# GuildOfWeavers/distaff

Hardware: AMD Instinct MI355X
Metric: trace_cells_per_sec (higher is better)
Workload: dtype u128 (prime field 2^128-45*2^40+1, 4x u32 limbs)

## Files before the change

### distaff_amd/csrc/air_kernel.h

```cpp
#pragma once
#include "ctx.h"
#include "air_stack_nested.h"

#ifndef AIR_THREADS
#define AIR_THREADS 128
#endif
#ifndef AIR_WAVES_PER_SIMD
#define AIR_WAVES_PER_SIMD 2
#endif

struct AirConsts { fe sponge_mds[16], sponge_inv_mds[16], hasher_mds[36], hasher_inv_mds[36]; };

struct AirArgs {
    const fe* lde;
    fe* out;
    const fe* coef;
    const fe* tc;
    const fe* periodic;
    const AirConsts* consts;
    fe* partial;
    fe* ev[10];
    const fe* tw_lo; const fe* tw_hi; uint32_t lo_bits;
    unsigned long long* bad_step;
    size_t n, col_stride;
    uint32_t log_n, log_N, log_b, W, ctx_depth, loop_depth, stack_depth;
    uint32_t cl, ll, sl;
    uint32_t coset_step;
    uint32_t q0;
    uint32_t num_inputs, num_outputs;
    fe inputs[8], outputs[8], program_hash[2], op_count;
};



__device__ __forceinline__ fe dpow(const AirArgs& a, uint64_t e) {
    uint32_t l = (uint32_t)e & ((1u << a.lo_bits) - 1u), h = (uint32_t)(e >> a.lo_bits);
    fe v = a.tw_lo[l];
    return h ? fe_mul(v, a.tw_hi[h]) : v;
}

template <int Wd>
__device__ __forceinline__ void matmul(fe* s, const fe* m) {
    fe r[Wd];
#pragma unroll
    for (int i = 0; i < Wd; i++) {
        fe_acc A; fe_acc_zero(A);
#pragma unroll
        for (int j = 0; j < Wd; j++) fe_acc_mac(A, m[i * Wd + j], s[j]);
        r[i] = fe_acc_reduce(A);
    }
#pragma unroll
    for (int i = 0; i < Wd; i++) s[i] = r[i];
}

#define AS_BOUNDARY 1
#define AS_OP_BITS 2
#define AS_SPONGE 4
#define AS_STACK_MOVE 8
#define AS_STACK_HIGH 16
#define AS_STACK_ARITH 32
#define AS_STACK_RESCR 64
#define AS_FLOW 128
#define AS_STACK_ANY (AS_STACK_MOVE | AS_STACK_HIGH | AS_STACK_ARITH | AS_STACK_RESCR)
#define AS_STACK_AUX (AS_STACK_MOVE | AS_STACK_ARITH)
#define AF_FIRST 1
#define AF_LAST 2
#define AF_EV_IN 4
#define AF_EV_OUT 8

struct AirStack {
    bool nested, deep;
    int sl;
    int slots;
    int partials;
};
constexpr AirStack air_stack(int sd, int slcap) {
    if (sd == 4) return AirStack{true, false, 8, 4, 6};
    if (sd == 0 && slcap == 8) return AirStack{true, false, 8, 8, 10};
    if (sd == 0 && slcap == 12) return AirStack{true, true, 12, 8, 10};
    return AirStack{false, false, sd ? (sd > 8 ? sd : 8) : slcap, 0, 0};
}

template <uint32_t ACC_MASK>
struct Acc {
    fe_acc res_acc;
    fe_acc adj_acc[6];
    fe res, adj[6];
    bool nonzero;
    const fe* tc; uint32_t nc;
    __device__ __forceinline__ void emit(uint32_t cidx, int slot, const fe& d) {
        nonzero |= !fe_is_zero(d);
        fe_acc_mac(res_acc, d, tc[cidx]);
        if ((ACC_MASK >> slot) & 1u) fe_acc_mac(adj_acc[slot], d, tc[nc + cidx]);
        else adj[slot] = fe_add(adj[slot], fe_mul(d, tc[nc + cidx]));
    }
};
constexpr uint32_t air_acc_mask(const AirStack& st, int sect) { return !st.nested ? 0u : ((sect & AS_OP_BITS) ? 0x01u : 0x3Fu); }

struct AirColumns {
    const fe* cur_p; const fe* nxt_p; size_t cs;
    __device__ __forceinline__ fe cur(size_t c) const { return cur_p[c * cs]; }
    __device__ __forceinline__ fe nxt(size_t c) const { return nxt_p[c * cs]; }
};

template <int CL, int LL>
struct AirRows {
    fe c_opc, n_opc, c_sp[4], n_sp[4], cf[3], n_cf[3], ld[5], hd[2];
    fe c_ctx[CL], n_ctx[CL], c_lp[LL], n_lp[LL];
};

template <int SL, int CL, int LL>
__device__ __forceinline__ void air_load_rows(AirRows<CL, LL>& r, fe* o, fe* nw, const AirArgs& a, const AirColumns p, int sd) {
    r.c_opc = p.cur(0); r.n_opc = p.nxt(0);
#pragma unroll
    for (int i = 0; i < 4; i++) { r.c_sp[i] = p.cur(1 + i); r.n_sp[i] = p.nxt(1 + i); }
#pragma unroll
    for (int i = 0; i < 3; i++) { r.cf[i] = p.cur(5 + i); r.n_cf[i] = p.nxt(5 + i); }
#pragma unroll
    for (int i = 0; i < 5; i++) r.ld[i] = p.cur(8 + i);
#pragma unroll
    for (int i = 0; i < 2; i++) r.hd[i] = p.cur(13 + i);
    uint32_t col = 15;
#pragma unroll
    for (int i = 0; i < CL; i++) { bool on = (uint32_t)i < a.ctx_depth; r.c_ctx[i] = on ? p.cur(col + i) : fe_zero(); r.n_ctx[i] = on ? p.nxt(col + i) : fe_zero(); }
    col += a.ctx_depth;
#pragma unroll
    for (int i = 0; i < LL; i++) { bool on = (uint32_t)i < a.loop_depth; r.c_lp[i] = on ? p.cur(col + i) : fe_zero(); r.n_lp[i] = on ? p.nxt(col + i) : fe_zero(); }
    col += a.loop_depth;
#pragma unroll
    for (int i = 0; i < SL; i++) { bool on = i < sd; o[i] = on ? p.cur(col + i) : fe_zero(); nw[i] = on ? p.nxt(col + i) : fe_zero(); }
}

struct AirFlags {
    fe cff[8], hdf[4], begin_flag, noop_flag, n_void, assert_flag;
    fe lo2[4], mid[4], top[2];
    fe ld_all;
    __device__ __forceinline__ fe ldf(int idx) const { return fe_mul(fe_mul(lo2[idx & 3], mid[(idx >> 2) & 3]), top[idx >> 4]); }
};

__device__ __forceinline__ void air_bit_pairs(fe* t, const fe& a, const fe& na, const fe& nb) {
    t[0] = fe_mul(na, nb); t[1] = fe_sub(nb, t[0]); t[2] = fe_sub(na, t[0]); t[3] = fe_sub(a, t[1]);
}

template <class ROWS>
__device__ __forceinline__ void air_op_flags(AirFlags& f, const ROWS& r) {
    const fe* cf = r.cf; const fe* ld = r.ld; const fe* hd = r.hd;
    {
        fe n0 = bnot(cf[0]), n1 = bnot(cf[1]), n2 = bnot(cf[2]);
        fe t[4];
        air_bit_pairs(t, cf[0], n0, n1);
#pragma unroll
        for (int i = 0; i < 4; i++) { f.cff[i] = fe_mul(t[i], n2); f.cff[4 + i] = fe_sub(t[i], f.cff[i]); }
        f.n_void = fe_mul(fe_mul(r.n_cf[0], r.n_cf[1]), r.n_cf[2]);
        fe l0 = bnot(ld[0]), l1 = bnot(ld[1]), l2 = bnot(ld[2]), l3 = bnot(ld[3]);
        f.lo2[0] = fe_mul(l0, l1); f.lo2[1] = fe_sub(l1, f.lo2[0]);
        f.lo2[2] = fe_mul(l0, cf[1]);
        f.lo2[3] = fe_sub(ld[0], f.lo2[1]);
        air_bit_pairs(f.mid, ld[2], l2, l3);
        f.top[0] = bnot(ld[4]); f.top[1] = ld[4];
        fe h0 = bnot(hd[0]), h1 = bnot(hd[1]);
        air_bit_pairs(f.hdf, hd[0], h0, h1);
    }
    {
        fe ld0 = f.ldf(0);
        f.ld_all = f.ldf(31);
        f.begin_flag = fe_mul(ld0, f.hdf[0]);
        f.noop_flag = fe_mul(f.ld_all, f.hdf[3]);
        f.hdf[0] = fe_mul(f.hdf[0], ld[0]);
        f.assert_flag = fe_mul(ld0, hd[0]);
    }
}

#include "air_stack_perop.h"

template <int CL, int LL, class ROWS>
__device__ __forceinline__ void air_boundary(const AirArgs& a, const ROWS& r, const fe* o, int cl, int ll, uint64_t gi, uint64_t n64, uint64_t nmask, uint32_t ql, size_t k) {
    const fe xp = dpow(a, (gi * (6 * n64 + 2)) & nmask);
    const fe one = fe_one();
#pragma unroll 1
    for (int pass = 0; pass < 2; pass++) {
        const fe* cc = a.coef + pass * 94;
        fe_acc R, A; fe_acc_zero(R); fe_acc_zero(A);
        auto term = [&](const fe& v, uint32_t idx) { fe_acc_mac(R, v, cc[idx]); fe_acc_mac(A, v, cc[idx + 1]); };
        term(pass ? fe_sub(r.c_opc, a.op_count) : r.c_opc, 0);
        if (pass == 0) { for (int i = 0; i < 4; i++) term(r.c_sp[i], 2 + 2 * i); }
        else { for (int i = 0; i < 2; i++) term(fe_sub(r.c_sp[i], a.program_hash[i]), 2 + 2 * i); }
        for (int i = 0; i < 3; i++) term(pass ? fe_sub(r.cf[i], one) : r.cf[i], 10 + 2 * i);
        for (int i = 0; i < 5; i++) term(pass ? fe_sub(r.ld[i], one) : r.ld[i], 16 + 2 * i);
        for (int i = 0; i < 2; i++) term(pass ? fe_sub(r.hd[i], one) : r.hd[i], 26 + 2 * i);
        for (int i = 0; i < CL; i++) if (i < cl) term(r.c_ctx[i], 30 + 2 * i);
        for (int i = 0; i < LL; i++) if (i < ll) term(r.c_lp[i], 62 + 2 * i);
        const uint32_t nio = pass ? a.num_outputs : a.num_inputs;
#pragma unroll
        for (int i = 0; i < 8; i++) if ((uint32_t)i < nio) term(fe_sub(o[i], pass ? a.outputs[i] : a.inputs[i]), 78 + 2 * i);
        const fe adj = fe_acc_reduce(A);
        fe_acc_mac(R, adj, xp);
        a.out[((size_t)pass * gridDim.y + ql) * a.n + k] = fe_acc_reduce(R);
    }
}

template <class ACC, class ROWS>
__device__ __forceinline__ void air_op_bits(ACC& acc, const ROWS& r, const AirFlags& f, const fe* per) {
    const fe* cf = r.cf; const fe* ld = r.ld; const fe* hd = r.hd;
    fe cf_sum = fe_add(fe_add(cf[0], cf[1]), cf[2]);
    const fe ld_prod = f.ld_all, hd_prod = f.hdf[3], all_prod = f.noop_flag;
#pragma unroll
    for (int i = 0; i < 3; i++) acc.emit(i, 0, is_bin(cf[i]));
#pragma unroll
    for (int i = 0; i < 5; i++) acc.emit(3 + i, 0, is_bin(ld[i]));
#pragma unroll
    for (int i = 0; i < 2; i++) acc.emit(8 + i, 0, is_bin(hd[i]));
    const fe is_hacc = f.cff[0];
    acc.emit(10, 1, fe_sub(fe_add(r.c_opc, is_hacc), r.n_opc));
    acc.emit(11, 5, fe_mul(r.c_opc, fe_add(fe_sub(bnot(ld_prod), hd_prod), all_prod)));
    acc.emit(12, 5, fe_mul(cf_sum, bnot(all_prod)));
    acc.emit(13, 3, fe_mul(f.cff[7], bnot(f.n_void)));
    fe prefix = fe_add(fe_add(f.cff[1], f.cff[4]), fe_add(f.cff[5], f.cff[6]));
    fe v = fe_mul(prefix, per[21]);
    v = fe_add(v, fe_mul(fe_add(f.cff[2], f.cff[3]), per[20]));
    v = fe_add(v, fe_mul(f.hdf[0], per[22]));
    acc.emit(14, 2, v);
}

template <bool OWN_CTX, class ACC, class ROWS>
__device__ __forceinline__ void air_sponge(ACC& acc, const AirArgs& a, const AirColumns p, const ROWS& r, const fe* nw, const AirFlags& f, const fe* per) {
    const AirConsts* consts = a.consts;
    fe ctx0;
    if constexpr (OWN_CTX) ctx0 = 0u < a.ctx_depth ? p.cur(15u) : fe_zero();
    else ctx0 = r.c_ctx[0];
    fe sp[4];
    const fe f_begin = f.cff[1], f_tend = f.cff[2], f_fend = f.cff[3], f_loop = f.cff[4], f_wrap = f.cff[5], f_break = f.cff[6], f_void = f.cff[7];
    {
        fe os[4], ns[4];
#pragma unroll
        for (int i = 0; i < 4; i++) os[i] = fe_cube(fe_add(r.c_sp[i], per[i]));
        matmul<4>(os, consts->sponge_mds);
        fe op_code = r.hd[1];
        op_code = fe_add(fe_double(op_code), r.hd[0]);
        op_code = fe_add(fe_double(op_code), r.ld[4]);
        op_code = fe_add(fe_double(op_code), r.ld[3]);
        op_code = fe_add(fe_double(op_code), r.ld[2]);
        op_code = fe_add(fe_double(op_code), r.ld[1]);
        op_code = fe_add(fe_double(op_code), r.ld[0]);
        os[0] = fe_add(os[0], op_code);
        os[1] = fe_add(os[1], fe_mul(nw[0], f.hdf[0]));
#pragma unroll
        for (int i = 0; i < 4; i++) ns[i] = r.n_sp[i];
        matmul<4>(ns, consts->sponge_inv_mds);
#pragma unroll
        for (int i = 0; i < 4; i++) ns[i] = fe_sub(fe_cube(ns[i]), per[4 + i]);
        const fe clr = fe_add(fe_add(f_begin, f_loop), f_wrap);
        const fe cpy = fe_add(f_break, f_void);
        const fe tf = fe_add(f_tend, f_fend);
        const fe xf[4] = {tf, f_tend, f_fend, tf};
        const fe xv[4] = {fe_sub(ctx0, r.n_sp[0]), fe_sub(r.c_sp[0], r.n_sp[1]), fe_sub(r.c_sp[0], r.n_sp[2]), r.n_sp[3]};
#pragma unroll
        for (int i = 0; i < 4; i++) {
            fe_acc A; fe_acc_zero(A);
            fe_acc_mac(A, f.cff[0], fe_sub(os[i], ns[i]));
            fe_acc_mac(A, clr, r.n_sp[i]);
            fe_acc_mac(A, cpy, fe_sub(r.c_sp[i], r.n_sp[i]));
            fe_acc_mac(A, xf[i], xv[i]);
            sp[i] = fe_acc_reduce(A);
        }
    }
    acc.emit(15, 3, sp[0]); acc.emit(16, 4, sp[1]); acc.emit(17, 3, sp[2]); acc.emit(18, 3, sp[3]);
}

template <class CUR>
__device__ __forceinline__ fe air_ctx_constraint(int i, int cl, const fe& push, const fe& pop, const fe& ccpy, const fe& sp0, CUR&& ctx_cur, const fe& ni) {
    fe_acc A; fe_acc_zero(A);
    fe_acc_mac(A, push, fe_sub(i == 0 ? sp0 : ctx_cur(i - 1), ni));
    fe_acc_mac(A, pop, i + 1 < cl ? fe_sub(ctx_cur(i + 1), ni) : ni);
    fe_acc_mac(A, ccpy, fe_sub(ctx_cur(i), ni));
    return fe_acc_reduce(A);
}

template <int CL, int LL, class ACC, class ROWS>
__device__ __forceinline__ void air_flow(ACC& acc, const AirArgs& a, const AirColumns p, const ROWS& r, const AirFlags& f, int cl, int ll) {
    const fe f_begin = f.cff[1], f_tend = f.cff[2], f_fend = f.cff[3], f_loop = f.cff[4], f_wrap = f.cff[5], f_break = f.cff[6], f_void = f.cff[7];
    acc.emit(19, 2, fe_mul(fe_add(f_wrap, f_break), fe_sub(r.c_sp[0], r.c_lp[0])));
    const fe push = fe_add(f_begin, f_loop), pop = fe_add(f_tend, f_fend), ccpy = fe_add(fe_add(f_wrap, f_break), f_void);
    const fe lcpy = fe_add(fe_add(fe_add(f_begin, f_tend), fe_add(f_fend, f_wrap)), f_void);
    if constexpr (CL <= 2 && LL <= 1) {
        auto ctx_cur = [&](int j) { return r.c_ctx[j < 0 ? 0 : (j < CL ? j : 0)]; };
#pragma unroll
        for (int i = 0; i < CL; i++) {
            if (i >= cl) break;
            const fe v = air_ctx_constraint(i, cl, push, pop, ccpy, r.c_sp[0], ctx_cur, r.n_ctx[i]);
            acc.emit(20 + i, 2, v);
        }
#pragma unroll
        for (int i = 0; i < LL; i++) {
            if (i >= ll) break;
            fe v = fe_mul(lcpy, fe_sub(r.c_lp[i], r.n_lp[i]));
            if (i >= 1) v = fe_add(v, fe_mul(f_loop, fe_sub(r.c_lp[i - 1 < 0 ? 0 : i - 1], r.n_lp[i])));
            v = fe_add(v, fe_mul(f_break, i + 1 < ll ? fe_sub(r.c_lp[i + 1 < LL ? i + 1 : 0], r.n_lp[i]) : r.n_lp[i]));
            acc.emit(20 + cl + i, 2, v);
        }
    } else {
        auto ctx_cur = [&](int i) { return (uint32_t)i < a.ctx_depth ? p.cur(15 + i) : fe_zero(); };
        auto ctx_nxt = [&](int i) { return (uint32_t)i < a.ctx_depth ? p.nxt(15 + i) : fe_zero(); };
        const uint32_t lcol = 15 + a.ctx_depth;
        auto lp_cur = [&](int i) { return (uint32_t)i < a.loop_depth ? p.cur(lcol + i) : fe_zero(); };
        auto lp_nxt = [&](int i) { return (uint32_t)i < a.loop_depth ? p.nxt(lcol + i) : fe_zero(); };
#pragma unroll 1
        for (int i = 0; i < cl; i++) {
            const fe ni = ctx_nxt(i);
            acc.emit(20 + i, 2, air_ctx_constraint(i, cl, push, pop, ccpy, r.c_sp[0], ctx_cur, ni));
        }
#pragma unroll 1
        for (int i = 0; i < ll; i++) {
            const fe ni = lp_nxt(i);
            fe_acc A; fe_acc_zero(A);
            fe_acc_mac(A, lcpy, fe_sub(lp_cur(i), ni));
            if (i >= 1) fe_acc_mac(A, f_loop, fe_sub(lp_cur(i - 1), ni));
            fe_acc_mac(A, f_break, i + 1 < ll ? fe_sub(lp_cur(i + 1), ni) : ni);
            acc.emit(20 + cl + i, 2, fe_acc_reduce(A));
        }
    }
}

template <int SD, int NS>
__device__ __forceinline__ void air_rescr_differences(fe* resc, const fe* o, const fe* nw, const fe* per, const AirConsts* consts) {
    constexpr int NZ = (SD != 0 && SD < 6) ? SD : 6;
    fe os[6], ns[6];
#pragma unroll
    for (int i = 0; i < 6; i++) os[i] = i < NZ ? fe_cube(fe_add(o[i], per[8 + i])) : per[23 + i];
    matmul<6>(os, consts->hasher_mds);
    constexpr int NR = NS < 6 ? NS : 6;
#pragma unroll
    for (int i = 0; i < NR; i++) {
        fe_acc A; fe_acc_zero(A);
#pragma unroll
        for (int j = 0; j < NZ; j++) fe_acc_mac(A, consts->hasher_inv_mds[i * 6 + j], nw[j]);
        ns[i] = fe_acc_reduce(A);
    }
#pragma unroll
    for (int i = 0; i < NR; i++) resc[i] = fe_sub(fe_sub(fe_cube(ns[i]), per[14 + i]), os[i]);
}

template <int SD, bool DEEP, int NS, int SL, uint32_t GROUPS, bool EV_IN, bool EV_OUT, class ACC, class ROWS>
__device__ __forceinline__ void air_stack_nested(ACC& acc, const AirArgs& a, const ROWS& r, const fe* o, const fe* nw, const AirFlags& f, const fe* per, int cl, int ll, int sl, int sd, size_t pidx) {
    StackRows rows;
#pragma unroll
    for (int i = 0; i < 8; i++) { rows.o[i] = o[i]; rows.nw[i] = nw[i]; }
#pragma unroll
    for (int i = 8; i < 12; i++) rows.o[i] = DEEP ? o[i < SL ? i : 0] : fe_zero();
    rows.sl = DEEP ? sl : 8;
    const fe lo0h = fe_mul(f.lo2[0], r.hd[0]);
    StackHigh high;
    high.push = f.hdf[0]; high.cmp = f.hdf[1]; high.rescr = f.hdf[2]; high.keep = fe_add(f.begin_flag, f.noop_flag);
    if constexpr ((GROUPS & AG_RESCR) != 0) air_rescr_differences<SD, NS>(high.resc, o, nw, per, a.consts);
    const uint32_t sbase = 20 + cl + ll;
    static_for_air<0, NS + 2>([&](auto k_) {
        constexpr int kk = decltype(k_)::value;
        constexpr int I = kk < NS ? kk : (kk == NS ? ST_AUX0 : ST_AUX1);
        constexpr bool touched = st_touches<I, GROUPS>();
        if constexpr (touched || !EV_OUT) {
            if (I >= 8 || I < sd) {
                fe v = fe_zero();
                if constexpr (touched) v = st_output<I, GROUPS, SD, DEEP>(rows, f.lo2, lo0h, f.mid, f.top, high);
                fe* slot = a.ev[I] + pidx;
                if constexpr (EV_IN) v = touched ? fe_add(v, *slot) : *slot;
                if constexpr (EV_OUT) *slot = v;
                else acc.emit(I >= 8 ? sbase + (I - 8) : sbase + 2 + I, 4, v);
            }
        } else if constexpr (!EV_IN) {
            a.ev[I][pidx] = fe_zero();
        }
    });
}

template <class ACC>
__device__ __forceinline__ void air_stack_deep_slots(ACC& acc, const AirArgs& a, const AirColumns p, const AirFlags& f, int cl, int ll, int sl, int sd) {
    const fe* lo2 = f.lo2; const fe* mid = f.mid; const fe* top = f.top;
    const uint32_t sbase = 20 + cl + ll;
    const fe lo_all = fe_add(fe_add(lo2[0], lo2[1]), fe_add(lo2[2], lo2[3]));
    fe fl1, fl2, fl4, fr1, fr2, fr4, fcp;
    { fe_acc A; fe_acc_zero(A); fe_acc_mac(A, mid[0], lo2[3]); fe_acc_mac(A, mid[2], lo_all); fl1 = fe_add(fe_mul(top[0], fe_acc_reduce(A)), f.assert_flag); }
    { fe_acc A; fe_acc_zero(A); fe_acc_mac(A, mid[0], fe_add(lo2[1], lo2[2])); fe_acc_mac(A, mid[1], fe_add(lo2[1], lo2[3])); fl2 = fe_mul(top[0], fe_acc_reduce(A)); }
    fl4 = fe_mul(top[0], fe_mul(mid[1], fe_add(lo2[0], lo2[2])));
    fr1 = fe_add(fe_mul(top[1], fe_mul(mid[0], fe_add(lo2[0], lo2[2]))), f.hdf[0]);
    { fe_acc A; fe_acc_zero(A); fe_acc_mac(A, mid[0], fe_add(lo2[1], lo2[3])); fe_acc_mac(A, mid[1], lo2[1]); fr2 = fe_mul(top[1], fe_acc_reduce(A)); }
    fr4 = fe_mul(top[1], fe_mul(mid[1], lo2[0]));
    {
        fe_acc A; fe_acc_zero(A); fe_acc_mac(A, mid[2], lo_all); fe_acc_mac(A, mid[3], fe_add(lo2[0], lo2[1]));
        fe_acc B; fe_acc_zero(B); fe_acc_mac(B, top[1], fe_acc_reduce(A)); fe_acc_mac(B, top[0], fe_mul(mid[3], fe_add(fe_add(lo2[0], lo2[1]), lo2[2])));
        fcp = fe_add(fe_add(fe_acc_reduce(B), fe_add(f.hdf[1], f.hdf[2])), fe_add(f.begin_flag, f.noop_flag));
    }
    const uint32_t scol = 15 + a.ctx_depth + a.loop_depth;
#pragma unroll 1
    for (int i = 8; i < sd; i++) {
        const fe ni = p.nxt(scol + i);
        auto item = [&](int j) { return p.cur(scol + j); };
        auto left = [&](int num) { return i + num < sl ? fe_sub(item(i + num), ni) : ni; };
        fe_acc A; fe_acc_zero(A);
        fe_acc_mac(A, fcp, fe_sub(item(i), ni));
        fe_acc_mac(A, fr1, fe_sub(item(i - 1), ni)); fe_acc_mac(A, fr2, fe_sub(item(i - 2), ni)); fe_acc_mac(A, fr4, fe_sub(item(i - 4), ni));
        fe_acc_mac(A, fl1, left(1)); fe_acc_mac(A, fl2, left(2)); fe_acc_mac(A, fl4, left(4));
        acc.emit(sbase + 2 + i, 4, fe_acc_reduce(A));
    }
}

__device__ __forceinline__ void air_combine(const fe& res, const fe* adj, const AirArgs& a, size_t k, uint32_t ql, uint32_t qg, uint64_t gi, uint64_t n64, uint64_t nmask) {
    const bool on_trace = (qg == 0);
    fe t;
    if (on_trace && k + 1 != a.n) {
        t = fe_zero();
    } else {
        const uint32_t degs[6] = {2, 3, 4, 6, 7, 8};
        fe_acc T; fe_acc_zero(T);
        fe_acc_add(T, res);
#pragma unroll
        for (int g = 0; g < 6; g++) {
            uint64_t p = 8 * n64 - 1 - (n64 - 1) * degs[g];
            fe_acc_mac(T, adj[g], dpow(a, (gi * p) & nmask));
        }
        t = fe_acc_reduce(T);
    }
    a.out[((size_t)2 * gridDim.y + ql) * a.n + k] = t;
}

template <int CL, int LL, int SD, int SLCAP, int SECT, uint32_t GROUPS, int FLAGS>
__global__ void __launch_bounds__(AIR_THREADS, AIR_WAVES_PER_SIMD) air_kernel(AirArgs a) {
    constexpr AirStack ST = air_stack(SD, SLCAP);
    constexpr bool FIRST = (FLAGS & AF_FIRST) != 0, LAST = (FLAGS & AF_LAST) != 0, EV_IN = (FLAGS & AF_EV_IN) != 0, EV_OUT = (FLAGS & AF_EV_OUT) != 0;
    static_assert(ST.nested ? (SECT & AS_STACK_ANY) == 0 : (GROUPS == 0 && !EV_IN && !EV_OUT),
                  "nested-sum instances select stack operations with GROUPS, the per-operation instance with SECT");
    const int cl = (int)a.cl, ll = (int)a.ll;
    const int sl = SD ? ST.sl : (int)a.sl;
    const int sd = SD ? SD : (int)a.stack_depth;
    const size_t k = (size_t)blockIdx.x * AIR_THREADS + threadIdx.x;
    if (k >= a.n) return;
    const uint32_t ql = blockIdx.y;
    const uint32_t qg = a.q0 + ql;
    const uint32_t jl = ql * a.coset_step;
    const size_t kn = (k + 1 == a.n) ? 0 : k + 1;
    const AirColumns cols{a.lde + (size_t)jl * a.n + k, a.lde + (size_t)jl * a.n + kn, a.col_stride};
    const uint64_t nmask = ((uint64_t)1 << a.log_N) - 1;
    const uint64_t gi = ((uint64_t)k << a.log_b) + (uint64_t)qg * a.coset_step;
    const uint32_t step = (uint32_t)(((uint64_t)k << 3) + qg);
    const uint64_t n64 = a.n;

    AirRows<CL, LL> rows;
    fe o[ST.sl], nw[ST.sl];
    air_load_rows<ST.sl>(rows, o, nw, a, cols, sd);
    if constexpr ((SECT & AS_BOUNDARY) != 0) air_boundary<CL, LL>(a, rows, o, cl, ll, gi, n64, nmask, ql, k);
    if constexpr (SECT == AS_BOUNDARY) return;
    AirFlags flags;
    air_op_flags(flags, rows);
    const fe* per = a.periodic + (size_t)(step & 127u) * AIR_PERIODIC_STRIDE;

    constexpr uint32_t ACC_MASK = air_acc_mask(ST, SECT);
    Acc<ACC_MASK> acc;
#pragma unroll
    for (int i = 0; i < 6; i++) if ((ACC_MASK >> i) & 1u) fe_acc_zero(acc.adj_acc[i]);
    fe_acc_zero(acc.res_acc); acc.res = fe_zero(); acc.nonzero = false; acc.tc = a.tc; acc.nc = 20 + cl + ll + 2 + sd;
#pragma unroll
    for (int i = 0; i < 6; i++) acc.adj[i] = fe_zero();
    const size_t pstride = (size_t)gridDim.y * a.n, pidx = (size_t)ql * a.n + k;

    if constexpr ((SECT & AS_OP_BITS) != 0) air_op_bits(acc, rows, flags, per);
    if constexpr ((SECT & AS_SPONGE) != 0) air_sponge<SD == 0>(acc, a, cols, rows, nw, flags, per);
    if constexpr ((SECT & AS_FLOW) != 0) air_flow<CL, LL>(acc, a, cols, rows, flags, cl, ll);
    if constexpr (ST.nested && (GROUPS & AG_STACK_ALL & ~AG_DEEP) != 0) air_stack_nested<SD, ST.deep, ST.slots, ST.sl, GROUPS, EV_IN, EV_OUT>(acc, a, rows, o, nw, flags, per, cl, ll, sl, sd, pidx);
    if constexpr (!ST.nested && (SECT & AS_STACK_ANY) != 0) air_stack_per_operation<ST.sl, SECT>(acc, o, nw, sl, sd, 20 + cl + ll, flags, per, a.consts);
    if constexpr (ST.deep && (GROUPS & AG_DEEP) != 0) air_stack_deep_slots(acc, a, cols, flags, cl, ll, sl, sd);

    constexpr bool EMITS_STACK = (SECT & AS_STACK_ANY) != 0 || (GROUPS & AG_DEEP) != 0 || ((GROUPS & AG_STACK_ALL) != 0 && !EV_OUT);
    constexpr uint32_t USED = ((SECT & AS_OP_BITS) ? 0x2Fu : 0u) | ((SECT & AS_SPONGE) ? 0x18u : 0u) | ((SECT & AS_FLOW) ? 0x04u : 0u) | (EMITS_STACK ? 0x10u : 0u);
    const bool on_trace = (qg == 0);
    if (on_trace && k + 1 != a.n && acc.nonzero) atomicMin(a.bad_step, (unsigned long long)k);
    acc.res = fe_acc_reduce(acc.res_acc);
#pragma unroll
    for (int i = 0; i < 6; i++) if (((ACC_MASK & USED) >> i) & 1u) acc.adj[i] = fe_add(acc.adj[i], fe_acc_reduce(acc.adj_acc[i]));
    if constexpr (!FIRST) {
        acc.res = fe_add(acc.res, a.partial[pidx]);
#pragma unroll
        for (int i = 0; i < 6; i++) if (LAST || ((USED >> i) & 1u)) acc.adj[i] = fe_add(acc.adj[i], a.partial[(size_t)(i + 1) * pstride + pidx]);
    }
    if constexpr (!LAST) {
        a.partial[pidx] = acc.res;
#pragma unroll
        for (int i = 0; i < 6; i++) if (FIRST || ((USED >> i) & 1u)) a.partial[(size_t)(i + 1) * pstride + pidx] = acc.adj[i];
        return;
    }
    air_combine(acc.res, acc.adj, a, k, ql, qg, gi, n64, nmask);
}


template <int CL, int LL, int SD, int SLCAP, int SECT, uint32_t GROUPS, int FLAGS>
static void launch_air(dst_ctx* c, const AirArgs& a, uint32_t Q) {
    dim3 g((unsigned)((c->n + AIR_THREADS - 1) / AIR_THREADS), Q);
    static char name[64];
    if (!name[0]) snprintf(name, sizeof(name), "air_kernel<%d,%d,%d,%d,%d,%u,%d>", CL, LL, SD, SLCAP, SECT, (unsigned)GROUPS, FLAGS);
    constexpr int NS = air_stack(SD, SLCAP).partials;
    const double units = c->W + ((FLAGS & AF_FIRST) ? 0 : 7) + ((FLAGS & AF_LAST) ? 1 : 7) + ((SECT & AS_BOUNDARY) ? 2 : 0) + ((FLAGS & AF_EV_IN) ? NS : 0) + ((FLAGS & AF_EV_OUT) ? NS : 0);
    { KScope ks_(c, name, 16.0 * c->n * Q * units, true); hipLaunchKernelGGL((air_kernel<CL, LL, SD, SLCAP, SECT, GROUPS, FLAGS>), g, dim3(AIR_THREADS), 0, c->stream, a); }
}
template <int CL, int LL, int SD, int SLCAP>
static void launch_air_boundary(dst_ctx* c, const AirArgs& a, uint32_t Q) {
#if DST_TEST_HOOKS
    if (dst_internal_boundary_by_evaluation(c)) launch_air<CL, LL, SD, SLCAP, AS_BOUNDARY, 0, 0>(c, a, Q);
#endif
}
void air_launch_sd4(dst_ctx* c, const AirArgs& a, uint32_t Q);
void air_launch_small(dst_ctx* c, const AirArgs& a, uint32_t Q);
void air_launch_deep(dst_ctx* c, const AirArgs& a, uint32_t Q);
void air_launch_generic(dst_ctx* c, const AirArgs& a, uint32_t Q);
```

### distaff_amd/csrc/api.hip

```cpp
#include <algorithm>
#include <cstdio>
#include <cstdlib>
#include "ctx.h"
#include "host/ctx_tables.h"
#include "host/steps.h"
#include "host_proof.h"
#include "host_util.h"
#include "host_vm.h"
#include "verify/host_verify.h"

using namespace dsth;
#include "host/steps_impl.h"
using step::wall_ms;
using step::event_ms;

static std::string g_create_error;

static std::vector<fe> build_periodic_table() {
    const size_t cyc = 128;
    std::vector<fe> out(cyc * AIR_PERIODIC_STRIDE);
    u128 w16 = fe_to_u128(h_root_of_unity(4)), w128 = fe_to_u128(h_root_of_unity(7));
    u128 w16_inv = hf_pow(w16, 15), inv16 = hf_pow(16, FIELD_P - 2);
    static const uint8_t masks[3][16] = {{0, 1, 1, 1, 1, 1, 1, 1, 1, 1, 1, 1, 1, 1, 1, 1}, {1, 1, 1, 1, 1, 1, 1, 1, 1, 1, 1, 1, 1, 1, 1, 0}, {0, 1, 1, 1, 1, 1, 1, 1, 0, 1, 1, 1, 1, 1, 1, 1}};
    for (int row = 0; row < 23; row++) {
        u128 vals[16], coef[16];
        for (int i = 0; i < 16; i++) vals[i] = row < 8 ? limbs(SPONGE_ARK[row][i]) : row < 20 ? limbs(HASHER_ARK[row - 8][i]) : (u128)masks[row - 20][i];
        for (int j = 0; j < 16; j++) {
            u128 acc = 0;
            for (int i = 0; i < 16; i++) acc = hf_add(acc, hf_mul(vals[i], hf_pow(w16_inv, (u128)((i * j) % 16))));
            coef[j] = hf_mul(acc, inv16);
        }
        for (size_t s = 0; s < cyc; s++) {
            u128 x = hf_pow(w128, s), acc = 0, pw = 1;
            for (int j = 0; j < 16; j++) { acc = hf_add(acc, hf_mul(coef[j], pw)); pw = hf_mul(pw, x); }
            out[s * AIR_PERIODIC_STRIDE + row] = fe_from_u128(acc);
        }
    }
    for (size_t s = 0; s < cyc; s++)
        for (int i = 0; i < 6; i++) { const u128 v = fe_to_u128(out[s * AIR_PERIODIC_STRIDE + 8 + i]); out[s * AIR_PERIODIC_STRIDE + 23 + i] = fe_from_u128(hf_mul(hf_mul(v, v), v)); }
    return out;
}

static void free_all(dst_ctx* c) {
    void* ptrs[] = {c->tw_lo, c->tw_hi, c->itw_lo, c->itw_hi, c->prescale, c->dit_last, c->tw4_lde, c->tw4_fwd, c->tw4_inv, c->tw4_row_fwd, c->tw4_row_inv, c->tmp2, c->periodic, c->trace == c->lde ? nullptr : c->trace, c->polys, c->lde, c->tmp,
                    c->trace_leaves, c->trace_nodes, c->air_consts, c->ceval, c->cwork, c->cpoly, c->cevals, c->cnodes, c->comp_poly, c->comp, c->scratch, c->d_u64, c->d_stage, c->d_fri_chain};
    for (void* p : ptrs) if (p) hipFree(p);
    for (auto& pass : c->ntt_stage_tw) for (fe_tw* p : pass) if (p) hipFree(p);
    for (auto& pass : c->ntt_pre_tw) for (fe_tw* p : pass) if (p) hipFree(p);
    for (auto& e : c->kpending) { hipEventDestroy(e.e0); hipEventDestroy(e.e1); }
    for (hipEvent_t e : c->event_pool) hipEventDestroy(e);
    if (c->gather_buf) hipFree(c->gather_buf);
    if (c->trace_upper) hipFree(c->trace_upper);
    if (c->c_upper) hipFree(c->c_upper);
    for (int d = 0; d < DST_MAX_FRI_LAYERS; d++) if (c->fri_upper[d]) hipFree(c->fri_upper[d]);
    if (c->fri_nat0) hipFree(c->fri_nat0);
    for (int d = 0; d < DST_MAX_FRI_LAYERS; d++) {
        if (d > 0 && c->fri_e[d]) hipFree(c->fri_e[d]);
        if (c->fri_leaves[d]) hipFree(c->fri_leaves[d]);
        if (c->fri_nodes[d]) hipFree(c->fri_nodes[d]);
    }
    for (hipEvent_t e : c->upload_done) hipEventDestroy(e);
    if (c->upload_stream) hipStreamDestroy(c->upload_stream);
    for (hipEvent_t e : c->comm_events) hipEventDestroy(e);
    if (c->comm_stream) hipStreamDestroy(c->comm_stream);
    if (c->d_status) hipFree(c->d_status);
    if (c->h_stage) hipHostFree(c->h_stage);
    for (hipEvent_t e : c->ph_ev) if (e) hipEventDestroy(e);
    for (hipEvent_t e : c->sh_ev) if (e) hipEventDestroy(e);
    for (auto& ce : c->coll_ev) { hipEventDestroy(ce.e0); hipEventDestroy(ce.e1); }
    if (c->stream) hipStreamDestroy(c->stream);
}

static int ctx_init(dst_ctx* c) {
    c->read_switches();
    const dst_params& p = c->prm;
    if (p.log_trace_length < 4 || p.log_trace_length > 24) { c->err = "log_trace_length must be in [4, 24]"; return DST_ERR_ARG; }
    if (p.log_blowup < 4 || p.log_blowup > 8) { c->err = "extension factor must be in [16, 256]"; return DST_ERR_ARG; }
    if (p.ctx_depth > 16 || p.loop_depth > 8) { c->err = "context / loop depth out of range"; return DST_ERR_ARG; }
    if (p.width >= 128 || p.width <= 15 + p.ctx_depth + p.loop_depth) { c->err = "register count out of range"; return DST_ERR_ARG; }
    if (p.num_queries == 0 || p.num_queries > 128 || p.grinding_factor > 32) { c->err = "invalid proof options"; return DST_ERR_ARG; }
    if (p.world == 0 || p.rank >= p.world || (p.world & (p.world - 1)) || p.world > 8 || p.world > (1u << p.log_blowup) / 2) {
        c->err = "invalid rank / world: world must be a power of two <= min(8, blowup / 2)"; return DST_ERR_ARG;
    }
    if (p.log_trace_length + p.log_blowup > 40) { c->err = "LDE domain exceeds 2^40"; return DST_ERR_ARG; }
    c->log_n = p.log_trace_length; c->log_b = p.log_blowup; c->log_N = c->log_n + c->log_b;
    c->n = (size_t)1 << c->log_n; c->B = (size_t)1 << c->log_b; c->N = c->n * c->B; c->W = p.width;
    c->Bc = c->B / p.world; c->j0 = c->Bc * p.rank;
    c->stack_depth = p.width - 15 - p.ctx_depth - p.loop_depth;
    if (c->stack_depth > 32) { c->err = "user stack deeper than 32 registers"; return DST_ERR_ARG; }
    c->device = p.device;
    HIP_TRY(c, hipSetDevice(c->device));
    HIP_TRY(c, hipStreamCreate(&c->stream));
    HIP_TRY(c, hipHostMalloc((void**)&c->h_stage, HS_TOTAL, hipHostMallocDefault));
    for (hipEvent_t& e : c->ph_ev) HIP_TRY(c, hipEventCreate(&e));

    fe wN = h_root_of_unity(c->log_N), wN_inv = h_inv(wN);
    c->tw_lo_bits = (c->log_N + 1) / 2;
    uint32_t hi_bits = c->log_N - c->tw_lo_bits;
    int r;
    if ((r = dev_upload(c, &c->tw_lo, h_powers(wN, (size_t)1 << c->tw_lo_bits)))) return r;
    if ((r = dev_upload(c, &c->tw_hi, h_powers(h_pow(wN, (u128)1 << c->tw_lo_bits), (size_t)1 << hi_bits)))) return r;
    if ((r = dev_upload(c, &c->itw_lo, h_powers(wN_inv, (size_t)1 << c->tw_lo_bits)))) return r;
    if ((r = dev_upload(c, &c->itw_hi, h_powers(h_pow(wN_inv, (u128)1 << c->tw_lo_bits), (size_t)1 << hi_bits)))) return r;
    if ((r = k_ntt_init(c))) return r;
    if ((r = dev_upload(c, &c->periodic, build_periodic_table()))) return r;
    c->n_inv = fe_from_u128(hf_pow((u128)c->n, FIELD_P - 2));
    c->n_inv_tw = fe_tw_make(c->n_inv);
    c->eight_inv = fe_from_u128(hf_pow(8, FIELD_P - 2));
    c->four_inv = fe_from_u128(hf_pow(4, FIELD_P - 2));
    c->iota = h_root_of_unity(2);
    c->g_trace = h_root_of_unity(c->log_n);
    c->x_last = h_inv(c->g_trace);

    const size_t n = c->n, Nl = c->Bc * n;
    if ((r = dev_alloc(c, &c->polys, (c->W + c->prm.world - 1) / c->prm.world * c->prm.world * n))) return r;
    if ((r = dev_alloc(c, &c->lde, c->W * Nl))) return r;
    if (c->j0 == 0 && c->Bc > 1 && !c->sw_is("DISTAFF_TRACE_BUFFER", "1")) { c->trace = c->lde; c->trace_stride = Nl; }
    else { if ((r = dev_alloc(c, &c->trace, c->W * n))) return r; c->trace_stride = n; }
    size_t stage_cap = (size_t)12 << 30;
    { size_t free_b = 0, total_b = 0; if (hipMemGetInfo(&free_b, &total_b) == hipSuccess && free_b / 4 < stage_cap) stage_cap = free_b / 4; }
    c->tmp_regs = 4;
    while (c->tmp_regs < c->W && (c->tmp_regs + 1) * (c->plan.count == 3 ? 2 : 1) * c->Bc * n * sizeof(fe) <= stage_cap) c->tmp_regs++;
    if (const char* e = c->sw("DISTAFF_TMP_REGS")) { const long k = atol(e); if (k >= 4 && k <= (long)c->W) c->tmp_regs = (size_t)k; }
    if ((r = dev_alloc(c, &c->tmp, c->Bc * c->tmp_regs * n))) return r;
    if (c->plan.count == 3 && (r = dev_alloc(c, &c->tmp2, c->Bc * c->tmp_regs * n))) return r;
    if ((r = dev_alloc(c, &c->trace_leaves, Nl))) return r;
    if ((r = dev_alloc(c, &c->trace_nodes, Nl))) return r;
    if ((r = dev_alloc(c, &c->ceval, 3 * 8 * n))) return r;
    if ((r = dev_alloc(c, &c->cwork, 8 * 8 * n))) return r;
    if ((r = dev_alloc(c, &c->cpoly, 8 * n))) return r;
    if ((r = dev_alloc(c, &c->cevals, Nl))) return r;
    if ((r = dev_alloc(c, &c->cnodes, Nl / 2))) return r;
    if ((r = dev_alloc(c, &c->comp_poly, 8 * n))) return r;
    if ((r = dev_alloc(c, &c->comp, Nl))) return r;
    c->scratch_elems = (size_t)1 << 21;
    if ((r = dev_alloc(c, &c->scratch, c->scratch_elems))) return r;
    if ((r = dev_alloc(c, &c->d_u64, 64))) return r;
    if ((r = dev_alloc(c, &c->d_fri_chain, DST_MAX_FRI_LAYERS * 48))) return r;
    c->stage_bytes = (size_t)8 << 20;
    if ((r = dev_alloc(c, &c->d_stage, c->stage_bytes))) return r;
    size_t sz = c->N;
    int d = 0;
    for (;; d++) {
        if (d >= DST_MAX_FRI_LAYERS) { c->err = "too many FRI layers"; return DST_ERR_ARG; }
        c->fri_size[d] = sz;
        if (d == 0) c->fri_e[0] = c->comp;
        else if ((r = dev_alloc(c, &c->fri_e[d], sz))) return r;
        if ((r = dev_alloc(c, &c->fri_leaves[d], sz / 4))) return r;
        if ((r = dev_alloc(c, &c->fri_nodes[d], sz / 4))) return r;
        if (sz <= 256) break;
        sz /= 4;
    }
    c->num_fri_layers = d + 1;
    return DST_OK;
}

static const fe* as_fe(const uint8_t* p) { return reinterpret_cast<const fe*>(p); }
static std::vector<fe> copy_fe(const uint8_t* p, size_t count) { std::vector<fe> v(count); memcpy(v.data(), p, count * 16); return v; }

static int drain_pending_upload(dst_ctx* c) {
    if (c->upload_pending && c->upload_stream) HIP_TRY(c, hipStreamSynchronize(c->upload_stream));
    c->upload_pending = false;
    return DST_OK;
}


int dst_ctx_create(const dst_params* params, dst_ctx** out) {
    if (!params || !out) { g_create_error = "null argument"; return DST_ERR_ARG; }
    dst_ctx* c = new dst_ctx();
    c->prm = *params;
    int r = ctx_init(c);
    if (r == DST_OK && c->prm.world > 1) r = ensure_shard_buffers(c);
    if (r != DST_OK) { g_create_error = c->err; free_all(c); delete c; *out = nullptr; return r; }
    *out = c;
    return DST_OK;
}
void dst_ctx_destroy(dst_ctx* c) { if (!c) return; hipSetDevice(c->device); free_all(c); delete c; }
const char* dst_last_error(const dst_ctx* c) { return c ? c->err.c_str() : g_create_error.c_str(); }
int dst_phase_ms(const dst_ctx* c, double out_ms[9]) { if (!c || !out_ms) return DST_ERR_ARG; for (int i = 0; i < 9; i++) out_ms[i] = c->phase_ms[i]; return DST_OK; }

int dst_trace_upload(dst_ctx* c, const uint8_t* const* cols) {
    if (!c || !cols) return DST_ERR_ARG;
    HIP_TRY(c, hipSetDevice(c->device));
    { int rd = drain_pending_upload(c); if (rd) return rd; }
    for (size_t i = 0; i < c->W; i++) HIP_TRY(c, hipMemcpyAsync(c->trace + i * c->trace_stride, cols[i], c->n * 16, hipMemcpyHostToDevice, c->stream));
    HIP_TRY(c, hipStreamSynchronize(c->stream));
    c->upload_pending = false; c->trace_owned_only = false;
    c->have_trace = true; c->committed = c->constraints_done = c->composed = false;
    return DST_OK;
}
int dst_trace_upload_owned(dst_ctx* c, const uint8_t* const* cols) {
    if (!c || !cols) return DST_ERR_ARG;
    HIP_TRY(c, hipSetDevice(c->device));
    { int rd = drain_pending_upload(c); if (rd) return rd; }
    for (size_t i = c->prm.rank; i < c->W; i += c->prm.world) {
        if (!cols[i]) { c->err = "dst_trace_upload_owned: register " + std::to_string(i) + " belongs to this rank but has no data"; return DST_ERR_ARG; }
        HIP_TRY(c, hipMemcpyAsync(c->trace + i * c->trace_stride, cols[i], c->n * 16, hipMemcpyHostToDevice, c->stream));
    }
    HIP_TRY(c, hipStreamSynchronize(c->stream));
    c->upload_pending = false; c->trace_owned_only = c->prm.world > 1;
    c->have_trace = true; c->committed = c->constraints_done = c->composed = false;
    return DST_OK;
}
int dst_trace_upload_contiguous(dst_ctx* c, const uint8_t* cols) {
    if (!c || !cols) return DST_ERR_ARG;
    HIP_TRY(c, hipSetDevice(c->device));
    { int rd = drain_pending_upload(c); if (rd) return rd; }
    for (size_t i = 0; i < c->W; i++) HIP_TRY(c, hipMemcpy(c->trace + i * c->trace_stride, cols + i * c->n * 16, c->n * 16, hipMemcpyHostToDevice));
    c->upload_pending = false; c->trace_owned_only = false;
    c->have_trace = true; c->committed = c->constraints_done = c->composed = false;
    return DST_OK;
}

int dst_pinned_alloc(size_t bytes, void** out) {
    if (!out || bytes == 0) return DST_ERR_ARG;
    return hipHostMalloc(out, bytes, hipHostMallocDefault) == hipSuccess ? DST_OK : DST_ERR_HIP;
}
int dst_pinned_free(void* p) { return (!p || hipHostFree(p) == hipSuccess) ? DST_OK : DST_ERR_HIP; }

int dst_trace_upload_async(dst_ctx* c, const uint8_t* const* cols) {
    if (!c || !cols) return DST_ERR_ARG;
    HIP_TRY(c, hipSetDevice(c->device));
    if (!c->upload_stream) HIP_TRY(c, hipStreamCreateWithFlags(&c->upload_stream, hipStreamNonBlocking));
    { int rd = drain_pending_upload(c); if (rd) return rd; }
    HIP_TRY(c, hipStreamSynchronize(c->stream));
    c->upload_bounds.clear();
    for (size_t first = 0; first < c->W;) { c->upload_bounds.push_back(first); first += (first == 0 && c->W > 4) ? (c->W % 4 ? c->W % 4 : 1) : 4; }
    c->upload_bounds.push_back(c->W);
    const size_t groups = c->upload_bounds.size() - 1;
    while (c->upload_done.size() < groups) { hipEvent_t e; HIP_TRY(c, hipEventCreateWithFlags(&e, hipEventDisableTiming)); c->upload_done.push_back(e); }
    for (size_t g = 0; g < groups; g++) {
        for (size_t i = c->upload_bounds[g]; i < c->upload_bounds[g + 1]; i++)
            HIP_TRY(c, hipMemcpyAsync(c->trace + i * c->trace_stride, cols[i], c->n * 16, hipMemcpyHostToDevice, c->upload_stream));
        HIP_TRY(c, hipEventRecord(c->upload_done[g], c->upload_stream));
    }
    c->upload_pending = true; c->trace_owned_only = false;
    c->have_trace = true; c->committed = c->constraints_done = c->composed = false;
    return DST_OK;
}

int dst_commit_trace(dst_ctx* c, uint8_t trace_root[32]) {
    if (!c || !trace_root) return DST_ERR_ARG;
    if (!c->have_trace) { c->err = "dst_commit_trace: no trace uploaded"; return DST_ERR_STATE; }
    if (c->trace_owned_only) { c->err = "dst_commit_trace: only this rank's registers were uploaded (dst_trace_upload_owned): use dst_prove_sharded"; return DST_ERR_STATE; }
    HIP_TRY(c, hipSetDevice(c->device));
    c->sharded_layout = false;
    double t0 = wall_ms();
    HIP_TRY(c, hipEventRecord(c->ph_ev[4], c->stream));
    if (c->upload_pending) {
        for (size_t g = 0; g + 1 < c->upload_bounds.size(); g++) {
            const size_t first = c->upload_bounds[g], cnt = c->upload_bounds[g + 1] - first;
            HIP_TRY(c, hipStreamWaitEvent(c->stream, c->upload_done[g], 0));
            k_intt_columns(c, c->trace + first * c->trace_stride, c->trace_stride, c->polys + first * c->n, cnt);
            k_lde_columns(c, c->polys + first * c->n, c->lde + first * c->Bc * c->n, cnt);
        }
        c->upload_pending = false;
    } else {
        k_intt_columns(c, c->trace, c->trace_stride, c->polys, c->W);
        k_lde_columns(c, c->polys, c->lde, c->W);
    }
    HIP_TRY(c, hipEventRecord(c->ph_ev[5], c->stream));
    k_trace_leaves(c);
    k_merkle(c, c->trace_leaves, c->trace_nodes, c->Bc * c->n, 0);
    HIP_TRY(c, hipMemcpyAsync(c->trace_root, c->trace_nodes + 1, 32, hipMemcpyDeviceToHost, c->stream));
    fe last[3];
    for (int i = 0; i < 3; i++) HIP_TRY(c, hipMemcpyAsync(&last[i], c->trace + (size_t)i * c->trace_stride + (c->n - 1), 16, hipMemcpyDeviceToHost, c->stream));
    HIP_TRY(c, hipStreamSynchronize(c->stream));
    HIP_TRY(c, hipGetLastError());
    c->op_count = (uint64_t)fe_to_u128(last[0]); c->op_counter = last[0];
    c->program_hash[0] = last[1]; c->program_hash[1] = last[2];
    memcpy(trace_root, c->trace_root, 32);
    {
        const double total = wall_ms() - t0;
        double lde_ms = event_ms(c->ph_ev[4], c->ph_ev[5]);
        if (lde_ms < 0 || lde_ms > total) lde_ms = 0;
        c->phase_ms[0] = lde_ms; c->phase_ms[1] = total - lde_ms;
    }
    c->committed = true; c->constraints_done = c->composed = false;
    return DST_OK;
}

int dst_eval_constraints(dst_ctx* c, const dst_public* pub, const uint8_t* coeffs, uint8_t constraint_root[32], int64_t* bad_step) {
    if (!c || !pub || !coeffs || !constraint_root) return DST_ERR_ARG;
    if (!c->committed) { c->err = "dst_eval_constraints: trace not committed"; return DST_ERR_STATE; }
    if (pub->num_inputs > 8 || pub->num_outputs > 8) { c->err = "too many public inputs / outputs"; return DST_ERR_ARG; }
    if (c->prm.world != 1) { c->err = "dst_eval_constraints: multi-GPU combination is driven by the host (see distaff_amd/sharded.py)"; return DST_ERR_ARG; }
    HIP_TRY(c, hipSetDevice(c->device));
    const double t0 = wall_ms();
    HIP_TRY(c, hipEventRecord(c->ph_ev[0], c->stream));
    const bool steps = dst_internal_combine_by_steps(c);
    int r = step::eval_constraints(c, pub, coeffs, bad_step, !steps);
    if (r != DST_OK) return r;
    HIP_TRY(c, hipEventRecord(c->ph_ev[1], c->stream));
    if ((r = step::combine(c, 3))) return r;
    HIP_TRY(c, hipEventRecord(c->ph_ev[2], c->stream));
    k_lde_fold8(c, c->cpoly, c->cevals);
    k_constraint_tree(c);
    HIP_TRY(c, hipMemcpyAsync(c->constraint_root, c->cnodes + 1, 32, hipMemcpyDeviceToHost, c->stream));
    HIP_TRY(c, hipEventRecord(c->ph_ev[3], c->stream));
    HIP_TRY(c, hipStreamSynchronize(c->stream));
    HIP_TRY(c, hipGetLastError());
    if (!steps) {
        c->air_flag_host = *reinterpret_cast<unsigned long long*>(c->h_stage + HS_AIR_FLAG);
        if ((r = k_constraint_check(c, bad_step)) != DST_OK) { c->err = "transition constraints were not satisfied"; return r; }
    }
    memcpy(constraint_root, c->constraint_root, 32);
    auto between = [&](int from, int to) { const double ms = event_ms(c->ph_ev[from], c->ph_ev[to]); return ms > 0 ? ms : 0.0; };
    const double total = wall_ms() - t0, e1 = between(0, 1), e2 = between(1, 2), e3 = between(2, 3);
    const double rest = total > e1 + e2 + e3 ? total - (e1 + e2 + e3) : 0.0;
    c->phase_ms[2] = e1 + rest / 2; c->phase_ms[3] = e2; c->phase_ms[4] = e3 + rest / 2;
    c->constraints_done = true; c->composed = false;
    return DST_OK;
}

static void finish_deep_values(dst_ctx* c) {
    if (!c->deep_pending) return;
    const size_t W = c->W;
    c->deep_z1.assign(c->h_stage + HS_DEEP, c->h_stage + HS_DEEP + W * 16);
    c->deep_z2.assign(c->h_stage + HS_DEEP + HS_DEEP_HALF, c->h_stage + HS_DEEP + HS_DEEP_HALF + W * 16);
    c->deep_pending = false;
}
static int compose_impl(dst_ctx* c, const uint8_t* draws_bytes, uint8_t* trace_at_z1, uint8_t* trace_at_z2, bool wait);
int dst_compose(dst_ctx* c, const uint8_t* draws_bytes, uint8_t* trace_at_z1, uint8_t* trace_at_z2) {
    if (!c || !draws_bytes || !trace_at_z1 || !trace_at_z2) return DST_ERR_ARG;
    return compose_impl(c, draws_bytes, trace_at_z1, trace_at_z2, true);
}
static int compose_impl(dst_ctx* c, const uint8_t* draws_bytes, uint8_t* trace_at_z1, uint8_t* trace_at_z2, bool wait) {
    if (!c->constraints_done) { c->err = "dst_compose: constraints not evaluated"; return DST_ERR_STATE; }
    HIP_TRY(c, hipSetDevice(c->device));
    double t0 = wall_ms();
    HIP_TRY(c, hipEventRecord(c->ph_ev[0], c->stream));
    const size_t n = c->n, D = 8 * n, W = c->W;
    std::vector<fe> draws = copy_fe(draws_bytes, 516);
    const fe z = draws[0];
    const fe next_z = fe_mul(z, c->g_trace);
    const fe k1 = draws[513], k2 = draws[514], k3 = draws[515];
    const step::ScratchTail tail(c);
    fe* d_draws = tail.draws(); fe* d_tz1 = tail.tz1(); fe* d_tz2 = tail.tz2(); fe* d_cz = tail.cz();
    {
        fe* h_draws = reinterpret_cast<fe*>(c->h_stage + HS_COMPOSE);
        memcpy(h_draws, draws.data(), 516 * 16);
        HIP_TRY(c, hipMemcpyAsync(d_draws, h_draws, 516 * 16, hipMemcpyHostToDevice, c->stream));
    }
    const bool steps = dst_internal_combine_by_steps(c);
    const fe zz[2] = {z, next_z};
    k_horner(c, c->polys, W, n, z, d_tz1);
    k_horner(c, c->polys, W, n, next_z, d_tz2);
    fe* t1 = c->cwork; fe* t2 = c->cwork + n; fe* cp = c->cwork + D;
    k_lincomb2(c, c->polys, W, n, d_draws + 1, 256, t1, t2);
    const size_t inc = 6 * n + 1;
    if (steps) {
        k_sub_dot_at0(c, t1, d_tz1, d_draws + 1, W);
        k_sub_dot_at0(c, t2, d_tz2, d_draws + 257, W);
        k_syn_div(c, t1, n, z);
        k_syn_div(c, t2, n, next_z);
        k_add(c, t1, t2, n);
        HIP_TRY(c, hipMemsetAsync(c->comp_poly, 0, D * 16, c->stream));
        k_axpy(c, c->comp_poly, t1, k1, n);
        k_axpy(c, c->comp_poly + inc, t1, k2, n);
        k_horner(c, c->cpoly, 1, D, z, d_cz);
        HIP_TRY(c, hipMemcpyAsync(cp, c->cpoly, D * 16, hipMemcpyDeviceToDevice, c->stream));
        k_sub_at0(c, cp, d_cz);
        k_syn_div(c, cp, D, z);
        k_axpy(c, c->comp_poly, cp, k3, D);
    } else {
        fe* both[2] = {t1, t2};
        k_syn_div_batch(c, both, zz, 2, n);
        k_add(c, t1, t2, n);
        k_syn_div_compose(c, c->cpoly, c->comp_poly, D, z, t1, n, inc, k1, k2, k3);
    }
    k_lde_fold8(c, c->comp_poly, c->comp);
    HIP_TRY(c, hipEventRecord(c->ph_ev[1], c->stream));
    HIP_TRY(c, hipMemcpyAsync(c->h_stage + HS_DEEP, d_tz1, W * 16, hipMemcpyDeviceToHost, c->stream));
    HIP_TRY(c, hipMemcpyAsync(c->h_stage + HS_DEEP + HS_DEEP_HALF, d_tz2, W * 16, hipMemcpyDeviceToHost, c->stream));
    c->deep_pending = true;
    if (wait) {
        CTX_SYNC(c, "the DEEP composition");
        HIP_TRY(c, hipGetLastError());
        finish_deep_values(c);
        memcpy(trace_at_z1, c->deep_z1.data(), W * 16);
        memcpy(trace_at_z2, c->deep_z2.data(), W * 16);
    }
    c->phase_ms[5] = wall_ms() - t0;
    c->composed = true; c->fri_committed = 0; c->fri_folded = 0; c->fri_roots.clear(); c->fri_tail_pending = false;
    return DST_OK;
}

int dst_fri_commit_layer(dst_ctx* c, uint8_t layer_root[32], int* more) {
    if (!c || !layer_root || !more) return DST_ERR_ARG;
    if (!c->composed) { c->err = "dst_fri_commit_layer: composition not built"; return DST_ERR_STATE; }
    int d = c->fri_committed;
    if (d >= c->num_fri_layers || d != c->fri_folded) { c->err = "dst_fri_commit_layer: fold the previous layer first"; return DST_ERR_STATE; }
    HIP_TRY(c, hipSetDevice(c->device));
    double t0 = wall_ms();
    if (d == 0) k_fri_leaves_layer0(c); else k_fri_leaves(c, d);
    k_merkle(c, c->fri_leaves[d], c->fri_nodes[d], c->fri_size[d] / 4, 0);
    uint8_t root[32];
    HIP_TRY(c, hipMemcpyAsync(root, c->fri_nodes[d] + 1, 32, hipMemcpyDeviceToHost, c->stream));
    HIP_TRY(c, hipStreamSynchronize(c->stream));
    HIP_TRY(c, hipGetLastError());
    memcpy(layer_root, root, 32);
    step::fri_file_root(c, d, root);
    c->fri_committed = d + 1;
    *more = (d + 1 < c->num_fri_layers) ? 1 : 0;
    if (d == 0) c->phase_ms[6] = 0;
    c->phase_ms[6] += wall_ms() - t0;
    return DST_OK;
}
int dst_fri_fold(dst_ctx* c, const uint8_t special_x[16]) {
    if (!c || !special_x) return DST_ERR_ARG;
    int d = c->fri_folded;
    if (d + 1 != c->fri_committed || d + 1 >= c->num_fri_layers) { c->err = "dst_fri_fold: nothing to fold"; return DST_ERR_STATE; }
    HIP_TRY(c, hipSetDevice(c->device));
    double t0 = wall_ms();
    k_fri_fold(c, d, fe_from_bytes(special_x));
    c->fri_folded = d + 1;
    c->phase_ms[6] += wall_ms() - t0;
    return DST_OK;
}

int dst_pow_grind(dst_ctx* c, const uint8_t seed[32], uint32_t grinding_factor, uint8_t out_seed[32], uint64_t* nonce) {
    if (!c || !seed || !out_seed || !nonce || grinding_factor > 64) return DST_ERR_ARG;
    HIP_TRY(c, hipSetDevice(c->device));
    int r = k_pow(c, seed, grinding_factor, nonce);
    if (r != DST_OK) return r;
    uint8_t buf[64];
    memset(buf, 0, 64);
    memcpy(buf, seed, 32);
    memcpy(buf + 32, nonce, 8);
    blake3_short(buf, 64, out_seed);
    return DST_OK;
}

int dst_build_proof(dst_ctx* c, const uint64_t* positions_in, uint32_t num_positions, uint64_t pow_nonce, uint8_t* out, size_t cap, size_t* out_len) {
    if (!c || !positions_in || !out_len) return DST_ERR_ARG;
    if (!c->composed || c->fri_committed != c->num_fri_layers) { c->err = "dst_build_proof: FRI commit phase not finished"; return DST_ERR_STATE; }
    if (c->prm.world != 1) { c->err = "dst_build_proof: single-GPU contexts only"; return DST_ERR_ARG; }
    HIP_TRY(c, hipSetDevice(c->device));
    double t0 = wall_ms();
    finish_deep_values(c);
    std::vector<uint8_t> proof;
    int rc = build_proof_local(c, positions_in, num_positions, pow_nonce, proof);
    if (rc == DST_OK) {
        *out_len = proof.size();
        if (out) {
            if (cap < proof.size()) { c->err = "proof buffer too small"; rc = DST_ERR_ARG; }
            else memcpy(out, proof.data(), proof.size());
        }
    }
    c->phase_ms[8] = wall_ms() - t0;
    return rc;
}

static int fri_commit_all(dst_ctx* c, bool chained) {
    if (chained) {
        if (!c->composed || c->fri_committed != 0 || c->fri_folded != 0) { c->err = "dst_prove: FRI state"; return DST_ERR_STATE; }
        return step::fri_commit_natural(c, 0);
    }
    for (;;) {
        if (fri_tail_starts_at(c, c->fri_committed)) return step::fri_commit_natural(c, c->fri_committed);
        uint8_t root[32]; int more = 0, rc;
        if ((rc = dst_fri_commit_layer(c, root, &more))) return rc;
        if (!more) return DST_OK;
        fe sx = prng(root);
        if ((rc = dst_fri_fold(c, (const uint8_t*)&sx))) return rc;
    }
}

int dst_prove(dst_ctx* c, const dst_public* pub, uint8_t* proof_out, size_t cap, size_t* proof_len) {
    if (!c || !pub || !proof_len) return DST_ERR_ARG;
    int rc;
    uint8_t trace_root[32], constraint_root[32];
    if ((rc = dst_commit_trace(c, trace_root))) return rc;
    std::vector<fe> coef(344);
    prng_vector(trace_root, 344, coef.data());
    int64_t bad = -1;
    if ((rc = dst_eval_constraints(c, pub, (const uint8_t*)coef.data(), constraint_root, &bad))) return rc;
    std::vector<fe> draws(516);
    prng_vector(constraint_root, 516, draws.data());
    std::vector<uint8_t> z1(c->W * 16), z2(c->W * 16);
    const double t_compose = wall_ms();
    if ((rc = compose_impl(c, (const uint8_t*)draws.data(), z1.data(), z2.data(), false))) return rc;
    {
        const char* ce = c->sw("DISTAFF_FRI_CHAIN");
        if ((rc = fri_commit_all(c, !(ce && ce[0] == '0')))) return rc;
        const double both = wall_ms() - t_compose, dev = event_ms(c->ph_ev[0], c->ph_ev[1]);
        if (dev > 0 && dev < both) { c->phase_ms[5] = dev; c->phase_ms[6] = both - dev; }
        else { c->phase_ms[6] = both > c->phase_ms[5] ? both - c->phase_ms[5] : 0.0; }
    }
    double t0 = wall_ms();
    uint64_t nonce = 0;
    std::vector<uint64_t> positions;
    if ((rc = step::query_seed(c, &nonce, positions))) return rc;
    c->phase_ms[7] = wall_ms() - t0;
    return dst_build_proof(c, positions.data(), (uint32_t)positions.size(), nonce, proof_out, cap, proof_len);
}

void dst_prng_vector(const uint8_t seed[32], uint32_t count, uint8_t* out) {
    std::vector<fe> v(count);
    prng_vector(seed, count, v.data());
    memcpy(out, v.data(), (size_t)count * 16);
}
int dst_query_positions(const uint8_t seed[32], uint64_t domain_size, uint32_t blowup, uint32_t num_queries, uint64_t* out) {
    if (!seed || !out || domain_size == 0 || blowup == 0 || num_queries == 0 || num_queries > 128) return DST_ERR_ARG;
    std::vector<uint64_t> p;
    if (query_positions(seed, domain_size, blowup, num_queries, p)) return DST_ERR_ARG;
    memcpy(out, p.data(), p.size() * 8);
    return (int)p.size();
}
void dst_blake3(const uint8_t* in, size_t len, uint8_t out[32]) { if (!blake3_short(in, len, out)) memset(out, 0, 32); }

int dst_fibonacci_trace(uint32_t log_n, uint8_t* cols, uint8_t program_hash[32], uint8_t result[16]) {
    if (!cols || !program_hash || !result || log_n < 7 || log_n > 26) return DST_ERR_ARG;
    u128 ph[2], res;
    int r = fibonacci_trace(log_n, (u128*)cols, ph, &res);
    if (r) return DST_ERR_ARG;
    memcpy(program_hash, ph, 32);
    memcpy(result, &res, 16);
    return DST_OK;
}

static void put_text(char* err, size_t err_cap, const std::string& s) { if (err && err_cap) snprintf(err, err_cap, "%s", s.c_str()); }
int dst_verify(const uint8_t program_hash[32], const dst_public* pub, const uint8_t* proof, size_t len, int* accepted, char* err, size_t err_cap) {
    if (accepted) *accepted = 0;
    put_text(err, err_cap, "");
    if (!program_hash || !pub || !accepted || pub->num_inputs > 8 || pub->num_outputs > 8) { put_text(err, err_cap, "invalid argument"); return DST_ERR_ARG; }
    hver::VProof p;
    std::string why;
    if (hver::parse_proof(proof, len, p, why)) { put_text(err, err_cap, why); return DST_ERR_ARG; }
    u128 in[8], out[8];
    memcpy(in, pub->inputs, sizeof(in)); memcpy(out, pub->outputs, sizeof(out));
    for (uint32_t i = 0; i < 8; i++)
        if ((i < pub->num_inputs && in[i] >= FIELD_P) || (i < pub->num_outputs && out[i] >= FIELD_P)) { put_text(err, err_cap, "public value not below the modulus"); return DST_ERR_ARG; }
    hver::VerifyResult r = hver::verify_proof(program_hash, in, pub->num_inputs, out, pub->num_outputs, p);
    *accepted = r.ok ? 1 : 0;
    put_text(err, err_cap, r.error);
    return DST_OK;
}
int dst_proof_info(const uint8_t* proof, size_t len, dst_proof_info_t* info) {
    if (!info) return DST_ERR_ARG;
    memset(info, 0, sizeof(*info));
    hver::VProof p;
    std::string why;
    if (hver::parse_proof(proof, len, p, why)) return DST_ERR_ARG;
    info->log_trace_length = (uint32_t)p.domain_depth - p.log_blowup;
    info->extension_factor = 1u << p.log_blowup; info->num_queries = p.num_queries; info->grinding_factor = p.grinding;
    info->ctx_depth = p.ctx_depth; info->loop_depth = p.loop_depth; info->stack_depth = p.stack_depth;
    info->register_count = 15u + p.ctx_depth + p.loop_depth + p.stack_depth;
    info->op_count = p.op_count;
    info->fri_layers = (uint32_t)p.layers.size(); info->remainder_length = (uint32_t)p.rem_values.size();
    info->security_level = hver::security_level(p, true); info->security_level_proven = hver::security_level(p, false);
    info->pow_nonce = p.pow_nonce;
    return DST_OK;
}

#include "host/rtree_impl.h"
#include "host/stree_impl.h"

int dst_read_buffer(dst_ctx* c, uint32_t what, uint32_t arg, uint8_t* out, size_t cap, size_t* len) {
    if (!c || !len) return DST_ERR_ARG;
    HIP_TRY(c, hipSetDevice(c->device));
    const size_t n = c->n, Nl = c->Bc * n;
    const void* src = nullptr; size_t bytes = 0;
    const fe* coset_major = nullptr; size_t cosets = 0;
    switch (what) {
        case DST_BUF_POLYS: src = c->polys; bytes = c->W * n * 16; break;
        case DST_BUF_LDE: if (arg >= c->W) return DST_ERR_ARG; coset_major = c->lde + (size_t)arg * Nl; cosets = c->Bc; break;
        case DST_BUF_TRACE_LEAVES: src = c->trace_leaves; bytes = Nl * 32; break;
        case DST_BUF_TRACE_NODES: src = c->trace_nodes; bytes = Nl * 32; break;
        case DST_BUF_CEVAL_I: case DST_BUF_CEVAL_F: case DST_BUF_CEVAL_T: coset_major = c->ceval + (size_t)(what - DST_BUF_CEVAL_I) * 8 * n; cosets = 8; break;
        case DST_BUF_CPOLY: src = c->cpoly; bytes = 8 * n * 16; break;
        case DST_BUF_CEVALS: coset_major = c->cevals; cosets = c->Bc; break;
        case DST_BUF_CNODES: src = c->cnodes; bytes = Nl / 2 * 32; break;
        case DST_BUF_COMP_POLY: src = c->comp_poly; bytes = 8 * n * 16; break;
        case DST_BUF_COMP_EVALS: coset_major = c->comp; cosets = c->Bc; break;
        case DST_BUF_FRI_EVALS:
            if ((int)arg >= c->num_fri_layers) return DST_ERR_ARG;
            if (arg == 0) { coset_major = c->comp; cosets = c->Bc; } else { src = c->fri_e[arg]; bytes = c->fri_size[arg] * 16; }
            break;
        case DST_BUF_FRI_NODES: if ((int)arg >= c->num_fri_layers) return DST_ERR_ARG; src = c->fri_nodes[arg]; bytes = c->fri_size[arg] / 4 * 32; break;
        case DST_BUF_FRI_LEAVES: if ((int)arg >= c->num_fri_layers) return DST_ERR_ARG; src = c->fri_leaves[arg]; bytes = c->fri_size[arg] / 4 * 32; break;
        default: c->err = "unknown buffer id"; return DST_ERR_ARG;
    }
    if (coset_major) bytes = cosets * n * 16;
    *len = bytes;
    if (!out) return DST_OK;
    if (cap < bytes) { c->err = "output buffer too small"; return DST_ERR_ARG; }
    if (coset_major) {
        fe* tmp = nullptr;
        HIP_TRY(c, hipMalloc((void**)&tmp, bytes));
        k_coset_to_natural_len(c, coset_major, cosets, c->n, tmp);
        hipError_t e = hipMemcpyAsync(out, tmp, bytes, hipMemcpyDeviceToHost, c->stream);
        if (e == hipSuccess) e = hipStreamSynchronize(c->stream);
        hipFree(tmp);
        HIP_TRY(c, e);
    } else {
        HIP_TRY(c, hipMemcpyAsync(out, src, bytes, hipMemcpyDeviceToHost, c->stream));
        HIP_TRY(c, hipStreamSynchronize(c->stream));
    }
    return DST_OK;
}

int dst_field_op(dst_ctx* c, int op, const uint8_t* a, const uint8_t* b, uint8_t* out, size_t count) {
    if (!c || !a || !b || !out) return DST_ERR_ARG;
    HIP_TRY(c, hipSetDevice(c->device));
    return k_field_op(c, op, a, b, out, count);
}
int dst_set_profiling(dst_ctx* c, int level) { if (!c || level < 0 || level > 2) return DST_ERR_ARG; c->profile = level; return DST_OK; }
int dst_kernel_stats(dst_ctx* c, char* json_out, size_t cap, int reset) {
    if (!c || !json_out) return DST_ERR_ARG;
    HIP_TRY(c, hipSetDevice(c->device));
    HIP_TRY(c, hipStreamSynchronize(c->stream));
    for (auto& e : c->kpending) {
        const double ms = event_ms(e.e0, e.e1);
        if (ms >= 0) { auto& st = c->kstats[e.name]; st.launches++; st.ms += ms; st.bytes += e.bytes; st.mads += e.mads; }
        c->event_pool.push_back(e.e0); c->event_pool.push_back(e.e1);
    }
    c->kpending.clear();
    std::string js = "{";
    bool first = true;
    for (auto& kv : c->kstats) {
        char buf[256];
        snprintf(buf, sizeof(buf), "%s\"%s\": {\"launches\": %llu, \"ms\": %.6f, \"bytes\": %.0f, \"mads\": %.0f}", first ? "" : ", ", kv.first.c_str(),
                 (unsigned long long)kv.second.launches, kv.second.ms, kv.second.bytes, kv.second.mads);
        js += buf; first = false;
    }
    js += "}";
    if (reset) c->kstats.clear();
    if (js.size() + 1 > cap) { c->err = "stats buffer too small"; return DST_ERR_ARG; }
    memcpy(json_out, js.c_str(), js.size() + 1);
    return DST_OK;
}

#if DST_TEST_HOOKS
int dst_bench_mulmod(dst_ctx* c, uint64_t lanes, uint32_t iters, double* ms) {
    if (!c || !ms) return DST_ERR_ARG;
    HIP_TRY(c, hipSetDevice(c->device));
    return k_bench_mulmod(c, lanes, iters, ms);
}
int dst_bench_code(dst_ctx* c, uint32_t code_kib, double* ms) {
    if (!c || !ms) return DST_ERR_ARG;
    HIP_TRY(c, hipSetDevice(c->device));
    return k_bench_code(c, code_kib, ms);
}
int dst_bench_clock(dst_ctx* c, uint64_t lanes, uint32_t iters, double* mhz) {
    if (!c || !mhz) return DST_ERR_ARG;
    HIP_TRY(c, hipSetDevice(c->device));
    return k_bench_clock(c, lanes, iters, mhz);
}
int dst_bench_mad(dst_ctx* c, uint64_t lanes, uint32_t iters, double* ms) {
    if (!c || !ms) return DST_ERR_ARG;
    HIP_TRY(c, hipSetDevice(c->device));
    return k_bench_mad(c, lanes, iters, ms);
}
#else
static int no_hooks(dst_ctx* c) { if (c) c->err = "calibration kernels are part of the test / bench build (libdistaff_hip_hooks.so) only"; return c ? DST_ERR_STATE : DST_ERR_ARG; }
int dst_bench_mulmod(dst_ctx* c, uint64_t, uint32_t, double*) { return no_hooks(c); }
int dst_bench_code(dst_ctx* c, uint32_t, double*) { return no_hooks(c); }
int dst_bench_mad(dst_ctx* c, uint64_t, uint32_t, double*) { return no_hooks(c); }
int dst_bench_clock(dst_ctx* c, uint64_t, uint32_t, double*) { return no_hooks(c); }
#endif
int dst_test_hooks(void) { return DST_TEST_HOOKS; }
```

### distaff_amd/csrc/ctx.h

```cpp
#pragma once
#include <hip/hip_runtime.h>
#include <stdint.h>
#include <string.h>
#include <memory>
#include <string>
#include <map>
#include <vector>
#include "fe.h"
#include "../../include/distaff_hip.h"

struct __attribute__((aligned(16))) digest { uint32_t w[8]; };
#define AIR_PERIODIC_STRIDE 29

#ifndef NTT_TW4_PAIRS
#define NTT_TW4_PAIRS 0
#endif
#if NTT_TW4_PAIRS
typedef fe_tw tw4_t;
#else
typedef fe tw4_t;
#endif

#define DST_MAX_FRI_LAYERS 24

struct dst_switch_def { const char* name; bool product; const char* values; const char* what; };
static const dst_switch_def DST_SWITCHES[] = {
    {"DISTAFF_SHARD_DEBUG",        true,  "1",               "stderr line per tree exchange on rank 0; communicators record the order of their collectives (dst_comm_trace)"},
    {"DISTAFF_SHARD_TREE_GATHER",  true,  "1",               "sharded Merkle trees: all-gather of all boundary nodes + upper levels repeated on every rank (BASELINE north_star's all-gather-only form) instead of the k-range all-to-all"},
    {"DISTAFF_SHARD_NO_OVERLAP",   true,  "1",               "sharded prover: every collective on the context's main stream (no second stream / events) also on a stream-ordered transport"},
    {"DISTAFF_COMM_TIMEOUT_S",     true,  "seconds",         "communicators: limit of every host wait behind a collective (default 60; <= 0: none); on expiry the rank aborts the communicator and returns DST_ERR_COMM (dst_comm_set_timeout changes it per handle)"},
    {"DISTAFF_LOCAL_TRANSPORT",    true,  "blocking",        "in-process transport (dst_comm_init_local, dst_prove_sharded_local): drain every rank's stream around each collective instead of the stream-ordered form (events between the ranks' streams, nothing waited for)"},
    {"DISTAFF_TMP_REGS",           true,  "4..W",            "registers per transform launch = size of the staging array (default: as many as 12 GiB hold, at most W)"},
    {"DISTAFF_AIR",                false, "small|deep|generic", "force a more general constraint-kernel instance set than the trace shape needs (generic = per-operation formulation)"},
    {"DISTAFF_BOUNDARY",           false, "eval",            "boundary combinations by evaluation on the 8n domain (the reference's route) instead of coefficient form"},
    {"DISTAFF_COMBINE",            false, "steps",           "combine_polys / DEEP composition as the reference's sequence of whole-array steps instead of the fused passes"},
    {"DISTAFF_NTT",                false, "pre|pre_a|3pass|reg|lds|row", "force a transform plan family (pre_a: a register pre-stage in the first pass only; row: the default plan with row-major staging array and tables)"},
    {"DISTAFF_NTT_SHAPE",          false, "a,b",             "three-pass plans: log2 of the first two pass lengths"},
    {"DISTAFF_NTT_ORDER",          false, "0",               "first pass of an extension in coset-slow block order"},
    {"DISTAFF_NTT_WAVES",          false, "4|8",             "force the 512- or 1024-lane instances of the LDS passes"},
    {"DISTAFF_NTT_FIXED",          false, "0",               "use the any-shape instances where a shape-compiled one exists"},
    {"DISTAFF_NTT_DIF",            false, "0|1|2",           "first pass of an extension: coset DIT (0), pre-scale + DIF (1), DIT with last-stage twiddles from global memory (2)"},
    {"DISTAFF_NTT_DEBUG",          false, "1",               "print the occupancy of every transform launch shape once"},
    {"DISTAFF_LDE_BATCH",          false, "cols,cosets",     "registers x cosets per transform launch"},
    {"DISTAFF_FOLD8_DFT",          false, "0",               "8n-coefficient extensions without the fused fold + 8-point step"},
    {"DISTAFF_TRACE_BUFFER",       false, "1",               "give the trace its own buffer instead of coset 0 of the extension"},
    {"DISTAFF_MERKLE_LEVEL2_LOG",  false, "k",               "build two tree levels per launch from 2^k grandparents per launch on (default 2^19)"},
    {"DISTAFF_MERKLE_LEVELS",      false, "1",               "one launch per tree level"},
    {"DISTAFF_SYN_DIV_TABLES",     false, "1",               "synthetic division by power tables + scan instead of the blocked form"},
    {"DISTAFF_FRI_TAIL",           false, "0",               "no single-launch tail: every FRI layer by its own launches (the tail otherwise starts at the first layer of at most 2^13 elements)"},
    {"DISTAFF_FRI_CHAIN",          false, "0",               "FRI commit phase with a root read-back and a host draw per layer"},
    {"DISTAFF_FRI_REPLICATE_LOG",  false, "k",               "sharded prover: replicate FRI layers from 2^k elements on (default 2^17)"},
    {"DISTAFF_SHARD_FORCE_OVERLAP", false, "1",              "sharded prover: the two-stream choreography of a stream-ordered transport over a blocking one"},
    {"DISTAFF_TEST_STALL_COLLECTIVE", false, "k|k@r",        "communicators: fault injection -- before device collective number k (of rank r only) a kernel holds the stream until the communicator is aborted"},
};
enum : size_t {
    HS_WEIGHTS = 0,
    HS_WEIGHTS_BYTES = (4 * 128 + 4) * 16,
    HS_DEEP = 32768,
    HS_DEEP_HALF = 2048,
    HS_FRI_ROOTS = 40960,
    HS_FRI_SLOTS = 45056,
    HS_FRI_SLOT_BYTES = 800,
    HS_AIR_FLAG = 65536 - 64,
    HS_DRAWS = 65536,
    HS_DRAWS_BYTES = (344 + 160) * 16,
    HS_COMPOSE = 65536 + 8192,
    HS_COMPOSE_BYTES = 516 * 16,
    HS_STATUS = 65536 + 8192 + 8320,
    HS_STATUS_SLOTS = 32,
    HS_TREE_READBACK = 65536 + 8192 + 8320 + 2048,
    HS_TAIL_ROOTS = HS_TREE_READBACK + 1024,
    HS_POW = HS_TAIL_ROOTS + 1024,
    HS_TOTAL = 131072
};
static_assert(HS_WEIGHTS + HS_WEIGHTS_BYTES <= HS_DEEP, "boundary weights overlap the DEEP values");
static_assert(HS_DEEP_HALF >= 128 * 16 && HS_DEEP + 2 * HS_DEEP_HALF <= HS_FRI_ROOTS, "DEEP values: W <= 128 registers");
static_assert(HS_FRI_ROOTS + DST_MAX_FRI_LAYERS * 32 <= HS_FRI_SLOTS, "FRI roots overlap the layer slots");
static_assert(8 * 96 + 32 <= HS_FRI_SLOT_BYTES && HS_FRI_SLOTS + DST_MAX_FRI_LAYERS * HS_FRI_SLOT_BYTES <= HS_AIR_FLAG, "FRI layer slots: G <= 8 ranks, DST_MAX_FRI_LAYERS layers");
static_assert(HS_DRAWS + HS_DRAWS_BYTES <= HS_COMPOSE && HS_COMPOSE + HS_COMPOSE_BYTES <= HS_STATUS && HS_STATUS + HS_STATUS_SLOTS * 64 <= HS_TOTAL, "upload regions overlap");
static_assert(HS_STATUS_SLOTS >= 2 + DST_MAX_FRI_LAYERS, "one status slot per tree exchange of a proof");
static_assert(HS_STATUS + HS_STATUS_SLOTS * 64 <= HS_TREE_READBACK && 8 * 96 + 32 <= 1024 && DST_MAX_FRI_LAYERS * 32 <= 1024 && HS_POW + 64 <= HS_TOTAL, "read-back regions overlap");

#ifdef DISTAFF_TEST_HOOKS
#define DST_TEST_HOOKS 1
#else
#define DST_TEST_HOOKS 0
#endif

enum {
    DST_BUF_POLYS = 0,
    DST_BUF_LDE = 1,
    DST_BUF_TRACE_LEAVES = 2,
    DST_BUF_TRACE_NODES = 3,
    DST_BUF_CEVAL_I = 4,
    DST_BUF_CEVAL_F = 5,
    DST_BUF_CEVAL_T = 6,
    DST_BUF_CPOLY = 7,
    DST_BUF_CEVALS = 8,
    DST_BUF_CNODES = 9,
    DST_BUF_COMP_POLY = 10,
    DST_BUF_COMP_EVALS = 11,
    DST_BUF_FRI_EVALS = 12,
    DST_BUF_FRI_NODES = 13,
    DST_BUF_FRI_LEAVES = 14,
};

struct NttInstance;
struct NttRegInstance;
enum NttKind : uint32_t { NTT_FIRST, NTT_MIDDLE, NTT_LAST };
struct NttPass {
    NttKind kind = NTT_FIRST;
    uint32_t log_len = 0;
    uint32_t log_tile = 0, pre = 0;
    uint32_t dit = 0;
    size_t lds = 0;
    const NttInstance* inst = nullptr;
    const NttRegInstance* reg = nullptr;
    const fe_tw* stage_tw[2] = {nullptr, nullptr}; const fe_tw* pre_tw[2] = {nullptr, nullptr}; const tw4_t* tw4[2] = {nullptr, nullptr};
};
struct NttPlan {
    uint32_t log_n1 = 0, log_n2 = 0;
    uint32_t log_n3 = 0;
    uint32_t count = 0;
    bool coset_slow = false; uint32_t debug = 0;
    bool tile_major = false;
    NttPass pass[3], first_lde;
    const NttPass& at(uint32_t i, bool lde) const { return (i == 0 && lde) ? first_lde : pass[i]; }
};

struct dst_ctx {
    dst_params prm{};
    std::string err;
    std::map<std::string, std::string> sw_values;
    const char* sw(const char* name) const { auto it = sw_values.find(name); return it == sw_values.end() ? nullptr : it->second.c_str(); }
    bool sw_is(const char* name, const char* value) const { const char* v = sw(name); return v && !strcmp(v, value); }
    bool sw_flag(const char* name) const { const char* v = sw(name); return v && v[0] && v[0] != '0'; }
    void read_switches() {
        sw_values.clear();
        for (const dst_switch_def& d : DST_SWITCHES)
            if (d.product || DST_TEST_HOOKS) if (const char* v = getenv(d.name)) sw_values[d.name] = v;
    }
    int device = 0;
    hipStream_t stream = nullptr;

    uint32_t log_n = 0, log_b = 0, log_N = 0;
    size_t n = 0, B = 0, N = 0, W = 0;
    size_t Bc = 0, j0 = 0;
    size_t stack_depth = 0;
    NttPlan plan;
    std::vector<fe> air_draws;
    std::shared_ptr<void> open_plan;
    std::vector<uint64_t> open_plan_positions;
    uint8_t open_plan_root[32] = {0};
    int fri_rep_from = 0;
    bool fri_tail_pending = false;
    fe* fri_nat0 = nullptr;
    bool sharded_layout = false;

    fe *tw_lo = nullptr, *tw_hi = nullptr;
    fe *itw_lo = nullptr, *itw_hi = nullptr;
    uint32_t tw_lo_bits = 0;
    fe_tw *ntt_stage_tw[3][2] = {}, *ntt_pre_tw[3][2] = {};
    fe_tw *prescale = nullptr;
    fe_tw *dit_last = nullptr;
    tw4_t *tw4_lde = nullptr;
    tw4_t *tw4_fwd = nullptr, *tw4_inv = nullptr;
    tw4_t *tw4_row_fwd = nullptr, *tw4_row_inv = nullptr;
    fe *tmp2 = nullptr;
    fe *periodic = nullptr;
    void *air_consts = nullptr;
    fe c16f[8], c16i[8];
    fe_tw n_inv_tw{};
    fe n_inv{}, eight_inv{}, four_inv{}, iota{}, g_trace{}, x_last{};

    fe *trace = nullptr, *polys = nullptr, *lde = nullptr, *tmp = nullptr;
    size_t tmp_regs = 4;
    size_t trace_stride = 0;
    digest *trace_leaves = nullptr, *trace_nodes = nullptr;
    fe *ceval = nullptr;
    fe *cwork = nullptr;
    fe *cpoly = nullptr;
    fe *cevals = nullptr;
    digest *cnodes = nullptr;
    fe *comp_poly = nullptr;
    fe *comp = nullptr;
    fe *scratch = nullptr;
    size_t scratch_elems = 0;
    int num_fri_layers = 0, fri_committed = 0, fri_folded = 0;
    fe *fri_e[DST_MAX_FRI_LAYERS] = {nullptr};
    digest *fri_leaves[DST_MAX_FRI_LAYERS] = {nullptr};
    digest *fri_nodes[DST_MAX_FRI_LAYERS] = {nullptr};
    size_t fri_size[DST_MAX_FRI_LAYERS] = {0};
    digest *trace_upper = nullptr, *c_upper = nullptr, *fri_upper[DST_MAX_FRI_LAYERS] = {nullptr};
    uint8_t *gather_buf = nullptr; size_t gather_bytes = 0;
    bool tree_krange[2 + DST_MAX_FRI_LAYERS] = {false};
    uint64_t *d_u64 = nullptr;
    uint8_t *d_fri_chain = nullptr;
    uint8_t *h_stage = nullptr;
    unsigned long long air_flag_host = ~0ull;
    hipEvent_t ph_ev[6] = {nullptr};
    uint8_t *d_stage = nullptr;
    size_t stage_bytes = 0;

    dst_public pub{};
    uint8_t trace_root[32] = {0}, constraint_root[32] = {0};
    std::vector<uint8_t> deep_z1, deep_z2;
    bool deep_pending = false;
    std::vector<std::vector<uint8_t>> fri_roots;
    uint64_t op_count = 0;
    fe op_counter{};
    fe program_hash[2] = {};
    bool have_trace = false, committed = false, constraints_done = false, composed = false;
    hipStream_t upload_stream = nullptr;
    std::vector<hipEvent_t> upload_done;
    std::vector<size_t> upload_bounds;
    bool upload_pending = false;
    bool trace_owned_only = false;
    bool ceval_inverted = false;
    hipStream_t comm_stream = nullptr;
    std::vector<hipEvent_t> comm_events;
    uint8_t* d_status = nullptr;
    double phase_ms[9] = {0};
    double shard_ms[2] = {0, 0};
    uint32_t shard_trees = 0;
    struct dst_comm* wait_comm = nullptr;
    hipEvent_t sh_ev[8] = {nullptr};
    struct CollEv { hipEvent_t e0, e1; int kind; };
    std::vector<CollEv> coll_ev;
    size_t coll_used = 0;
    double exchange_ms[8] = {0};

    int profile = 0;
    struct KEvent { hipEvent_t e0, e1; std::string name; double bytes, mads; };
    std::vector<KEvent> kpending;
    std::vector<hipEvent_t> event_pool;
    struct KStat { uint64_t launches = 0; double ms = 0, bytes = 0, mads = 0; };
    std::map<std::string, KStat> kstats;
};

struct KScope {
    dst_ctx* c; bool on;
    dst_ctx::KEvent ev;
    KScope(dst_ctx* ctx, const char* name, double bytes, bool heavy = false, double mads = 0.0) : c(ctx), on(ctx->profile == 1 || (ctx->profile == 2 && heavy)) {
        if (!on) return;
        ev.name = name; ev.bytes = bytes; ev.mads = mads;
        if (c->event_pool.size() >= 2) { ev.e0 = c->event_pool.back(); c->event_pool.pop_back(); ev.e1 = c->event_pool.back(); c->event_pool.pop_back(); }
        else if (hipEventCreate(&ev.e0) != hipSuccess || hipEventCreate(&ev.e1) != hipSuccess) { on = false; return; }
        (void)hipEventRecord(ev.e0, c->stream);
    }
    ~KScope() { if (on) { (void)hipEventRecord(ev.e1, c->stream); c->kpending.push_back(ev); } }
};

#define HIP_TRY(ctx, expr)                                                                          \
    do {                                                                                            \
        hipError_t _e = (expr);                                                                     \
        if (_e != hipSuccess) {                                                                     \
            (ctx)->err = std::string(#expr) + ": " + hipGetErrorString(_e);                          \
            return DST_ERR_HIP;                                                                     \
        }                                                                                           \
    } while (0)

int ctx_sync(dst_ctx* c, const char* what);
#define CTX_SYNC(ctx, what) do { const int _r = ctx_sync((ctx), (what)); if (_r) return _r; } while (0)

inline bool dst_internal_boundary_by_evaluation(const dst_ctx* c) { return DST_TEST_HOOKS && c->sw_is("DISTAFF_BOUNDARY", "eval"); }
inline bool dst_internal_combine_by_steps(const dst_ctx* c) { return DST_TEST_HOOKS && (c->sw_is("DISTAFF_COMBINE", "steps") || dst_internal_boundary_by_evaluation(c)); }
inline bool fri_tail_starts_at(const dst_ctx* c, int d) {
    if (d < 1 || d >= c->num_fri_layers || c->fri_size[d] > ((size_t)1 << 13)) return false;
    const char* e = c->sw("DISTAFF_FRI_TAIL");
    return !(e && e[0] == '0');
}
int k_ntt_init(dst_ctx* c);
void k_intt_columns(dst_ctx* c, const fe* src, size_t src_stride, fe* dst, size_t ncols);
void k_lde_columns(dst_ctx* c, const fe* polys, fe* lde, size_t ncols);
void k_lde_fold8(dst_ctx* c, const fe* poly8n, fe* out);
void k_intt8_cosets(dst_ctx* c, fe* vals , fe* out8n, fe* work);
void k_coset_to_natural_len(dst_ctx* c, const fe* src, size_t cosets, size_t len, fe* dst);
void k_fri_leaves_at(dst_ctx* c, const fe* e, digest* leaves, size_t R);
void k_fri_fold_at(dst_ctx* c, const fe* e, fe* out, size_t R, int layer, fe special_x, const fe* alpha_dev = nullptr);
void k_trace_leaves(dst_ctx* c);
void k_merkle(dst_ctx* c, const digest* leaves, digest* nodes, size_t count, size_t stop_count);
void k_constraint_tree(dst_ctx* c);
void k_fri_leaves_layer0(dst_ctx* c);
void k_fri_leaves(dst_ctx* c, int layer);
int k_eval_constraints(dst_ctx* c, const fe* coeffs_dev, const fe* tc_dev, int64_t* bad_step, bool defer_check = false);
int k_constraint_check(dst_ctx* c, int64_t* bad_step);
void k_syn_div(dst_ctx* c, fe* a, size_t len, fe b);
void k_syn_div_batch(dst_ctx* c, fe* const* a, const fe* b, int count, size_t len);
void k_syn_div_compose(dst_ctx* c, const fe* a, fe* out, size_t len, fe b, const fe* t, size_t tn, size_t inc, fe k1, fe k2, fe k3);
void k_combine_fused(dst_ctx* c, const fe* work, const fe* q4, size_t q_stride, fe* cpoly);
void k_syn_div_expanded(dst_ctx* c, const fe* a, fe* out, size_t len, size_t degree, fe exception);
void k_horner(dst_ctx* c, const fe* polys, size_t ncols, size_t len, fe x, fe* out_dev);
void k_lincomb2(dst_ctx* c, const fe* cols, size_t ncols, size_t len, const fe* coeffs_dev, size_t coef_stride, fe* out0, fe* out1);
void k_lincomb4(dst_ctx* c, const fe* cols, size_t ncols, size_t len, const fe* coeffs_dev, fe* out0, fe* out1, fe* out2, fe* out3);
void k_axpy(dst_ctx* c, fe* y, const fe* x, fe a, size_t len);
void k_add(dst_ctx* c, fe* y, const fe* x, size_t len);
void k_sub_dot_at0(dst_ctx* c, fe* y, const fe* values_dev, const fe* coeffs_dev, size_t count);
void k_sub_at0(dst_ctx* c, fe* y, const fe* v_dev);
void k_fri_fold(dst_ctx* c, int layer, fe special_x);
void k_fri_fold_dev(dst_ctx* c, int layer, const fe* alpha_dev);
void k_fri_draw(dst_ctx* c, int layer, fe* alpha_out, digest* root_out);
void k_intt_cosets_local(dst_ctx* c, fe* vals, fe* out, size_t cosets);
void k_cross8(dst_ctx* c, const fe* work, fe* out8n);
int k_fri_tail(dst_ctx* c, int first, uint8_t* roots_out);
int k_pow(dst_ctx* c, const uint8_t seed[32], uint32_t grinding, uint64_t* nonce);
void k_gather(dst_ctx* c, const void* src, size_t item_bytes, const uint64_t* idx_dev, size_t count, void* dst);
void k_gather_rows(dst_ctx* c, const uint64_t* positions_dev, size_t count, fe* out);
void k_gather_pieces(dst_ctx* c, const uint64_t* addr_dev, size_t count, void* dst);
int k_bench_mulmod(dst_ctx* c, uint64_t lanes, uint32_t iters, double* ms);
int k_bench_mad(dst_ctx* c, uint64_t lanes, uint32_t iters, double* ms);
int k_bench_clock(dst_ctx* c, uint64_t lanes, uint32_t iters, double* mhz);
int k_bench_code(dst_ctx* c, uint32_t code_kib, double* ms);
void k_upper_tree(dst_ctx* c, const digest* gathered, digest* upper, size_t nb, uint32_t G);
void k_digests_from_records(dst_ctx* c, const void* recs, size_t stride, digest* dst, size_t count);
void k_constraint_level1(dst_ctx* c);
void k_fri_leaves_cm(dst_ctx* c, const fe* e, digest* leaves, size_t nd);
void k_fri_fold_cm(dst_ctx* c, const fe* e, fe* out, size_t nd, int layer, fe special_x, const fe* alpha_dev = nullptr);
void k_fri_draw_at(dst_ctx* c, const digest* nodes, fe* alpha_out, digest* root_out);
void k_copy(dst_ctx* c, void* dst, const void* src, size_t bytes);
int k_field_op(dst_ctx* c, int op, const uint8_t* a, const uint8_t* b, uint8_t* out, size_t count);
int k_rescue_digests(hipStream_t stream, const fe* in , fe* out , size_t count, uint32_t* bad);
int k_rescue_tree(hipStream_t stream, fe* nodes , size_t leaves, uint32_t* bad);
int k_rescue_tree_update(hipStream_t stream, fe* nodes, uint32_t log_leaves, const uint32_t* lists , const size_t* off, const size_t* cnt);
int k_rescue_tree_scatter(hipStream_t stream, fe* nodes, const uint32_t* pos , const fe* vals , size_t count);
int k_rescue_tree_gather(hipStream_t stream, const fe* nodes, const uint32_t* pos , fe* out , size_t count);
int k_rescue_stree_level(hipStream_t stream, fe* nodes, const uint64_t* pref, const uint32_t* list, size_t count, size_t pstart, size_t cstart, size_t ccnt, const fe* empty);
int k_rescue_stree_carry(hipStream_t stream, fe* dst, const fe* src, const uint32_t* from , size_t count);
int k_rescue_stree_open(hipStream_t stream, const fe* nodes, const uint64_t* pref, const uint64_t* levels, const fe* empties, const uint64_t* indices, fe* out, size_t count, uint32_t depth);
```

### distaff_amd/csrc/host/steps.h

```cpp
#pragma once
#include <chrono>
#include <vector>
#include "../ctx.h"

namespace step {

inline double wall_ms() { return std::chrono::duration<double, std::milli>(std::chrono::steady_clock::now().time_since_epoch()).count(); }
inline double event_ms(hipEvent_t from, hipEvent_t to) {
    float ms = 0;
    if (from && to && hipEventElapsedTime(&ms, from, to) == hipSuccess) return (double)ms;
    (void)hipGetLastError();
    return -1.0;
}

struct ScratchTail {
    enum : size_t { ELEMS = 1024, MAX_W = 128, DRAWS = 344, MAX_TC = HS_DRAWS_BYTES / sizeof(fe) - DRAWS, COMPOSE = 516, TZ1 = 520, TZ2 = TZ1 + MAX_W, CZ = TZ2 + MAX_W };
    fe* base;
    explicit ScratchTail(const dst_ctx* c) : base(c->scratch + c->scratch_elems - ELEMS) {}
    fe* coef() const { return base; }
    fe* tc() const { return base + DRAWS; }
    fe* draws() const { return base; }
    fe* tz1() const { return base + TZ1; }
    fe* tz2() const { return base + TZ2; }
    fe* cz() const { return base + CZ; }
};
static_assert(ScratchTail::DRAWS + ScratchTail::MAX_TC <= ScratchTail::ELEMS && ScratchTail::COMPOSE <= ScratchTail::TZ1 && ScratchTail::CZ + 1 <= ScratchTail::ELEMS,
              "the scratch tail holds every phase's vectors for W <= 128 registers");

int eval_constraints(dst_ctx* c, const dst_public* pub, const uint8_t* coeffs, int64_t* bad_step, bool defer_check);
int boundary_polys(dst_ctx* c, const fe* draws344, fe* ip, fe* fp, fe* o0 = nullptr, fe* o1 = nullptr, fe* o2 = nullptr, fe* o3 = nullptr);
int boundary_quotients(dst_ctx* c, const fe* draws344, fe* q4, size_t stride);
int combine(dst_ctx* c, int parts);

void fri_file_root(dst_ctx* c, int d, const uint8_t root[32]);
inline size_t fri_nd(const dst_ctx* c, int d) { return c->fri_size[d] / c->B; }
inline fe* fri_layer_natural(const dst_ctx* c, int d) { return (d == 0 && c->fri_rep_from == 0) ? c->fri_nat0 : c->fri_e[d]; }
int fri_commit_natural(dst_ctx* c, int d0);
void fri_shard_layer(dst_ctx* c, int d);
void fri_shard_fold(dst_ctx* c, int d, fe x, const fe* alpha_dev = nullptr);

int query_seed(dst_ctx* c, uint64_t* nonce, std::vector<uint64_t>& positions);

}

int build_proof_local(dst_ctx* c, const uint64_t* positions, uint32_t num_positions, uint64_t pow_nonce, std::vector<uint8_t>& proof);
int ensure_shard_buffers(dst_ctx* c);
```

### distaff_amd/csrc/host/steps_impl.h

```cpp
#pragma once
#include "steps.h"
#include "../host_util.h"
#include "../host_vm.h"

static void transition_coefficients(const dst_ctx* c, const fe* draws344, std::vector<fe>& tc) {
    const size_t cl = c->prm.ctx_depth > 1 ? c->prm.ctx_depth : 1, ll = c->prm.loop_depth > 1 ? c->prm.loop_depth : 1;
    const size_t sl = c->stack_depth > 8 ? c->stack_depth : 8;
    std::vector<int> deg = {2, 2, 2, 2, 2, 2, 2, 2, 2, 2, 3, 8, 8, 6, 4, 6, 7, 6, 6, 4};
    deg.resize(20 + cl + ll, 4);
    deg.resize(20 + cl + ll + 2 + c->stack_depth, 7);
    const fe* t = draws344 + 188;
    std::vector<fe> cc;
    auto take = [&](size_t from, size_t cnt) { for (size_t i = 0; i < cnt; i++) cc.push_back(t[from + i]); };
    take(0, 40); take(40, 2 * cl); take(72, 2 * ll); take(88, 4); take(92, 2 * sl);
    const size_t nc = deg.size();
    tc.assign(2 * nc, fe_zero());
    size_t i = 0;
    for (int d = 0; d <= 8; d++)
        for (size_t k = 0; k < nc; k++)
            if (deg[k] == d) { tc[k] = cc[2 * i]; tc[nc + k] = cc[2 * i + 1]; i++; }
}

int step::eval_constraints(dst_ctx* c, const dst_public* pub, const uint8_t* coeffs, int64_t* bad_step, bool defer_check) {
    c->pub = *pub;
    c->air_draws.resize(344);
    memcpy(c->air_draws.data(), coeffs, 344 * sizeof(fe));
    c->ceval_inverted = false;
    std::vector<fe> tc;
    transition_coefficients(c, c->air_draws.data(), tc);
    if (tc.size() > ScratchTail::MAX_TC) { c->err = "too many transition coefficients for the staging area"; return DST_ERR_ARG; }
    const ScratchTail tail(c);
    fe* h = reinterpret_cast<fe*>(c->h_stage + HS_DRAWS);
    memcpy(h, c->air_draws.data(), 344 * sizeof(fe));
    memcpy(h + 344, tc.data(), tc.size() * sizeof(fe));
    HIP_TRY(c, hipMemcpyAsync(tail.coef(), h, 344 * sizeof(fe), hipMemcpyHostToDevice, c->stream));
    HIP_TRY(c, hipMemcpyAsync(tail.tc(), h + 344, tc.size() * sizeof(fe), hipMemcpyHostToDevice, c->stream));
    const int r = k_eval_constraints(c, tail.coef(), tail.tc(), bad_step, defer_check);
    if (r == DST_ERR_AIR) c->err = "transition constraints were not satisfied";
    return r;
}

int step::boundary_polys(dst_ctx* c, const fe* draws344, fe* ip, fe* fp, fe* o0, fe* o1, fe* o2, fe* o3) {
    const size_t n = c->n, D = 8 * n, W = c->W, p = 6 * n + 2;
    const uint32_t ctx_depth = c->prm.ctx_depth, loop_depth = c->prm.loop_depth;
    const size_t sd = c->stack_depth;
    const size_t cl = ctx_depth > 1 ? ctx_depth : 1, ll = loop_depth > 1 ? loop_depth : 1;
    std::vector<u128> w(4 * W, 0);
    u128 g[4] = {0, 0, 0, 0};
    const u128 one = 1;
    for (int pass = 0; pass < 2; pass++) {
        const fe* cc = draws344 + pass * 94;
        auto term = [&](int col, u128 constant, size_t idx) {
            for (int adj = 0; adj < 2; adj++) {
                const u128 k = fe_to_u128(cc[idx + adj]);
                if (col >= 0) w[(pass * 2 + adj) * W + col] = hf_add(w[(pass * 2 + adj) * W + col], k);
                if (constant != 0) g[pass * 2 + adj] = hf_add(g[pass * 2 + adj], hf_mul(k, constant));
            }
        };
        term(0, pass ? fe_to_u128(c->op_counter) : 0, 0);
        if (pass == 0) { for (int i = 0; i < 4; i++) term(1 + i, 0, 2 + 2 * i); }
        else { for (int i = 0; i < 2; i++) term(1 + i, fe_to_u128(c->program_hash[i]), 2 + 2 * i); }
        for (int i = 0; i < 3; i++) term(5 + i, pass ? one : 0, 10 + 2 * i);
        for (int i = 0; i < 5; i++) term(8 + i, pass ? one : 0, 16 + 2 * i);
        for (int i = 0; i < 2; i++) term(13 + i, pass ? one : 0, 26 + 2 * i);
        for (size_t i = 0; i < cl; i++) if (i < ctx_depth) term(15 + (int)i, 0, 30 + 2 * i);
        for (size_t i = 0; i < ll; i++) if (i < loop_depth) term(15 + (int)ctx_depth + (int)i, 0, 62 + 2 * i);
        const uint32_t nio = pass ? c->pub.num_outputs : c->pub.num_inputs;
        for (uint32_t i = 0; i < nio && i < 8; i++) {
            u128 v; memcpy(&v, pass ? c->pub.outputs[i] : c->pub.inputs[i], 16);
            term(i < sd ? 15 + (int)ctx_depth + (int)loop_depth + (int)i : -1, v, 78 + 2 * i);
        }
    }
    std::vector<fe> up(4 * W + 4);
    for (size_t i = 0; i < 4 * W; i++) up[i] = fe_from_u128(w[i]);
    for (int i = 0; i < 4; i++) up[4 * W + i] = fe_from_u128(g[i]);
    fe* d_w = (fe*)c->d_stage;
    fe* h_w = reinterpret_cast<fe*>(c->h_stage + HS_WEIGHTS);
    memcpy(h_w, up.data(), up.size() * sizeof(fe));
    HIP_TRY(c, hipMemcpyAsync(d_w, h_w, up.size() * sizeof(fe), hipMemcpyHostToDevice, c->stream));
    fe* outs[4] = {o0, o1, o2, o3};
    if (ip) {
        HIP_TRY(c, hipMemsetAsync(ip, 0, D * sizeof(fe), c->stream));
        HIP_TRY(c, hipMemsetAsync(fp, 0, D * sizeof(fe), c->stream));
        outs[0] = ip; outs[1] = ip + p; outs[2] = fp; outs[3] = fp + p;
    }
    k_lincomb4(c, c->polys, W, n, d_w, outs[0], outs[1], outs[2], outs[3]);
    for (int q = 0; q < 4; q++) k_sub_at0(c, outs[q], d_w + 4 * W + q);
    return DST_OK;
}

int step::boundary_quotients(dst_ctx* c, const fe* draws344, fe* q4, size_t stride) {
    const size_t n = c->n;
    HIP_TRY(c, hipMemsetAsync(q4, 0, 4 * stride * sizeof(fe), c->stream));
    int r = boundary_polys(c, draws344, nullptr, nullptr, q4 + 1, q4 + stride + 1, q4 + 2 * stride + 1, q4 + 3 * stride + 1);
    if (r) return r;
    fe* arrays[4] = {q4, q4 + stride, q4 + 2 * stride, q4 + 3 * stride};
    const fe divisors[4] = {fe_one(), fe_one(), c->x_last, c->x_last};
    k_syn_div_batch(c, arrays, divisors, 4, n + 1);
    return DST_OK;
}

int step::combine(dst_ctx* c, int parts) {
    const size_t n = c->n, D = 8 * n;
    fe* ip = c->cwork; fe* fp = c->cwork + D; fe* tp = c->cwork + 2 * D; fe* work = c->cwork + 3 * D;
    const bool steps = dst_internal_combine_by_steps(c);
    fe* q4 = c->cwork; const size_t qs = n + 16;
    const fe* draws = c->air_draws.data();
    if (parts & 1) {
        if (!steps) { if (int rb = boundary_quotients(c, draws, q4, qs)) return rb; }
        else {
            if (dst_internal_boundary_by_evaluation(c)) {
                k_intt8_cosets(c, c->ceval, ip, work);
                k_intt8_cosets(c, c->ceval + D, fp, work);
            } else if (int rb = boundary_polys(c, draws, ip, fp)) return rb;
            k_syn_div(c, ip, D, fe_one());
            k_syn_div(c, fp, D, c->x_last);
        }
    }
    if (parts & 2) {
        const bool inverted = c->ceval_inverted;
        c->ceval_inverted = false;
        if (!steps) {
            const fe* inv = c->ceval + 2 * D;
            if (!inverted) { k_intt_cosets_local(c, c->ceval + 2 * D, work, 8); inv = work; }
            k_combine_fused(c, inv, q4, qs, c->cpoly);
        } else {
            if (inverted) k_cross8(c, c->ceval + 2 * D, tp);
            else k_intt8_cosets(c, c->ceval + 2 * D, tp, work);
            k_syn_div_expanded(c, tp, c->cpoly, D, n, c->x_last);
            k_add(c, c->cpoly, ip, D);
            k_add(c, c->cpoly, fp, D);
        }
    }
    return DST_OK;
}

void step::fri_file_root(dst_ctx* c, int d, const uint8_t root[32]) {
    if (c->fri_roots.size() <= (size_t)d) c->fri_roots.resize(d + 1);
    c->fri_roots[d].assign(root, root + 32);
}

int step::fri_commit_natural(dst_ctx* c, int d0) {
    const int L = c->num_fri_layers;
    digest* d_roots = reinterpret_cast<digest*>(c->d_fri_chain);
    fe* d_alpha = reinterpret_cast<fe*>(c->d_fri_chain + DST_MAX_FRI_LAYERS * 32);
    uint8_t* h_roots = c->h_stage + HS_FRI_ROOTS;
    int d = d0;
    for (; d < L && !fri_tail_starts_at(c, d); d++) {
        const size_t R = c->fri_size[d] / 4;
        const bool coset_major = d == 0 && !c->sharded_layout;
        const fe* e = fri_layer_natural(c, d);
        if (coset_major) k_fri_leaves_layer0(c); else k_fri_leaves_at(c, e, c->fri_leaves[d], R);
        k_merkle(c, c->fri_leaves[d], c->fri_nodes[d], R, 0);
        k_fri_draw(c, d, d_alpha + d, d_roots + d);
        if (d + 1 == L) continue;
        if (coset_major) k_fri_fold_dev(c, 0, d_alpha); else k_fri_fold_at(c, e, c->fri_e[d + 1], R, d, fe_zero(), d_alpha + d);
    }
    if (d > d0) HIP_TRY(c, hipMemcpyAsync(h_roots, d_roots + d0, (size_t)(d - d0) * 32, hipMemcpyDeviceToHost, c->stream));
    if (d < L) {
        uint8_t tail_roots[DST_MAX_FRI_LAYERS * 32];
        if (int rt = k_fri_tail(c, d, tail_roots)) return rt;
        for (int i = d; i < L; i++) fri_file_root(c, i, tail_roots + 32 * (i - d));
    } else {
        CTX_SYNC(c, "the gathered FRI layer");
        HIP_TRY(c, hipGetLastError());
    }
    for (int i = d0; i < d; i++) fri_file_root(c, i, h_roots + 32 * (i - d0));
    c->fri_committed = L; c->fri_folded = L - 1;
    return DST_OK;
}

void step::fri_shard_layer(dst_ctx* c, int d) {
    const size_t nd = fri_nd(c, d), nb = nd / 4;
    k_fri_leaves_cm(c, c->fri_e[d], c->fri_leaves[d], nd);
    k_merkle(c, c->fri_leaves[d], c->fri_nodes[d], nb * c->Bc, nb);
    c->fri_committed = d + 1;
}
void step::fri_shard_fold(dst_ctx* c, int d, fe x, const fe* alpha_dev) {
    k_fri_fold_cm(c, c->fri_e[d], c->fri_e[d + 1], fri_nd(c, d), d, x, alpha_dev);
    c->fri_folded = d + 1;
}

int step::query_seed(dst_ctx* c, uint64_t* nonce, std::vector<uint64_t>& positions) {
    std::vector<uint8_t> roots;
    for (int d = 0; d < c->num_fri_layers; d++) roots.insert(roots.end(), c->fri_roots[d].begin(), c->fri_roots[d].end());
    uint8_t seed0[32], seed1[32];
    if (!blake3_short(roots.data(), roots.size(), seed0)) { c->err = "too many FRI roots"; return DST_ERR_ARG; }
    if (int r = dst_pow_grind(c, seed0, c->prm.grinding_factor, seed1, nonce)) return r;
    if (query_positions(seed1, c->N, (uint32_t)c->B, c->prm.num_queries, positions)) { c->err = "could not generate enough query positions"; return DST_ERR_ARG; }
    return DST_OK;
}
```

### distaff_amd/csrc/kernels_air.hip

```cpp
#include "air_kernel.h"
#include "rescue_constants.h"

#if DST_TEST_HOOKS
void air_launch_generic(dst_ctx* c, const AirArgs& a, uint32_t Q) {
    launch_air<16, 8, 0, 32, AS_OP_BITS, 0, AF_FIRST>(c, a, Q);
    launch_air_boundary<16, 8, 0, 32>(c, a, Q);
    launch_air<16, 8, 0, 32, AS_SPONGE | AS_FLOW, 0, 0>(c, a, Q);
    launch_air<16, 8, 0, 32, AS_STACK_MOVE, 0, 0>(c, a, Q);
    launch_air<16, 8, 0, 32, AS_STACK_ARITH, 0, 0>(c, a, Q);
    launch_air<16, 8, 0, 32, AS_STACK_HIGH, 0, 0>(c, a, Q);
    launch_air<16, 8, 0, 32, AS_STACK_RESCR, 0, AF_LAST>(c, a, Q);
}
#endif

enum AirInstanceSet { AIR_SET_SD4, AIR_SET_SMALL, AIR_SET_DEEP, AIR_SET_GENERIC };
static AirInstanceSet air_instance_set(uint32_t cl, uint32_t ll, uint32_t sd, const char* force) {
    const bool small_shape = cl <= 2 && ll <= 1 && sd <= 8;
    const auto forced = [&](const char* name) { return force && !strcmp(force, name); };
    if (forced("generic")) return DST_TEST_HOOKS ? AIR_SET_GENERIC : AIR_SET_DEEP;
    if (forced("deep") || !small_shape) return AIR_SET_DEEP;
    return sd == 4 && !forced("small") ? AIR_SET_SD4 : AIR_SET_SMALL;
}

int k_constraint_check(dst_ctx* c, int64_t* bad_step) {
    const unsigned long long res = c->air_flag_host;
    if (res != ~0ull) { if (bad_step) *bad_step = (int64_t)res; return DST_ERR_AIR; }
    if (bad_step) *bad_step = -1;
    return DST_OK;
}
int k_eval_constraints(dst_ctx* c, const fe* coeffs_dev, const fe* tc_dev, int64_t* bad_step, bool defer_check) {
    if (!c->air_consts) {
        AirConsts h;
        memcpy(h.sponge_mds, SPONGE_MDS, sizeof(h.sponge_mds)); memcpy(h.sponge_inv_mds, SPONGE_INV_MDS, sizeof(h.sponge_inv_mds));
        memcpy(h.hasher_mds, HASHER_MDS, sizeof(h.hasher_mds)); memcpy(h.hasher_inv_mds, HASHER_INV_MDS, sizeof(h.hasher_inv_mds));
        HIP_TRY(c, hipMalloc(&c->air_consts, sizeof(AirConsts)));
        HIP_TRY(c, hipMemcpy(c->air_consts, &h, sizeof(AirConsts), hipMemcpyHostToDevice));
    }
    AirArgs a{};
    a.lde = c->lde; a.out = c->ceval; a.coef = coeffs_dev; a.tc = tc_dev; a.periodic = c->periodic; a.consts = (const AirConsts*)c->air_consts; a.partial = c->cwork;
    {
        const size_t per = (size_t)(c->Bc / (c->B / 8)) * c->n;
        if (8 * per > c->Bc * c->tmp_regs * c->n) { c->err = "constraint evaluation: staging buffer too small for the stack partial values"; return DST_ERR_STATE; }
        for (int i = 0; i < 8; i++) a.ev[i] = c->tmp + (size_t)i * per;
        a.ev[8] = c->cpoly; a.ev[9] = c->comp_poly;
    }
    a.tw_lo = c->tw_lo; a.tw_hi = c->tw_hi; a.lo_bits = c->tw_lo_bits;
    a.bad_step = (unsigned long long*)c->d_u64;
    a.n = c->n; a.col_stride = c->Bc * c->n;
    a.log_n = c->log_n; a.log_N = c->log_N; a.log_b = c->log_b; a.W = (uint32_t)c->W;
    a.ctx_depth = c->prm.ctx_depth; a.loop_depth = c->prm.loop_depth; a.stack_depth = (uint32_t)c->stack_depth;
    a.coset_step = (uint32_t)(c->B / 8);
    a.q0 = (uint32_t)(c->j0 / (c->B / 8));
    uint32_t Q = (uint32_t)(c->Bc / (c->B / 8));
    a.num_inputs = c->pub.num_inputs; a.num_outputs = c->pub.num_outputs;
    memcpy(a.inputs, c->pub.inputs, sizeof(a.inputs)); memcpy(a.outputs, c->pub.outputs, sizeof(a.outputs));
    memcpy(a.program_hash, c->program_hash, sizeof(a.program_hash));
    a.op_count = c->op_counter;
    HIP_TRY(c, hipMemsetAsync(c->d_u64, 0xFF, 8, c->stream));
    const uint32_t cd = c->prm.ctx_depth, lp = c->prm.loop_depth, sd = (uint32_t)c->stack_depth;
    a.cl = cd > 1 ? cd : 1; a.ll = lp > 1 ? lp : 1; a.sl = sd > 8 ? sd : 8;
    switch (air_instance_set(a.cl, a.ll, sd, c->sw("DISTAFF_AIR"))) {
        case AIR_SET_SD4: air_launch_sd4(c, a, Q); break;
        case AIR_SET_SMALL: air_launch_small(c, a, Q); break;
        case AIR_SET_GENERIC:
#if DST_TEST_HOOKS
            air_launch_generic(c, a, Q); break;
#endif
        case AIR_SET_DEEP: air_launch_deep(c, a, Q); break;
    }
    unsigned long long* flag = c->h_stage ? reinterpret_cast<unsigned long long*>(c->h_stage + HS_AIR_FLAG) : &c->air_flag_host;
    HIP_TRY(c, hipMemcpyAsync(flag, c->d_u64, 8, hipMemcpyDeviceToHost, c->stream));
    if (defer_check && c->h_stage) return DST_OK;
    HIP_TRY(c, hipStreamSynchronize(c->stream));
    c->air_flag_host = *flag;
    return k_constraint_check(c, bad_step);
}
```

### distaff_amd/csrc/kernels_air_deep.hip

```cpp
#include "air_kernel.h"
void air_launch_deep(dst_ctx* c, const AirArgs& a, uint32_t Q) {
    launch_air_boundary<16, 8, 0, 12>(c, a, Q);
    launch_air<16, 8, 0, 12, AS_OP_BITS, 0, AF_FIRST>(c, a, Q);
    launch_air<16, 8, 0, 12, AS_SPONGE, 0, 0>(c, a, Q);
    launch_air<16, 8, 0, 12, AS_FLOW, 0, 0>(c, a, Q);
    launch_air<16, 8, 0, 12, 0, AG_DEEP, 0>(c, a, Q);
    launch_air<16, 8, 0, 12, 0, AG_RESCR, AF_EV_OUT>(c, a, Q);
    launch_air<16, 8, 0, 12, 0, AG_PUSH | AG_CMP | AG_KEEP, AF_EV_IN | AF_EV_OUT>(c, a, Q);
    launch_air<16, 8, 0, 12, 0, AG_LOW(0, 0) | AG_LOW(0, 2), AF_EV_IN | AF_EV_OUT>(c, a, Q);
    launch_air<16, 8, 0, 12, 0, AG_LOW(0, 1) | AG_LOW(0, 3), AF_EV_IN | AF_EV_OUT>(c, a, Q);
    launch_air<16, 8, 0, 12, 0, AG_LOW(1, 2) | AG_LOW(1, 3), AF_EV_IN | AF_EV_OUT>(c, a, Q);
    launch_air<16, 8, 0, 12, 0, AG_LOW(1, 0) | AG_LOW(1, 1), AF_EV_IN | AF_LAST>(c, a, Q);
}
```

### distaff_amd/csrc/kernels_air_sd4.hip

```cpp
#include "air_kernel.h"
void air_launch_sd4(dst_ctx* c, const AirArgs& a, uint32_t Q) {
    launch_air_boundary<2, 1, 4, 8>(c, a, Q);
    launch_air<2, 1, 4, 8, AS_OP_BITS | AS_FLOW, 0, AF_FIRST>(c, a, Q);
    launch_air<2, 1, 4, 8, AS_SPONGE, 0, 0>(c, a, Q);
    launch_air<2, 1, 4, 8, 0, AG_HIGH, AF_EV_OUT>(c, a, Q);
    launch_air<2, 1, 4, 8, 0, AG_LOW0, AF_EV_IN | AF_EV_OUT>(c, a, Q);
    launch_air<2, 1, 4, 8, 0, AG_LOW1, AF_EV_IN | AF_LAST>(c, a, Q);
}
```

### distaff_amd/csrc/kernels_air_small.hip

```cpp
#include "air_kernel.h"
void air_launch_small(dst_ctx* c, const AirArgs& a, uint32_t Q) {
    launch_air_boundary<2, 1, 0, 8>(c, a, Q);
    launch_air<2, 1, 0, 8, AS_OP_BITS | AS_FLOW, 0, AF_FIRST>(c, a, Q);
    launch_air<2, 1, 0, 8, AS_SPONGE, 0, 0>(c, a, Q);
    launch_air<2, 1, 0, 8, 0, AG_RESCR, AF_EV_OUT>(c, a, Q);
    launch_air<2, 1, 0, 8, 0, AG_PUSH | AG_CMP | AG_KEEP, AF_EV_IN | AF_EV_OUT>(c, a, Q);
    launch_air<2, 1, 0, 8, 0, AG_LOW(0, 0) | AG_LOW(0, 2), AF_EV_IN | AF_EV_OUT>(c, a, Q);
    launch_air<2, 1, 0, 8, 0, AG_LOW(0, 1) | AG_LOW(0, 3), AF_EV_IN | AF_EV_OUT>(c, a, Q);
    launch_air<2, 1, 0, 8, 0, AG_LOW(1, 2) | AG_LOW(1, 3), AF_EV_IN | AF_EV_OUT>(c, a, Q);
    launch_air<2, 1, 0, 8, 0, AG_LOW(1, 0) | AG_LOW(1, 1), AF_EV_IN | AF_LAST>(c, a, Q);
}
```

### distaff_amd/lib.py

```python
import ctypes
import os

import numpy as np

_HERE = os.path.dirname(os.path.abspath(__file__))
PRODUCT_LIB = os.path.join(_HERE, "libdistaff_hip.so")
HOOKS_LIB = os.path.join(_HERE, "libdistaff_hip_hooks.so")
LIB_PATH = os.environ.get("DISTAFF_HIP_LIB") or (HOOKS_LIB if os.environ.get("DISTAFF_TEST_HOOKS") == "1" else PRODUCT_LIB)


def use_test_hooks():
    global LIB_PATH
    if _lib is not None:
        raise RuntimeError("use_test_hooks() must be called before the library is loaded")
    os.environ["DISTAFF_TEST_HOOKS"] = "1"
    if not os.environ.get("DISTAFF_HIP_LIB"):
        LIB_PATH = HOOKS_LIB


def use_product():
    global LIB_PATH
    if _lib is not None:
        raise RuntimeError("use_product() must be called before the library is loaded")
    os.environ.pop("DISTAFF_TEST_HOOKS", None)
    if not os.environ.get("DISTAFF_HIP_LIB"):
        LIB_PATH = PRODUCT_LIB


def library_path():
    return LIB_PATH

DST_OK, DST_ERR_ARG, DST_ERR_HIP, DST_ERR_AIR, DST_ERR_STATE, DST_ERR_COMM = 0, -1, -2, -3, -4, -5

BUF = {"polys": 0, "lde": 1, "trace_leaves": 2, "trace_nodes": 3, "ceval_i": 4, "ceval_f": 5, "ceval_t": 6, "cpoly": 7, "cevals": 8,
       "cnodes": 9, "comp_poly": 10, "comp_evals": 11, "fri_evals": 12, "fri_nodes": 13, "fri_leaves": 14}

EXPORTS = ["dst_ctx_create", "dst_ctx_destroy", "dst_last_error", "dst_phase_ms", "dst_trace_upload", "dst_trace_upload_contiguous", "dst_trace_upload_owned",
           "dst_commit_trace", "dst_eval_constraints", "dst_compose", "dst_fri_commit_layer", "dst_fri_fold", "dst_pow_grind",
           "dst_build_proof", "dst_prove", "dst_prng_vector", "dst_query_positions", "dst_blake3", "dst_fibonacci_trace",
           "dst_read_buffer", "dst_bench_mulmod", "dst_bench_mad", "dst_bench_code", "dst_trace_upload_async", "dst_pinned_alloc", "dst_pinned_free", "dst_set_profiling", "dst_kernel_stats", "dst_field_op",
           "dst_shard_commit_trace", "dst_shard_eval_constraints", "dst_shard_combine", "dst_shard_fri_layer", "dst_shard_fri_fold",
           "dst_shard_export_size", "dst_shard_export", "dst_shard_import", "dst_shard_read", "dst_shard_fri_begin", "dst_shard_fri_end", "dst_shard_fri_roots", "dst_shard_open", "dst_shard_assemble", "dst_shard_info",
           "dst_comm_unique_id", "dst_comm_init", "dst_comm_init_local", "dst_comm_init_callbacks", "dst_comm_destroy", "dst_comm_last_error", "dst_comm_copy", "dst_prove_sharded", "dst_prove_sharded_local", "dst_shard_stage_ms",
           "dst_comm_describe", "dst_comm_trace", "dst_test_hooks", "dst_comm_set_timeout", "dst_comm_abort", "dst_shard_exchange_ms", "dst_bench_clock",
           "dst_verify", "dst_proof_info",
           "dst_rescue_digest_many", "dst_rtree_build", "dst_rtree_root", "dst_rtree_path", "dst_rtree_tapes", "dst_rtree_read_nodes", "dst_rtree_build_ms",
           "dst_rtree_destroy", "dst_rtree_last_error", "dst_rtree_update", "dst_rtree_update_ms", "dst_rtree_paths", "dst_rtree_tapes_many",
           "dst_stree_create", "dst_stree_set", "dst_stree_root", "dst_stree_paths", "dst_stree_tapes_many", "dst_stree_read_level", "dst_stree_info",
           "dst_stree_destroy", "dst_stree_last_error"]


class DistaffError(RuntimeError):
    def __init__(self, code, message):
        super().__init__("libdistaff_hip error %d: %s" % (code, message))
        self.code = code
        self.reason = message


class Params(ctypes.Structure):
    _fields_ = [("log_trace_length", ctypes.c_uint32), ("log_blowup", ctypes.c_uint32), ("width", ctypes.c_uint32),
                ("ctx_depth", ctypes.c_uint32), ("loop_depth", ctypes.c_uint32), ("num_queries", ctypes.c_uint32),
                ("grinding_factor", ctypes.c_uint32), ("device", ctypes.c_int32), ("rank", ctypes.c_uint32), ("world", ctypes.c_uint32)]


class Public(ctypes.Structure):
    _fields_ = [("num_inputs", ctypes.c_uint32), ("num_outputs", ctypes.c_uint32),
                ("inputs", (ctypes.c_uint8 * 16) * 8), ("outputs", (ctypes.c_uint8 * 16) * 8)]


class CommInfo(ctypes.Structure):
    _fields_ = [("transport", ctypes.c_uint32), ("rank", ctypes.c_uint32), ("world", ctypes.c_uint32), ("device", ctypes.c_int32),
                ("rccl_ranks", ctypes.c_uint32), ("rccl_rank", ctypes.c_uint32), ("rccl_version", ctypes.c_uint32),
                ("peers_other_device", ctypes.c_uint32), ("peers_enabled", ctypes.c_uint32)]


class ProofInfo(ctypes.Structure):
    _fields_ = [(f, ctypes.c_uint32) for f in ("log_trace_length", "extension_factor", "num_queries", "grinding_factor", "register_count", "ctx_depth", "loop_depth",
                                               "stack_depth", "op_count", "fri_layers", "remainder_length", "security_level", "security_level_proven")] + [("pow_nonce", ctypes.c_uint64)]


_lib = None


def _share_hip_runtime_with_torch():
    if os.environ.get("DISTAFF_HIP_RUNTIME", "torch") != "torch":
        return
    try:
        import importlib.util
        spec = importlib.util.find_spec("torch")
        if spec is None or not spec.submodule_search_locations:
            return
        cand = os.path.join(list(spec.submodule_search_locations)[0], "lib", "libamdhip64.so")
        if os.path.exists(cand):
            ctypes.CDLL(cand, mode=ctypes.RTLD_GLOBAL)
    except OSError:
        pass


def _open(path):
    if not os.path.exists(path):
        raise ImportError("%s is missing: the HIP extension must be built (python -c 'import __graft_entry__ as g; g.build()'), there is no CPU fallback" % path)
    _share_hip_runtime_with_torch()
    lib = ctypes.CDLL(path)
    lib.dst_last_error.restype = ctypes.c_char_p
    lib.dst_last_error.argtypes = [ctypes.c_void_p]
    return lib


def load():
    global _lib
    if _lib is None:
        _lib = _open(LIB_PATH)
    return _lib


_hooks_lib = None


def load_hooks():
    global _hooks_lib
    if _hooks_lib is None:
        bound = load()
        has = getattr(bound, "dst_test_hooks", None)
        _hooks_lib = bound if (has is not None and has() == 1) else _open(HOOKS_LIB)
    return _hooks_lib


def ntt_describe(log_n, log_blowup, inverse, lde, cosets, cols, skip=0, lib=None):
    buf = ctypes.create_string_buffer(4096)
    r = (lib or load_hooks()).dst_ntt_describe(ctypes.c_uint32(log_n), ctypes.c_uint32(log_blowup), ctypes.c_int(int(inverse)), ctypes.c_int(int(lde)),
                                               ctypes.c_uint32(cosets), ctypes.c_uint32(cols), ctypes.c_uint32(skip), buf, ctypes.c_size_t(len(buf)))
    if r != DST_OK:
        raise DistaffError(r, "dst_ntt_describe(%d, %d) failed" % (log_n, log_blowup))
    return buf.value.decode().splitlines()


def _ptr(a):
    return a.ctypes.data_as(ctypes.c_void_p)


def int_to_bytes(v):
    return int(v).to_bytes(16, "little")


def ints_to_arr(values):
    out = np.empty((len(values), 2), dtype=np.uint64)
    for i, v in enumerate(values):
        out[i, 0] = int(v) & 0xFFFFFFFFFFFFFFFF
        out[i, 1] = int(v) >> 64
    return out


def arr_to_ints(a):
    a = np.asarray(a, dtype=np.uint64).reshape(-1, 2)
    return [int(lo) | (int(hi) << 64) for lo, hi in a]


def make_public(inputs, outputs):
    p = Public()
    p.num_inputs, p.num_outputs = len(inputs), len(outputs)
    for i, v in enumerate(inputs):
        p.inputs[i][:] = list(int_to_bytes(v))
    for i, v in enumerate(outputs):
        p.outputs[i][:] = list(int_to_bytes(v))
    return p


def prng_vector(seed, count):
    out = np.zeros((count, 2), dtype=np.uint64)
    load().dst_prng_vector(bytes(seed), ctypes.c_uint32(count), _ptr(out))
    return out


def query_positions(seed, domain_size, blowup, num_queries):
    out = np.zeros(num_queries, dtype=np.uint64)
    k = load().dst_query_positions(bytes(seed), ctypes.c_uint64(domain_size), ctypes.c_uint32(blowup), ctypes.c_uint32(num_queries), _ptr(out))
    if k < 0:
        raise DistaffError(k, "could not generate enough query positions")
    return [int(x) for x in out[:k]]


def blake3(data):
    out = ctypes.create_string_buffer(32)
    load().dst_blake3(bytes(data), ctypes.c_size_t(len(data)), out)
    return out.raw


def verify(proof, program_hash, inputs, outputs, lib=None):
    proof, program_hash = bytes(proof), bytes(program_hash)
    if len(program_hash) != 32:
        raise DistaffError(DST_ERR_ARG, "program_hash must be 32 bytes")
    if len(inputs) > 8 or len(outputs) > 8:
        raise DistaffError(DST_ERR_ARG, "at most 8 public inputs and 8 outputs")
    pub = make_public(inputs, outputs)
    accepted = ctypes.c_int(0)
    err = ctypes.create_string_buffer(512)
    r = (lib or load()).dst_verify(program_hash, ctypes.byref(pub), proof, ctypes.c_size_t(len(proof)), ctypes.byref(accepted), err, ctypes.c_size_t(512))
    if r != DST_OK:
        raise DistaffError(r, err.value.decode())
    return accepted.value == 1, err.value.decode()


def proof_info(proof, lib=None):
    proof = bytes(proof)
    info = ProofInfo()
    r = (lib or load()).dst_proof_info(proof, ctypes.c_size_t(len(proof)), ctypes.byref(info))
    if r != DST_OK:
        raise DistaffError(r, "not a StarkProof")
    return {f: int(getattr(info, f)) for f, _ in ProofInfo._fields_}


def fibonacci_trace(log_n):
    n = 1 << log_n
    cols = np.zeros((20, n, 2), dtype=np.uint64)
    ph = ctypes.create_string_buffer(32)
    res = ctypes.create_string_buffer(16)
    r = load().dst_fibonacci_trace(ctypes.c_uint32(log_n), _ptr(cols), ph, res)
    if r != DST_OK:
        raise DistaffError(r, "dst_fibonacci_trace failed")
    return cols, ph.raw, int.from_bytes(res.raw, "little")


def _elements(values, per_item):
    if isinstance(values, np.ndarray) and values.dtype == np.uint64:
        a = np.ascontiguousarray(values)
    else:
        rows = [tuple(v) for v in values]
        if any(len(r) != per_item for r in rows):
            raise DistaffError(DST_ERR_ARG, "every item must have %d elements" % per_item)
        a = ints_to_arr([x for r in rows for x in r])
    if a.size % (2 * per_item):
        raise DistaffError(DST_ERR_ARG, "expected [count, %d, 2] uint64 words" % per_item)
    return a.reshape(-1, per_item, 2)


def _rtree_error(lib, handle=None):
    lib.dst_rtree_last_error.restype = ctypes.c_char_p
    lib.dst_rtree_last_error.argtypes = [ctypes.c_void_p]
    return (lib.dst_rtree_last_error(handle) or b"").decode()


def rescue_digest(values, device=0, lib=None):
    lib = lib or load()
    a = _elements(values, 4)
    out = np.zeros((a.shape[0], 2, 2), dtype=np.uint64)
    r = lib.dst_rescue_digest_many(ctypes.c_int(device), _ptr(a), ctypes.c_size_t(a.shape[0]), _ptr(out))
    if r != DST_OK:
        raise DistaffError(r, _rtree_error(lib) or "dst_rescue_digest_many failed")
    return out


class RescueTree:

    def __init__(self, leaves, device=0, lib=None):
        self.lib = lib or load()
        a = _elements(leaves, 2)
        n = a.shape[0]
        if n < 2 or n & (n - 1):
            raise DistaffError(DST_ERR_ARG, "the number of leaves must be a power of two >= 2")
        self.log_leaves = n.bit_length() - 1
        h = ctypes.c_void_p()
        r = self.lib.dst_rtree_build(ctypes.c_int(device), _ptr(a), ctypes.c_uint32(self.log_leaves), ctypes.byref(h))
        if r != DST_OK:
            raise DistaffError(r, _rtree_error(self.lib))
        self._h = h

    def _check(self, r):
        if r != DST_OK:
            raise DistaffError(r, _rtree_error(self.lib, self._h))

    def close(self):
        if getattr(self, "_h", None):
            self.lib.dst_rtree_destroy.restype = None
            self.lib.dst_rtree_destroy(self._h)
            self._h = None

    def __del__(self):
        self.close()

    @property
    def root(self):
        out = np.zeros((2, 2), dtype=np.uint64)
        self._check(self.lib.dst_rtree_root(self._h, _ptr(out)))
        return tuple(arr_to_ints(out))

    @property
    def build_ms(self):
        ms = ctypes.c_double(0)
        self._check(self.lib.dst_rtree_build_ms(self._h, ctypes.byref(ms)))
        return ms.value

    def path(self, index):
        out = np.zeros((self.log_leaves + 1, 2, 2), dtype=np.uint64)
        self._check(self.lib.dst_rtree_path(self._h, ctypes.c_uint64(index), _ptr(out)))
        v = arr_to_ints(out)
        return [(v[2 * k], v[2 * k + 1]) for k in range(self.log_leaves + 1)]

    def tapes(self, index, what=3):
        n = ctypes.c_size_t(0)
        self._check(self.lib.dst_rtree_tapes(self._h, ctypes.c_uint64(index), ctypes.c_uint32(what), None, None, ctypes.c_size_t(0), ctypes.byref(n)))
        a = np.zeros((max(n.value, 1), 2), dtype=np.uint64)
        b = np.zeros((max(n.value, 1), 2), dtype=np.uint64)
        self._check(self.lib.dst_rtree_tapes(self._h, ctypes.c_uint64(index), ctypes.c_uint32(what), _ptr(a), _ptr(b), ctypes.c_size_t(n.value), ctypes.byref(n)))
        return arr_to_ints(a[:n.value]), arr_to_ints(b[:n.value])

    @staticmethod
    def _indices(indices):
        idx = np.ascontiguousarray(np.array([int(i) for i in indices], dtype=np.uint64))
        return idx, (_ptr(idx) if idx.size else None)

    def update(self, indices, leaves):
        idx, ip = self._indices(indices)
        a = _elements(leaves, 2)
        if a.shape[0] != idx.size:
            raise DistaffError(DST_ERR_ARG, "as many leaves as indices")
        self._check(self.lib.dst_rtree_update(self._h, ip, _ptr(a) if idx.size else None, ctypes.c_size_t(idx.size)))

    @property
    def update_ms(self):
        ms = ctypes.c_double(0)
        self._check(self.lib.dst_rtree_update_ms(self._h, ctypes.byref(ms)))
        return ms.value

    def paths(self, indices):
        idx, ip = self._indices(indices)
        n = self.log_leaves + 1
        out = np.zeros((max(idx.size, 1) * n, 2, 2), dtype=np.uint64)
        self._check(self.lib.dst_rtree_paths(self._h, ip, ctypes.c_size_t(idx.size), _ptr(out)))
        v = arr_to_ints(out[:idx.size * n])
        return [[(v[2 * (i * n + k)], v[2 * (i * n + k) + 1]) for k in range(n)] for i in range(idx.size)]

    def tapes_many(self, indices, what=3):
        idx, ip = self._indices(indices)
        n = ctypes.c_size_t(0)
        self._check(self.lib.dst_rtree_tapes_many(self._h, ip, ctypes.c_size_t(idx.size), ctypes.c_uint32(what), None, None, ctypes.c_size_t(0), ctypes.byref(n)))
        each = n.value
        a = np.zeros((max(idx.size * each, 1), 2), dtype=np.uint64)
        b = np.zeros((max(idx.size * each, 1), 2), dtype=np.uint64)
        self._check(self.lib.dst_rtree_tapes_many(self._h, ip, ctypes.c_size_t(idx.size), ctypes.c_uint32(what), _ptr(a), _ptr(b), ctypes.c_size_t(each), ctypes.byref(n)))
        va, vb = arr_to_ints(a[:idx.size * each]), arr_to_ints(b[:idx.size * each])
        return [(va[i * each:(i + 1) * each], vb[i * each:(i + 1) * each]) for i in range(idx.size)]

    def nodes(self, first, count):
        out = np.zeros((count, 2, 2), dtype=np.uint64)
        self._check(self.lib.dst_rtree_read_nodes(self._h, ctypes.c_uint64(first), ctypes.c_uint64(count), _ptr(out)))
        return out

class StreeInfo(ctypes.Structure):
    _fields_ = [("depth", ctypes.c_uint32), ("device", ctypes.c_int32), ("keys", ctypes.c_uint64), ("nodes", ctypes.c_uint64),
                ("last_digests", ctypes.c_uint64), ("last_device_ms", ctypes.c_double)]


class SparseRescueTree:

    def __init__(self, depth, empty_leaf=(0, 0), device=0, lib=None):
        self.lib = lib or load()
        self.depth = int(depth)
        e = _elements([tuple(empty_leaf)], 2)
        h = ctypes.c_void_p()
        r = self.lib.dst_stree_create(ctypes.c_int(device), ctypes.c_uint32(self.depth), _ptr(e), ctypes.byref(h))
        if r != DST_OK:
            raise DistaffError(r, self._error(None))
        self._h = h

    def _error(self, handle):
        self.lib.dst_stree_last_error.restype = ctypes.c_char_p
        self.lib.dst_stree_last_error.argtypes = [ctypes.c_void_p]
        return (self.lib.dst_stree_last_error(handle) or b"").decode()

    def _check(self, r):
        if r != DST_OK:
            raise DistaffError(r, self._error(self._h))

    def close(self):
        if getattr(self, "_h", None):
            self.lib.dst_stree_destroy.restype = None
            self.lib.dst_stree_destroy(self._h)
            self._h = None

    def __del__(self):
        self.close()

    def set(self, indices, leaves):
        idx, ip = RescueTree._indices(indices)
        a = _elements(leaves, 2)
        if a.shape[0] != idx.size:
            raise DistaffError(DST_ERR_ARG, "as many leaves as indices")
        self._check(self.lib.dst_stree_set(self._h, ip, _ptr(a) if idx.size else None, ctypes.c_size_t(idx.size)))

    @property
    def root(self):
        out = np.zeros((2, 2), dtype=np.uint64)
        self._check(self.lib.dst_stree_root(self._h, _ptr(out)))
        return tuple(arr_to_ints(out))

    def paths_words(self, indices):
        idx, ip = RescueTree._indices(indices)
        n = self.depth + 1
        out = np.zeros((idx.size, n, 2, 2), dtype=np.uint64)
        self._check(self.lib.dst_stree_paths(self._h, ip, ctypes.c_size_t(idx.size), _ptr(out) if idx.size else None))
        return out

    def paths(self, indices):
        n = self.depth + 1
        w = self.paths_words(indices)
        v = arr_to_ints(w)
        return [[(v[2 * (i * n + k)], v[2 * (i * n + k) + 1]) for k in range(n)] for i in range(w.shape[0])]

    def path(self, index):
        return self.paths([index])[0]

    def tapes_many(self, indices, what=3):
        idx, ip = RescueTree._indices(indices)
        n = ctypes.c_size_t(0)
        self._check(self.lib.dst_stree_tapes_many(self._h, ip, ctypes.c_size_t(idx.size), ctypes.c_uint32(what), None, None, ctypes.c_size_t(0), ctypes.byref(n)))
        each = n.value
        a = np.zeros((max(idx.size * each, 1), 2), dtype=np.uint64)
        b = np.zeros((max(idx.size * each, 1), 2), dtype=np.uint64)
        self._check(self.lib.dst_stree_tapes_many(self._h, ip, ctypes.c_size_t(idx.size), ctypes.c_uint32(what), _ptr(a), _ptr(b), ctypes.c_size_t(each), ctypes.byref(n)))
        va, vb = arr_to_ints(a[:idx.size * each]), arr_to_ints(b[:idx.size * each])
        return [(va[i * each:(i + 1) * each], vb[i * each:(i + 1) * each]) for i in range(idx.size)]

    def tapes(self, index, what=3):
        return self.tapes_many([index], what)[0]

    def level(self, l):
        m = ctypes.c_uint64(0)
        self._check(self.lib.dst_stree_read_level(self._h, ctypes.c_uint32(l), ctypes.c_uint64(0), ctypes.c_uint64(0), None, None, ctypes.byref(m)))
        prefixes = np.zeros(m.value, dtype=np.uint64)
        nodes = np.zeros((m.value, 2, 2), dtype=np.uint64)
        if m.value:
            self._check(self.lib.dst_stree_read_level(self._h, ctypes.c_uint32(l), ctypes.c_uint64(0), ctypes.c_uint64(m.value), _ptr(prefixes), _ptr(nodes), ctypes.byref(m)))
        return prefixes, nodes

    def info(self):
        i = StreeInfo()
        self._check(self.lib.dst_stree_info(self._h, ctypes.byref(i)))
        return {f: getattr(i, f) for f, _ in StreeInfo._fields_}


class Comm:

    def __init__(self, handle):
        self.lib, self._h = load(), handle

    def describe(self):
        info = CommInfo()
        if self.lib.dst_comm_describe(self._h, ctypes.byref(info)) != DST_OK:
            raise DistaffError(DST_ERR_ARG, "dst_comm_describe failed")
        d = {f: int(getattr(info, f)) for f, _ in CommInfo._fields_}
        d["transport"] = ("rccl", "local", "callbacks")[d["transport"]]
        return d

    def set_timeout(self, seconds):
        if self.lib.dst_comm_set_timeout(self._h, ctypes.c_double(seconds)) != DST_OK:
            raise DistaffError(DST_ERR_ARG, "dst_comm_set_timeout failed")

    def abort(self):
        self.lib.dst_comm_abort(self._h)

    def last_error(self):
        self.lib.dst_comm_last_error.restype = ctypes.c_char_p
        self.lib.dst_comm_last_error.argtypes = [ctypes.c_void_p]
        return self.lib.dst_comm_last_error(self._h).decode()

    def trace(self, enable=-1):
        n = ctypes.c_size_t(0)
        self.lib.dst_comm_trace(self._h, ctypes.c_int(-1), None, ctypes.c_size_t(0), ctypes.byref(n))
        buf = ctypes.create_string_buffer(n.value + 1)
        if self.lib.dst_comm_trace(self._h, ctypes.c_int(enable), buf, ctypes.c_size_t(n.value + 1), ctypes.byref(n)) != DST_OK:
            raise DistaffError(DST_ERR_ARG, "dst_comm_trace failed")
        out = []
        for line in buf.value.decode().splitlines():
            k, b, st = line.split()
            out.append((k, int(b), None if st == "-" else int(st)))
        return out

    @staticmethod
    def unique_id():
        lib = load()
        buf = ctypes.create_string_buffer(128)
        if lib.dst_comm_unique_id(buf) != DST_OK:
            lib.dst_comm_last_error.restype = ctypes.c_char_p
            raise DistaffError(DST_ERR_HIP, lib.dst_comm_last_error(None).decode())
        return buf.raw

    @classmethod
    def rccl(cls, unique_id, rank, world, device):
        lib = load()
        h = ctypes.c_void_p()
        if lib.dst_comm_init(bytes(unique_id), ctypes.c_uint32(rank), ctypes.c_uint32(world), ctypes.c_int(device), ctypes.byref(h)) != DST_OK:
            lib.dst_comm_last_error.restype = ctypes.c_char_p
            raise DistaffError(DST_ERR_HIP, lib.dst_comm_last_error(None).decode())
        return cls(h)

    @classmethod
    def local(cls, world):
        lib = load()
        arr = (ctypes.c_void_p * world)()
        if lib.dst_comm_init_local(ctypes.c_uint32(world), arr) != DST_OK:
            raise DistaffError(DST_ERR_ARG, "dst_comm_init_local failed")
        return [cls(ctypes.c_void_p(arr[r])) for r in range(world)]

    @classmethod
    def callbacks(cls, rank, world, fn):
        lib = load()
        proto = ctypes.CFUNCTYPE(ctypes.c_int, ctypes.c_void_p, ctypes.c_int, ctypes.c_void_p, ctypes.c_void_p, ctypes.c_size_t)

        def tramp(user, kind, send, recv, nbytes):
            try:
                return int(fn(kind, send, recv, nbytes))
            except Exception:
                import traceback
                traceback.print_exc()
                return 1
        cb = proto(tramp)
        h = ctypes.c_void_p()
        if lib.dst_comm_init_callbacks(ctypes.c_uint32(rank), ctypes.c_uint32(world), cb, None, ctypes.byref(h)) != DST_OK:
            raise DistaffError(DST_ERR_ARG, "dst_comm_init_callbacks failed")
        c = cls(h)
        c._keep = cb
        return c

    @classmethod
    def over_torch(cls, dist, group=None):
        import numpy as np
        import torch
        lib = load()
        lib.dst_comm_copy.argtypes = [ctypes.c_void_p, ctypes.c_void_p, ctypes.c_size_t]
        rank, world = dist.get_rank(group), dist.get_world_size(group)
        on_device = str(dist.get_backend(group)).lower() == "nccl"

        def copy(dst, src, nbytes):
            if lib.dst_comm_copy(ctypes.c_void_p(dst), ctypes.c_void_p(src), ctypes.c_size_t(nbytes)) != DST_OK:
                lib.dst_comm_last_error.restype = ctypes.c_char_p
                raise DistaffError(DST_ERR_HIP, lib.dst_comm_last_error(None).decode())

        def staged(src, nbytes):
            t = torch.empty(nbytes, dtype=torch.uint8, device="cuda" if on_device else "cpu")
            copy(t.data_ptr(), src, nbytes)
            return t

        def fn(kind, send, recv, nbytes):
            if nbytes == 0:
                return 0
            if kind == 1:
                mine = staged(send, nbytes * world)
                out = torch.empty_like(mine)
                if on_device:
                    dist.all_to_all_single(out, mine, group=group)
                    torch.cuda.synchronize()
                else:
                    every = [torch.empty_like(mine) for _ in range(world)]
                    dist.all_gather(every, mine, group=group)
                    out = torch.cat([e[rank * nbytes:(rank + 1) * nbytes] for e in every])
                copy(recv, out.data_ptr(), nbytes * world)
                return 0
            if kind == 2 and not on_device:
                mine = torch.from_numpy(np.ctypeslib.as_array((ctypes.c_uint8 * nbytes).from_address(send)).copy())
            else:
                mine = staged(send, nbytes)
            if on_device:
                out = torch.empty(nbytes * world, dtype=torch.uint8, device="cuda")
                dist.all_gather_into_tensor(out, mine, group=group)
                torch.cuda.synchronize()
            else:
                every = [torch.empty_like(mine) for _ in range(world)]
                dist.all_gather(every, mine, group=group)
                out = torch.cat(every)
            if kind == 2 and not on_device:
                ctypes.memmove(recv, out.data_ptr(), nbytes * world)
            else:
                copy(recv, out.data_ptr(), nbytes * world)
            return 0
        return cls.callbacks(rank, world, fn)

    def close(self):
        if getattr(self, "_h", None):
            self.lib.dst_comm_destroy(self._h)
            self._h = None


class Calibration:

    def __init__(self, device=0):
        self.ctx = Context(10, 20, 1, 0, device=device, lib=load_hooks())
        if not self.ctx.lib.dst_test_hooks():
            raise RuntimeError("the calibration kernels need the test / bench build (libdistaff_hip_hooks.so)")

    def bench_mad(self, lanes=1 << 21, iters=2048):
        return self.ctx.bench_mad(lanes, iters)

    def bench_mulmod(self, lanes=1 << 20, iters=256, portable=False):
        return self.ctx.bench_mulmod(lanes, iters, portable)

    def bench_code(self, code_kib):
        return self.ctx.bench_code(code_kib)

    def bench_clock(self, lanes=1 << 20, iters=1024):
        mhz = ctypes.c_double(0)
        self.ctx._check(self.ctx.lib.dst_bench_clock(self.ctx._h, ctypes.c_uint64(lanes), ctypes.c_uint32(iters), ctypes.byref(mhz)))
        return mhz.value

    def close(self):
        self.ctx.close()


def prove_sharded_local(contexts, inputs, outputs, cap=1 << 22):
    lib = load()
    world = len(contexts)
    arr = (ctypes.c_void_p * world)(*[c._h.value for c in contexts])
    pub = make_public(inputs, outputs)
    buf = ctypes.create_string_buffer(cap)
    ln = ctypes.c_size_t(0)
    r = lib.dst_prove_sharded_local(arr, ctypes.c_uint32(world), ctypes.byref(pub), buf, ctypes.c_size_t(cap), ctypes.byref(ln))
    if r != DST_OK:
        msgs = [lib.dst_last_error(c._h).decode() for c in contexts]
        raise DistaffError(r, "; ".join("rank %d: %s" % (i, m) for i, m in enumerate(msgs) if m))
    return buf.raw[:ln.value]


class Context:

    def __init__(self, log_n, width, ctx_depth, loop_depth, log_blowup=5, num_queries=50, grinding=20, device=0, rank=0, world=1, lib=None):
        self.lib = lib or load()
        self.params = Params(log_n, log_blowup, width, ctx_depth, loop_depth, num_queries, grinding, device, rank, world)
        self.n, self.B, self.W = 1 << log_n, 1 << log_blowup, width
        self.N = self.n * self.B
        h = ctypes.c_void_p()
        r = self.lib.dst_ctx_create(ctypes.byref(self.params), ctypes.byref(h))
        if r != DST_OK:
            raise DistaffError(r, self.lib.dst_last_error(None).decode())
        self._h = h

    def close(self):
        if getattr(self, "_h", None):
            self.lib.dst_ctx_destroy(self._h)
            self._h = None

    def __del__(self):
        self.close()

    def _check(self, r):
        if r != DST_OK:
            raise DistaffError(r, self.lib.dst_last_error(self._h).decode())

    def upload(self, columns):
        cols = np.ascontiguousarray(columns, dtype=np.uint64)
        assert cols.shape == (self.W, self.n, 2), cols.shape
        self._check(self.lib.dst_trace_upload_contiguous(self._h, _ptr(cols)))

    def pinned_trace(self, columns):
        cols = np.ascontiguousarray(columns, dtype=np.uint64)
        assert cols.shape == (self.W, self.n, 2), cols.shape
        p = ctypes.c_void_p()
        if self.lib.dst_pinned_alloc(ctypes.c_size_t(cols.nbytes), ctypes.byref(p)) != DST_OK:
            raise DistaffError(DST_ERR_HIP, "dst_pinned_alloc failed")
        ctypes.memmove(p, cols.ctypes.data, cols.nbytes)
        table = (ctypes.c_void_p * self.W)(*[p.value + i * self.n * 16 for i in range(self.W)])
        return table, p

    def release_pinned(self, handle):
        self.lib.dst_pinned_free(handle)

    def upload_owned(self, cols):
        cols = np.ascontiguousarray(cols, dtype=np.uint64)
        rank, world = self.params.rank, self.params.world
        ptrs = (ctypes.c_void_p * self.W)(*[cols[i].ctypes.data if i % world == rank else None for i in range(self.W)])
        self._check(self.lib.dst_trace_upload_owned(self._h, ptrs))

    def upload_async(self, table):
        self._check(self.lib.dst_trace_upload_async(self._h, table))

    def prove_sharded(self, comm, inputs, outputs, cap=1 << 22):
        pub = make_public(inputs, outputs)
        buf = ctypes.create_string_buffer(cap)
        ln = ctypes.c_size_t(0)
        self._check(self.lib.dst_prove_sharded(self._h, comm._h, ctypes.byref(pub), buf, ctypes.c_size_t(cap), ctypes.byref(ln)))
        return buf.raw[:ln.value]

    def shard_stage_ms(self):
        v = (ctypes.c_double * 3)()
        self._check(self.lib.dst_shard_stage_ms(self._h, v))
        return {"transport_calls": v[0], "root_waits": v[1], "tree_exchanges": int(v[2])}

    def shard_exchange_ms(self):
        v = (ctypes.c_double * 8)()
        self._check(self.lib.dst_shard_exchange_ms(self._h, v))
        return {"coefficients": v[0], "tree_all_to_all": v[1], "tree_all_gather": v[2], "constraint_evaluations": v[3], "fri_tail": v[4],
                "host_values": v[5], "collectives": int(v[6]), "timed_by_events": int(v[7])}

    def commit_trace(self):
        root = ctypes.create_string_buffer(32)
        self._check(self.lib.dst_commit_trace(self._h, root))
        return root.raw

    def eval_constraints(self, inputs, outputs, coeffs):
        c = np.ascontiguousarray(coeffs, dtype=np.uint64)
        assert c.shape == (344, 2)
        root = ctypes.create_string_buffer(32)
        bad = ctypes.c_int64(-1)
        pub = make_public(inputs, outputs)
        r = self.lib.dst_eval_constraints(self._h, ctypes.byref(pub), _ptr(c), root, ctypes.byref(bad))
        self.bad_step = bad.value
        self._check(r)
        return root.raw

    def compose(self, draws):
        d = np.ascontiguousarray(draws, dtype=np.uint64)
        assert d.shape == (516, 2)
        z1 = np.zeros((self.W, 2), dtype=np.uint64)
        z2 = np.zeros((self.W, 2), dtype=np.uint64)
        self._check(self.lib.dst_compose(self._h, _ptr(d), _ptr(z1), _ptr(z2)))
        return z1, z2

    def fri_commit_layer(self):
        root = ctypes.create_string_buffer(32)
        more = ctypes.c_int(0)
        self._check(self.lib.dst_fri_commit_layer(self._h, root, ctypes.byref(more)))
        return root.raw, bool(more.value)

    def fri_fold(self, special_x):
        self._check(self.lib.dst_fri_fold(self._h, int_to_bytes(special_x)))

    def pow_grind(self, seed, grinding):
        out = ctypes.create_string_buffer(32)
        nonce = ctypes.c_uint64(0)
        self._check(self.lib.dst_pow_grind(self._h, bytes(seed), ctypes.c_uint32(grinding), out, ctypes.byref(nonce)))
        return out.raw, nonce.value

    def build_proof(self, positions, pow_nonce):
        pos = np.asarray(positions, dtype=np.uint64)
        ln = ctypes.c_size_t(0)
        self._check(self.lib.dst_build_proof(self._h, _ptr(pos), ctypes.c_uint32(len(positions)), ctypes.c_uint64(pow_nonce), None, ctypes.c_size_t(0), ctypes.byref(ln)))
        buf = ctypes.create_string_buffer(ln.value)
        self._check(self.lib.dst_build_proof(self._h, _ptr(pos), ctypes.c_uint32(len(positions)), ctypes.c_uint64(pow_nonce), buf, ctypes.c_size_t(ln.value), ctypes.byref(ln)))
        return buf.raw[:ln.value]

    def prove(self, inputs, outputs, cap=1 << 22):
        pub = make_public(inputs, outputs)
        buf = ctypes.create_string_buffer(cap)
        ln = ctypes.c_size_t(0)
        self._check(self.lib.dst_prove(self._h, ctypes.byref(pub), buf, ctypes.c_size_t(cap), ctypes.byref(ln)))
        return buf.raw[:ln.value]

    def phase_ms(self):
        ms = (ctypes.c_double * 9)()
        self._check(self.lib.dst_phase_ms(self._h, ms))
        return list(ms)

    def read(self, what, arg=0):
        ln = ctypes.c_size_t(0)
        self._check(self.lib.dst_read_buffer(self._h, ctypes.c_uint32(BUF[what]), ctypes.c_uint32(arg), None, ctypes.c_size_t(0), ctypes.byref(ln)))
        buf = np.zeros(ln.value, dtype=np.uint8)
        self._check(self.lib.dst_read_buffer(self._h, ctypes.c_uint32(BUF[what]), ctypes.c_uint32(arg), _ptr(buf), ctypes.c_size_t(ln.value), ctypes.byref(ln)))
        return buf

    def read_elements(self, what, arg=0):
        return self.read(what, arg).view(np.uint64).reshape(-1, 2)

    def shard_commit_trace(self):
        self._check(self.lib.dst_shard_commit_trace(self._h))

    def shard_eval_constraints(self, inputs, outputs, coeffs):
        c = np.ascontiguousarray(coeffs, dtype=np.uint64)
        bad = ctypes.c_int64(-1)
        pub = make_public(inputs, outputs)
        r = self.lib.dst_shard_eval_constraints(self._h, ctypes.byref(pub), _ptr(c), ctypes.byref(bad))
        if r == DST_ERR_AIR:
            return bad.value
        self._check(r)
        return -1

    def shard_combine(self):
        self._check(self.lib.dst_shard_combine(self._h))

    def shard_fri_layer(self):
        more = ctypes.c_int(0)
        self._check(self.lib.dst_shard_fri_layer(self._h, ctypes.byref(more)))
        return bool(more.value)

    def fri_fold_shard(self, special_x):
        self._check(self.lib.dst_shard_fri_fold(self._h, int_to_bytes(special_x)))

    def shard_export_size(self, what, arg=0):
        n = ctypes.c_size_t(0)
        self._check(self.lib.dst_shard_export_size(self._h, ctypes.c_uint32(what), ctypes.c_uint32(arg), ctypes.byref(n)))
        return n.value

    def shard_export(self, what, arg, dst_ptr, is_device):
        self._check(self.lib.dst_shard_export(self._h, ctypes.c_uint32(what), ctypes.c_uint32(arg), ctypes.c_void_p(dst_ptr), int(is_device)))

    def shard_import(self, what, arg, src_ptr, is_device):
        root = ctypes.create_string_buffer(32)
        self._check(self.lib.dst_shard_import(self._h, ctypes.c_uint32(what), ctypes.c_uint32(arg), ctypes.c_void_p(src_ptr), int(is_device), root))
        return root.raw

    def shard_read(self, buffer, arg, indices):
        idx = np.asarray(indices, dtype=np.uint64)
        item = self.W * 16 if buffer == 10 else (16 if buffer in (3, 6, 11) else 32)
        out = np.zeros(len(indices) * item, dtype=np.uint8)
        self._check(self.lib.dst_shard_read(self._h, ctypes.c_uint32(buffer), ctypes.c_uint32(arg), _ptr(idx), ctypes.c_uint32(len(indices)), _ptr(out)))
        return out.tobytes()

    def shard_fri_begin(self, send_ptr, is_device, cap):
        n, more = ctypes.c_size_t(0), ctypes.c_int(0)
        self._check(self.lib.dst_shard_fri_begin(self._h, ctypes.c_void_p(send_ptr), ctypes.c_int(1 if is_device else 0), ctypes.c_size_t(cap),
                                                 ctypes.byref(n), ctypes.byref(more)))
        return n.value, bool(more.value)

    def shard_fri_end(self, gathered_ptr, is_device):
        root = ctypes.create_string_buffer(32)
        self._check(self.lib.dst_shard_fri_end(self._h, ctypes.c_void_p(gathered_ptr), ctypes.c_int(1 if is_device else 0), root))
        return root.raw

    def shard_fri_roots(self):
        layers, rep = ctypes.c_uint32(0), ctypes.c_uint32(0)
        self._check(self.lib.dst_shard_fri_roots(self._h, None, ctypes.c_size_t(0), ctypes.byref(layers), ctypes.byref(rep)))
        buf = ctypes.create_string_buffer(32 * layers.value)
        self._check(self.lib.dst_shard_fri_roots(self._h, buf, ctypes.c_size_t(32 * layers.value), ctypes.byref(layers), ctypes.byref(rep)))
        return [buf.raw[32 * d:32 * d + 32] for d in range(layers.value)], rep.value

    def shard_open(self, positions):
        pos = np.ascontiguousarray(positions, dtype=np.uint64)
        ln = ctypes.c_size_t(0)
        lens = np.zeros(self.params.world, dtype=np.uint64)
        self._check(self.lib.dst_shard_open(self._h, _ptr(pos), ctypes.c_uint32(len(pos)), None, ctypes.c_size_t(0), ctypes.byref(ln), _ptr(lens)))
        blob = np.zeros(max(ln.value, 1), dtype=np.uint8)
        self._check(self.lib.dst_shard_open(self._h, _ptr(pos), ctypes.c_uint32(len(pos)), _ptr(blob), ctypes.c_size_t(ln.value), ctypes.byref(ln), None))
        return blob[:ln.value], [int(v) for v in lens]

    def shard_assemble(self, positions, nonce, blobs, lens):
        pos = np.ascontiguousarray(positions, dtype=np.uint64)
        bl = np.ascontiguousarray(blobs, dtype=np.uint8)
        ls = np.ascontiguousarray(lens, dtype=np.uint64)
        ln = ctypes.c_size_t(0)
        args = (self._h, _ptr(pos), ctypes.c_uint32(len(pos)), ctypes.c_uint64(nonce), _ptr(bl), _ptr(ls))
        self._check(self.lib.dst_shard_assemble(*args, None, ctypes.c_size_t(0), ctypes.byref(ln)))
        out = np.zeros(ln.value, dtype=np.uint8)
        self._check(self.lib.dst_shard_assemble(*args, _ptr(out), ctypes.c_size_t(ln.value), ctypes.byref(ln)))
        return out.tobytes()

    def shard_info(self):
        op = ctypes.c_uint64(0); layers = ctypes.c_uint32(0); sd = ctypes.c_uint32(0)
        self._check(self.lib.dst_shard_info(self._h, ctypes.byref(op), ctypes.byref(layers), ctypes.byref(sd)))
        return op.value, layers.value, sd.value

    def set_profiling(self, level=1):
        self._check(self.lib.dst_set_profiling(self._h, int(level)))

    def kernel_stats(self, reset=True):
        import json
        buf = ctypes.create_string_buffer(1 << 16)
        self._check(self.lib.dst_kernel_stats(self._h, buf, ctypes.c_size_t(1 << 16), int(reset)))
        return json.loads(buf.value.decode())

    def field_op(self, op, a, b):
        ops = {"add": 0, "sub": 1, "mul": 2, "mul_portable": 3, "inv": 4, "pow": 5, "dot40": 6, "mul_tw": 7, "shift64": 8, "addsub_sum": 9, "addsub_dif": 10,
               "mul_small": 11, "sqr": 12, "cube": 13}
        ops.update({"dot%d" % t: 256 + t for t in range(1, 65) if t != 40})
        a = np.ascontiguousarray(a, dtype=np.uint64); b = np.ascontiguousarray(b, dtype=np.uint64)
        out = np.zeros_like(a)
        self._check(self.lib.dst_field_op(self._h, ops[op], _ptr(a), _ptr(b), _ptr(out), ctypes.c_size_t(a.shape[0])))
        return out

    def bench_mad(self, lanes=1 << 21, iters=2048):
        ms = ctypes.c_double(0)
        self._check(self.lib.dst_bench_mad(self._h, ctypes.c_uint64(lanes), ctypes.c_uint32(iters), ctypes.byref(ms)))
        return ms.value

    def bench_code(self, code_kib):
        ms = ctypes.c_double(0)
        self._check(self.lib.dst_bench_code(self._h, ctypes.c_uint32(code_kib), ctypes.byref(ms)))
        return ms.value

    def bench_mulmod(self, lanes=1 << 20, iters=256, portable=False):
        ms = ctypes.c_double(0)
        self._check(self.lib.dst_bench_mulmod(self._h, ctypes.c_uint64(lanes), ctypes.c_uint32(iters | (0x80000000 if portable else 0)), ctypes.byref(ms)))
        return ms.value
```

### include/distaff_hip.h

```cpp
#ifndef DISTAFF_HIP_H
#define DISTAFF_HIP_H
#include <stddef.h>
#include <stdint.h>

#if defined(__GNUC__)
#define DST_API __attribute__((visibility("default")))
#else
#define DST_API
#endif

#ifdef __cplusplus
extern "C" {
#endif

#define DST_OK 0
#define DST_ERR_ARG (-1)
#define DST_ERR_HIP (-2)
#define DST_ERR_AIR (-3)
#define DST_ERR_STATE (-4)
#define DST_ERR_COMM (-5)

typedef struct dst_ctx dst_ctx;

typedef struct dst_params {
    uint32_t log_trace_length;
    uint32_t log_blowup;
    uint32_t width;
    uint32_t ctx_depth;
    uint32_t loop_depth;
    uint32_t num_queries;
    uint32_t grinding_factor;
    int32_t  device;
    uint32_t rank, world;
} dst_params;

typedef struct dst_public {
    uint32_t num_inputs, num_outputs;
    uint8_t inputs[8][16];
    uint8_t outputs[8][16];
} dst_public;

DST_API int dst_ctx_create(const dst_params* params, dst_ctx** out);
DST_API void dst_ctx_destroy(dst_ctx* ctx);
DST_API const char* dst_last_error(const dst_ctx* ctx);
DST_API int dst_phase_ms(const dst_ctx* ctx, double out_ms[9]);

DST_API int dst_trace_upload(dst_ctx* ctx, const uint8_t* const* cols);
DST_API int dst_trace_upload_contiguous(dst_ctx* ctx, const uint8_t* cols);
DST_API int dst_trace_upload_owned(dst_ctx* ctx, const uint8_t* const* cols);
DST_API int dst_trace_upload_async(dst_ctx* ctx, const uint8_t* const* cols);
DST_API int dst_pinned_alloc(size_t bytes, void** out);
DST_API int dst_pinned_free(void* p);

DST_API int dst_commit_trace(dst_ctx* ctx, uint8_t trace_root[32]);

DST_API int dst_eval_constraints(dst_ctx* ctx, const dst_public* pub, const uint8_t* coeffs , uint8_t constraint_root[32], int64_t* bad_step);

DST_API int dst_compose(dst_ctx* ctx, const uint8_t* draws , uint8_t* trace_at_z1 , uint8_t* trace_at_z2 );

DST_API int dst_fri_commit_layer(dst_ctx* ctx, uint8_t layer_root[32], int* more);
DST_API int dst_fri_fold(dst_ctx* ctx, const uint8_t special_x[16]);

DST_API int dst_pow_grind(dst_ctx* ctx, const uint8_t seed[32], uint32_t grinding_factor, uint8_t out_seed[32], uint64_t* nonce);

DST_API int dst_build_proof(dst_ctx* ctx, const uint64_t* positions, uint32_t num_positions, uint64_t pow_nonce,
                    uint8_t* out, size_t cap, size_t* out_len);

DST_API int dst_prove(dst_ctx* ctx, const dst_public* pub, uint8_t* proof_out, size_t cap, size_t* proof_len);

DST_API int dst_verify(const uint8_t program_hash[32], const dst_public* pub, const uint8_t* proof, size_t len,
                       int* accepted, char* err, size_t err_cap);
typedef struct dst_proof_info_t {
    uint32_t log_trace_length;
    uint32_t extension_factor, num_queries, grinding_factor;
    uint32_t register_count;
    uint32_t ctx_depth, loop_depth, stack_depth;
    uint32_t op_count;
    uint32_t fri_layers, remainder_length;
    uint32_t security_level;
    uint32_t security_level_proven;
    uint64_t pow_nonce;
} dst_proof_info_t;
DST_API int dst_proof_info(const uint8_t* proof, size_t len, dst_proof_info_t* out);

DST_API int dst_rescue_digest_many(int device, const uint8_t* in , size_t count, uint8_t* out );
typedef struct dst_rtree dst_rtree;
DST_API int dst_rtree_build(int device, const uint8_t* leaves, uint32_t log_leaves, dst_rtree** out);
DST_API int dst_rtree_root(const dst_rtree* t, uint8_t root[32]);
DST_API int dst_rtree_path(const dst_rtree* t, uint64_t index, uint8_t* path );
DST_API int dst_rtree_tapes(const dst_rtree* t, uint64_t index, uint32_t what, uint8_t* tape_a, uint8_t* tape_b, size_t cap_elems, size_t* elems);
DST_API int dst_rtree_read_nodes(const dst_rtree* t, uint64_t first, uint64_t count, uint8_t* out);
DST_API int dst_rtree_build_ms(const dst_rtree* t, double* device_ms);
DST_API int dst_rtree_update(dst_rtree* t, const uint64_t* indices, const uint8_t* leaves, size_t count);
DST_API int dst_rtree_update_ms(const dst_rtree* t, double* device_ms);
DST_API int dst_rtree_paths(const dst_rtree* t, const uint64_t* indices, size_t count, uint8_t* paths);
DST_API int dst_rtree_tapes_many(const dst_rtree* t, const uint64_t* indices, size_t count, uint32_t what,
                                 uint8_t* tape_a, uint8_t* tape_b, size_t cap_elems_each, size_t* elems_each);
DST_API void dst_rtree_destroy(dst_rtree* t);
DST_API const char* dst_rtree_last_error(const dst_rtree* t);

typedef struct dst_stree dst_stree;
DST_API int dst_stree_create(int device, uint32_t depth, const uint8_t empty_leaf[32] , dst_stree** out);
DST_API int dst_stree_set(dst_stree* t, const uint64_t* indices, const uint8_t* leaves , size_t count);
DST_API int dst_stree_root(const dst_stree* t, uint8_t root[32]);
DST_API int dst_stree_paths(const dst_stree* t, const uint64_t* indices, size_t count, uint8_t* paths );
DST_API int dst_stree_tapes_many(const dst_stree* t, const uint64_t* indices, size_t count, uint32_t what,
                                 uint8_t* tape_a, uint8_t* tape_b, size_t cap_elems_each, size_t* elems_each);
DST_API int dst_stree_read_level(const dst_stree* t, uint32_t level, uint64_t first, uint64_t count,
                                 uint64_t* prefixes, uint8_t* nodes , uint64_t* level_count);
typedef struct dst_stree_info_t {
    uint32_t depth;
    int32_t device;
    uint64_t keys, nodes;
    uint64_t last_digests;
    double last_device_ms;
} dst_stree_info_t;
DST_API int dst_stree_info(const dst_stree* t, dst_stree_info_t* out);
DST_API void dst_stree_destroy(dst_stree* t);
DST_API const char* dst_stree_last_error(const dst_stree* t);

DST_API void dst_prng_vector(const uint8_t seed[32], uint32_t count, uint8_t* out );
DST_API int dst_query_positions(const uint8_t seed[32], uint64_t domain_size, uint32_t blowup, uint32_t num_queries, uint64_t* out);
DST_API void dst_blake3(const uint8_t* in, size_t len, uint8_t out[32]);

DST_API int dst_fibonacci_trace(uint32_t log_n, uint8_t* cols, uint8_t program_hash[32], uint8_t result[16]);

DST_API int dst_shard_commit_trace(dst_ctx* ctx);
DST_API int dst_shard_eval_constraints(dst_ctx* ctx, const dst_public* pub, const uint8_t* coeffs , int64_t* bad_step);
DST_API int dst_shard_combine(dst_ctx* ctx);
DST_API int dst_shard_fri_layer(dst_ctx* ctx, int* more);
DST_API int dst_shard_fri_fold(dst_ctx* ctx, const uint8_t special_x[16]);
DST_API int dst_shard_export_size(dst_ctx* ctx, uint32_t what, uint32_t arg, size_t* bytes);
DST_API int dst_shard_export(dst_ctx* ctx, uint32_t what, uint32_t arg, void* dst, int dst_is_device);
DST_API int dst_shard_import(dst_ctx* ctx, uint32_t what, uint32_t arg, const void* src, int src_is_device, uint8_t root_out[32]);
DST_API int dst_shard_read(dst_ctx* ctx, uint32_t buffer, uint32_t arg, const uint64_t* idx, uint32_t count, uint8_t* out);
DST_API int dst_shard_fri_begin(dst_ctx* ctx, void* send, int send_is_device, size_t cap, size_t* bytes, int* more);
DST_API int dst_shard_fri_end(dst_ctx* ctx, const void* gathered, int src_is_device, uint8_t root_out[32]);
DST_API int dst_shard_fri_roots(dst_ctx* ctx, uint8_t* roots , size_t cap, uint32_t* num_layers, uint32_t* replicated_from);

DST_API int dst_shard_open(dst_ctx* ctx, const uint64_t* positions, uint32_t num_positions, uint8_t* blob, size_t cap, size_t* blob_len, uint64_t* all_lens);
DST_API int dst_shard_assemble(dst_ctx* ctx, const uint64_t* positions, uint32_t num_positions, uint64_t pow_nonce, const uint8_t* blobs,
                       const uint64_t* blob_lens, uint8_t* out, size_t cap, size_t* out_len);
DST_API int dst_shard_info(dst_ctx* ctx, uint64_t* op_count, uint32_t* num_fri_layers, uint32_t* stack_depth);

DST_API int dst_read_buffer(dst_ctx* ctx, uint32_t what, uint32_t arg, uint8_t* out, size_t cap, size_t* len);
DST_API int dst_test_hooks(void);
DST_API int dst_bench_mulmod(dst_ctx* ctx, uint64_t lanes, uint32_t iters, double* ms);
DST_API int dst_bench_mad(dst_ctx* ctx, uint64_t lanes, uint32_t iters, double* ms);
DST_API int dst_bench_clock(dst_ctx* ctx, uint64_t lanes, uint32_t iters, double* mhz);
DST_API int dst_bench_code(dst_ctx* ctx, uint32_t code_kib, double* ms);
DST_API int dst_field_op(dst_ctx* ctx, int op, const uint8_t* a, const uint8_t* b, uint8_t* out, size_t count);
DST_API int dst_set_profiling(dst_ctx* ctx, int level);
DST_API int dst_kernel_stats(dst_ctx* ctx, char* json_out, size_t cap, int reset);

typedef struct dst_comm dst_comm;
DST_API int dst_comm_unique_id(uint8_t id[128]);
DST_API int dst_comm_init(const uint8_t id[128], uint32_t rank, uint32_t world, int device, dst_comm** out);
DST_API int dst_comm_init_local(uint32_t world, dst_comm** out );
typedef int (*dst_comm_fn)(void* user, int kind, const void* send, void* recv, size_t bytes);
DST_API int dst_comm_init_callbacks(uint32_t rank, uint32_t world, dst_comm_fn fn, void* user, dst_comm** out);
DST_API void dst_comm_destroy(dst_comm* comm);
DST_API int dst_comm_set_timeout(dst_comm* comm, double seconds);
DST_API int dst_comm_abort(dst_comm* comm);
enum { DST_COMM_RCCL = 0, DST_COMM_LOCAL = 1, DST_COMM_CALLBACKS = 2 };
typedef struct dst_comm_info {
    uint32_t transport, rank, world;
    int32_t device;
    uint32_t rccl_ranks, rccl_rank, rccl_version;
    uint32_t peers_other_device, peers_enabled;
} dst_comm_info;
DST_API int dst_comm_describe(const dst_comm* comm, dst_comm_info* out);
DST_API int dst_comm_trace(dst_comm* comm, int enable, char* out, size_t cap, size_t* len);
DST_API int dst_comm_copy(void* dst, const void* src, size_t bytes);
DST_API const char* dst_comm_last_error(const dst_comm* comm);
DST_API int dst_prove_sharded(dst_ctx* ctx, dst_comm* comm, const dst_public* pub, uint8_t* proof, size_t cap, size_t* len);
DST_API int dst_shard_stage_ms(const dst_ctx* ctx, double out[3]);
DST_API int dst_shard_exchange_ms(const dst_ctx* ctx, double out[8]);
DST_API int dst_prove_sharded_local(dst_ctx** ctxs, uint32_t world, const dst_public* pub, uint8_t* proof, size_t cap, size_t* len);

#ifdef __cplusplus
}
#endif
#endif
```

Measured before the change: 622.1 million.

## Move trace-row constraint check to a low-priority side stream overlapped with FRI

The transition-constraint check on the trace rows (coset 0) is pulled out of the main evaluation kernels into a separate check-kernel chain. By default it is queued on a low-priority side stream after FRI commitment and drained at the end of proving, so it overlaps with proof-of-work and openings instead of sitting on the critical path. The main evaluation kernels now skip all constraint work for on-trace rows and just write zeros there. The cost is an extra launch chain, an extra partials buffer, and a constraint failure that is only reported at the end of dst_prove.

```diff
diff --git a/distaff_amd/csrc/air_kernel.h b/distaff_amd/csrc/air_kernel.h
--- a/distaff_amd/csrc/air_kernel.h
+++ b/distaff_amd/csrc/air_kernel.h
@@ -448,6 +448,10 @@
     air_load_rows<ST.sl>(rows, o, nw, a, cols, sd);
     if constexpr ((SECT & AS_BOUNDARY) != 0) air_boundary<CL, LL>(a, rows, o, cl, ll, gi, n64, nmask, ql, k);
     if constexpr (SECT == AS_BOUNDARY) return;
+    if (qg == 0 && k + 1 != a.n) {
+        if constexpr (LAST) a.out[((size_t)2 * gridDim.y + ql) * a.n + k] = fe_zero();
+        return;
+    }
     AirFlags flags;
     air_op_flags(flags, rows);
     const fe* per = a.periodic + (size_t)(step & 127u) * AIR_PERIODIC_STRIDE;
@@ -470,8 +474,6 @@
 
     constexpr bool EMITS_STACK = (SECT & AS_STACK_ANY) != 0 || (GROUPS & AG_DEEP) != 0 || ((GROUPS & AG_STACK_ALL) != 0 && !EV_OUT);
     constexpr uint32_t USED = ((SECT & AS_OP_BITS) ? 0x2Fu : 0u) | ((SECT & AS_SPONGE) ? 0x18u : 0u) | ((SECT & AS_FLOW) ? 0x04u : 0u) | (EMITS_STACK ? 0x10u : 0u);
-    const bool on_trace = (qg == 0);
-    if (on_trace && k + 1 != a.n && acc.nonzero) atomicMin(a.bad_step, (unsigned long long)k);
     acc.res = fe_acc_reduce(acc.res_acc);
 #pragma unroll
     for (int i = 0; i < 6; i++) if (((ACC_MASK & USED) >> i) & 1u) acc.adj[i] = fe_add(acc.adj[i], fe_acc_reduce(acc.adj_acc[i]));
@@ -489,6 +491,51 @@
     air_combine(acc.res, acc.adj, a, k, ql, qg, gi, n64, nmask);
 }
 
+struct AirCheckAcc {
+    bool nonzero;
+    __device__ __forceinline__ void emit(uint32_t, int, const fe& d) { nonzero |= !fe_is_zero(d); }
+};
+
+template <int CL, int LL, int SD, int SLCAP, int SECT, uint32_t GROUPS, int FLAGS>
+__global__ void __launch_bounds__(AIR_THREADS, AIR_WAVES_PER_SIMD) air_check_kernel(AirArgs a) {
+    constexpr AirStack ST = air_stack(SD, SLCAP);
+    constexpr bool EV_IN = (FLAGS & AF_EV_IN) != 0, EV_OUT = (FLAGS & AF_EV_OUT) != 0;
+    static_assert(ST.nested ? (SECT & AS_STACK_ANY) == 0 : (GROUPS == 0 && !EV_IN && !EV_OUT),
+                  "nested-sum instances select stack operations with GROUPS, the per-operation instance with SECT");
+    static_assert((SECT & AS_BOUNDARY) == 0, "the boundary combinations are no part of the check");
+    const int cl = (int)a.cl, ll = (int)a.ll;
+    const int sl = SD ? ST.sl : (int)a.sl;
+    const int sd = SD ? SD : (int)a.stack_depth;
+    const size_t k = (size_t)blockIdx.x * AIR_THREADS + threadIdx.x;
+    if (k + 1 >= a.n) return;
+    const AirColumns cols{a.lde + k, a.lde + k + 1, a.col_stride};
+
+    AirRows<CL, LL> rows;
+    fe o[ST.sl], nw[ST.sl];
+    air_load_rows<ST.sl>(rows, o, nw, a, cols, sd);
+    AirFlags flags;
+    air_op_flags(flags, rows);
+    const fe* per = a.periodic + (size_t)(((uint32_t)k << 3) & 127u) * AIR_PERIODIC_STRIDE;
+
+    AirCheckAcc acc; acc.nonzero = false;
+    if constexpr ((SECT & AS_OP_BITS) != 0) air_op_bits(acc, rows, flags, per);
+    if constexpr ((SECT & AS_SPONGE) != 0) air_sponge<SD == 0>(acc, a, cols, rows, nw, flags, per);
+    if constexpr ((SECT & AS_FLOW) != 0) air_flow<CL, LL>(acc, a, cols, rows, flags, cl, ll);
+    if constexpr (ST.nested && (GROUPS & AG_STACK_ALL & ~AG_DEEP) != 0) air_stack_nested<SD, ST.deep, ST.slots, ST.sl, GROUPS, EV_IN, EV_OUT>(acc, a, rows, o, nw, flags, per, cl, ll, sl, sd, k);
+    if constexpr (!ST.nested && (SECT & AS_STACK_ANY) != 0) air_stack_per_operation<ST.sl, SECT>(acc, o, nw, sl, sd, 20 + cl + ll, flags, per, a.consts);
+    if constexpr (ST.deep && (GROUPS & AG_DEEP) != 0) air_stack_deep_slots(acc, a, cols, flags, cl, ll, sl, sd);
+    if (acc.nonzero) atomicMin(a.bad_step, (unsigned long long)k);
+}
+
+template <int CL, int LL, int SD, int SLCAP, int SECT, uint32_t GROUPS, int FLAGS>
+static void launch_air_check(dst_ctx* c, const AirArgs& a, hipStream_t stream) {
+    dim3 g((unsigned)((c->n + AIR_THREADS - 1) / AIR_THREADS), 1);
+    static char name[64];
+    if (!name[0]) snprintf(name, sizeof(name), "air_check<%d,%d,%d,%d,%d,%u,%d>", CL, LL, SD, SLCAP, SECT, (unsigned)GROUPS, FLAGS);
+    constexpr int NS = air_stack(SD, SLCAP).partials;
+    const double units = c->W + ((FLAGS & AF_EV_IN) ? NS : 0) + ((FLAGS & AF_EV_OUT) ? NS : 0);
+    { KScope ks_(c, name, 16.0 * c->n * units, true, 0.0, stream); hipLaunchKernelGGL((air_check_kernel<CL, LL, SD, SLCAP, SECT, GROUPS, FLAGS>), g, dim3(AIR_THREADS), 0, stream, a); }
+}
 
 template <int CL, int LL, int SD, int SLCAP, int SECT, uint32_t GROUPS, int FLAGS>
 static void launch_air(dst_ctx* c, const AirArgs& a, uint32_t Q) {
@@ -505,7 +552,20 @@
     if (dst_internal_boundary_by_evaluation(c)) launch_air<CL, LL, SD, SLCAP, AS_BOUNDARY, 0, 0>(c, a, Q);
 #endif
 }
+struct AirEvalChain {
+    dst_ctx* c; const AirArgs& a; uint32_t Q;
+    template <int CL, int LL, int SD, int SLCAP, int SECT, uint32_t GROUPS, int FLAGS> void run() const { launch_air<CL, LL, SD, SLCAP, SECT, GROUPS, FLAGS>(c, a, Q); }
+    template <int CL, int LL, int SD, int SLCAP> void boundary() const { launch_air_boundary<CL, LL, SD, SLCAP>(c, a, Q); }
+};
+struct AirCheckChain {
+    dst_ctx* c; const AirArgs& a; hipStream_t stream;
+    template <int CL, int LL, int SD, int SLCAP, int SECT, uint32_t GROUPS, int FLAGS> void run() const { launch_air_check<CL, LL, SD, SLCAP, SECT, GROUPS, FLAGS>(c, a, stream); }
+    template <int CL, int LL, int SD, int SLCAP> void boundary() const {}
+};
 void air_launch_sd4(dst_ctx* c, const AirArgs& a, uint32_t Q);
 void air_launch_small(dst_ctx* c, const AirArgs& a, uint32_t Q);
 void air_launch_deep(dst_ctx* c, const AirArgs& a, uint32_t Q);
 void air_launch_generic(dst_ctx* c, const AirArgs& a, uint32_t Q);
+void air_check_sd4(dst_ctx* c, const AirArgs& a, hipStream_t stream);
+void air_check_small(dst_ctx* c, const AirArgs& a, hipStream_t stream);
+void air_check_deep(dst_ctx* c, const AirArgs& a, hipStream_t stream);
diff --git a/distaff_amd/csrc/api.hip b/distaff_amd/csrc/api.hip
--- a/distaff_amd/csrc/api.hip
+++ b/distaff_amd/csrc/api.hip
@@ -59,6 +59,9 @@
         if (c->fri_leaves[d]) hipFree(c->fri_leaves[d]);
         if (c->fri_nodes[d]) hipFree(c->fri_nodes[d]);
     }
+    if (c->check_partials) hipFree(c->check_partials);
+    if (c->check_ev) hipEventDestroy(c->check_ev);
+    if (c->check_stream) hipStreamDestroy(c->check_stream);
     for (hipEvent_t e : c->upload_done) hipEventDestroy(e);
     if (c->upload_stream) hipStreamDestroy(c->upload_stream);
     for (hipEvent_t e : c->comm_events) hipEventDestroy(e);
@@ -128,6 +131,7 @@
     if ((r = dev_alloc(c, &c->trace_nodes, Nl))) return r;
     if ((r = dev_alloc(c, &c->ceval, 3 * 8 * n))) return r;
     if ((r = dev_alloc(c, &c->cwork, 8 * 8 * n))) return r;
+    if (c->j0 == 0 && (r = dev_alloc(c, &c->check_partials, k_air_check_partials(c) * n))) return r;
     if ((r = dev_alloc(c, &c->cpoly, 8 * n))) return r;
     if ((r = dev_alloc(c, &c->cevals, Nl))) return r;
     if ((r = dev_alloc(c, &c->cnodes, Nl / 2))) return r;
@@ -159,6 +163,7 @@
 static std::vector<fe> copy_fe(const uint8_t* p, size_t count) { std::vector<fe> v(count); memcpy(v.data(), p, count * 16); return v; }
 
 static int drain_pending_upload(dst_ctx* c) {
+    { const int r = k_air_check_drain(c); if (r) return r; }
     if (c->upload_pending && c->upload_stream) HIP_TRY(c, hipStreamSynchronize(c->upload_stream));
     c->upload_pending = false;
     return DST_OK;
@@ -175,7 +180,8 @@
     *out = c;
     return DST_OK;
 }
-void dst_ctx_destroy(dst_ctx* c) { if (!c) return; hipSetDevice(c->device); free_all(c); delete c; }
+void dst_ctx_destroy(dst_ctx* c) { if (!c) return; hipSetDevice(c->device); (void)k_air_check_drain(c); free_all(c); delete c; }
+int64_t dst_last_bad_step(const dst_ctx* c) { return (!c || c->air_flag_host == ~0ull) ? -1 : (int64_t)c->air_flag_host; }
 const char* dst_last_error(const dst_ctx* c) { return c ? c->err.c_str() : g_create_error.c_str(); }
 int dst_phase_ms(const dst_ctx* c, double out_ms[9]) { if (!c || !out_ms) return DST_ERR_ARG; for (int i = 0; i < 9; i++) out_ms[i] = c->phase_ms[i]; return DST_OK; }
 
@@ -280,7 +286,11 @@
     return DST_OK;
 }
 
+static int eval_constraints_phase(dst_ctx* c, const dst_public* pub, const uint8_t* coeffs, uint8_t constraint_root[32], int64_t* bad_step, bool check_here);
 int dst_eval_constraints(dst_ctx* c, const dst_public* pub, const uint8_t* coeffs, uint8_t constraint_root[32], int64_t* bad_step) {
+    return eval_constraints_phase(c, pub, coeffs, constraint_root, bad_step, true);
+}
+static int eval_constraints_phase(dst_ctx* c, const dst_public* pub, const uint8_t* coeffs, uint8_t constraint_root[32], int64_t* bad_step, bool check_here) {
     if (!c || !pub || !coeffs || !constraint_root) return DST_ERR_ARG;
     if (!c->committed) { c->err = "dst_eval_constraints: trace not committed"; return DST_ERR_STATE; }
     if (pub->num_inputs > 8 || pub->num_outputs > 8) { c->err = "too many public inputs / outputs"; return DST_ERR_ARG; }
@@ -289,7 +299,7 @@
     const double t0 = wall_ms();
     HIP_TRY(c, hipEventRecord(c->ph_ev[0], c->stream));
     const bool steps = dst_internal_combine_by_steps(c);
-    int r = step::eval_constraints(c, pub, coeffs, bad_step, !steps);
+    int r = step::eval_constraints(c, pub, coeffs, bad_step, !steps, check_here);
     if (r != DST_OK) return r;
     HIP_TRY(c, hipEventRecord(c->ph_ev[1], c->stream));
     if ((r = step::combine(c, 3))) return r;
@@ -300,7 +310,7 @@
     HIP_TRY(c, hipEventRecord(c->ph_ev[3], c->stream));
     HIP_TRY(c, hipStreamSynchronize(c->stream));
     HIP_TRY(c, hipGetLastError());
-    if (!steps) {
+    if (!steps && check_here) {
         c->air_flag_host = *reinterpret_cast<unsigned long long*>(c->h_stage + HS_AIR_FLAG);
         if ((r = k_constraint_check(c, bad_step)) != DST_OK) { c->err = "transition constraints were not satisfied"; return r; }
     }
@@ -467,20 +477,42 @@
     }
 }
 
+enum AirCheckPlace { AIR_CHECK_INLINE, AIR_CHECK_TRACE, AIR_CHECK_FRI, AIR_CHECK_POW, AIR_CHECK_OPEN };
+static AirCheckPlace air_check_place(const dst_ctx* c) {
+    if (c->sw_is("DISTAFF_AIR_CHECK", "inline")) return AIR_CHECK_INLINE;
+    if (c->sw_is("DISTAFF_AIR_CHECK", "trace")) return AIR_CHECK_TRACE;
+    if (c->sw_is("DISTAFF_AIR_CHECK", "fri")) return AIR_CHECK_FRI;
+    if (c->sw_is("DISTAFF_AIR_CHECK", "open")) return AIR_CHECK_OPEN;
+    return AIR_CHECK_POW;
+}
+static int prove_impl(dst_ctx* c, const dst_public* pub, uint8_t* proof_out, size_t cap, size_t* proof_len);
 int dst_prove(dst_ctx* c, const dst_public* pub, uint8_t* proof_out, size_t cap, size_t* proof_len) {
     if (!c || !pub || !proof_len) return DST_ERR_ARG;
+    int rc = prove_impl(c, pub, proof_out, cap, proof_len);
+    const bool aside = c->check_pending;
+    const double t0 = wall_ms();
+    const int rd = k_air_check_drain(c);
+    if (aside) c->phase_ms[8] += wall_ms() - t0;
+    if (rc == DST_OK && rd != DST_OK) rc = rd;
+    if (rc == DST_OK && aside && k_constraint_check(c, nullptr) != DST_OK) { c->err = "transition constraints were not satisfied"; *proof_len = 0; rc = DST_ERR_AIR; }
+    return rc;
+}
+static int prove_impl(dst_ctx* c, const dst_public* pub, uint8_t* proof_out, size_t cap, size_t* proof_len) {
     int rc;
     uint8_t trace_root[32], constraint_root[32];
+    const AirCheckPlace place = air_check_place(c);
     if ((rc = dst_commit_trace(c, trace_root))) return rc;
+    if (place == AIR_CHECK_TRACE && (rc = k_air_check_side(c))) return rc;
     std::vector<fe> coef(344);
     prng_vector(trace_root, 344, coef.data());
     int64_t bad = -1;
-    if ((rc = dst_eval_constraints(c, pub, (const uint8_t*)coef.data(), constraint_root, &bad))) return rc;
+    if ((rc = eval_constraints_phase(c, pub, (const uint8_t*)coef.data(), constraint_root, &bad, place == AIR_CHECK_INLINE))) return rc;
     std::vector<fe> draws(516);
     prng_vector(constraint_root, 516, draws.data());
     std::vector<uint8_t> z1(c->W * 16), z2(c->W * 16);
     const double t_compose = wall_ms();
     if ((rc = compose_impl(c, (const uint8_t*)draws.data(), z1.data(), z2.data(), false))) return rc;
+    if (place == AIR_CHECK_FRI && (rc = k_air_check_side(c))) return rc;
     {
         const char* ce = c->sw("DISTAFF_FRI_CHAIN");
         if ((rc = fri_commit_all(c, !(ce && ce[0] == '0')))) return rc;
@@ -488,11 +520,13 @@
         if (dev > 0 && dev < both) { c->phase_ms[5] = dev; c->phase_ms[6] = both - dev; }
         else { c->phase_ms[6] = both > c->phase_ms[5] ? both - c->phase_ms[5] : 0.0; }
     }
+    if (place == AIR_CHECK_POW && (rc = k_air_check_side(c))) return rc;
     double t0 = wall_ms();
     uint64_t nonce = 0;
     std::vector<uint64_t> positions;
     if ((rc = step::query_seed(c, &nonce, positions))) return rc;
     c->phase_ms[7] = wall_ms() - t0;
+    if (place == AIR_CHECK_OPEN && (rc = k_air_check_side(c))) return rc;
     return dst_build_proof(c, positions.data(), (uint32_t)positions.size(), nonce, proof_out, cap, proof_len);
 }
 
diff --git a/distaff_amd/csrc/ctx.h b/distaff_amd/csrc/ctx.h
--- a/distaff_amd/csrc/ctx.h
+++ b/distaff_amd/csrc/ctx.h
@@ -32,6 +32,7 @@
     {"DISTAFF_LOCAL_TRANSPORT",    true,  "blocking",        "in-process transport (dst_comm_init_local, dst_prove_sharded_local): drain every rank's stream around each collective instead of the stream-ordered form (events between the ranks' streams, nothing waited for)"},
     {"DISTAFF_TMP_REGS",           true,  "4..W",            "registers per transform launch = size of the staging array (default: as many as 12 GiB hold, at most W)"},
     {"DISTAFF_AIR",                false, "small|deep|generic", "force a more general constraint-kernel instance set than the trace shape needs (generic = per-operation formulation)"},
+    {"DISTAFF_AIR_CHECK",          false, "inline|trace|fri|pow|open", "dst_prove: where the check of the trace rows is queued -- inline: on the main stream behind the evaluation; else on the low-priority side stream, from the end of the trace commitment on (trace), from the first FRI layer on (fri), from the proof of work on (pow), from the openings on (open)"},
     {"DISTAFF_BOUNDARY",           false, "eval",            "boundary combinations by evaluation on the 8n domain (the reference's route) instead of coefficient form"},
     {"DISTAFF_COMBINE",            false, "steps",           "combine_polys / DEEP composition as the reference's sequence of whole-array steps instead of the fused passes"},
     {"DISTAFF_NTT",                false, "pre|pre_a|3pass|reg|lds|row", "force a transform plan family (pre_a: a register pre-stage in the first pass only; row: the default plan with row-major staging array and tables)"},
@@ -198,6 +199,10 @@
     uint8_t *d_fri_chain = nullptr;
     uint8_t *h_stage = nullptr;
     unsigned long long air_flag_host = ~0ull;
+    hipStream_t check_stream = nullptr;
+    hipEvent_t check_ev = nullptr;
+    fe *check_partials = nullptr;
+    bool check_pending = false;
     hipEvent_t ph_ev[6] = {nullptr};
     uint8_t *d_stage = nullptr;
     size_t stage_bytes = 0;
@@ -240,15 +245,17 @@
 
 struct KScope {
     dst_ctx* c; bool on;
+    hipStream_t s;
     dst_ctx::KEvent ev;
-    KScope(dst_ctx* ctx, const char* name, double bytes, bool heavy = false, double mads = 0.0) : c(ctx), on(ctx->profile == 1 || (ctx->profile == 2 && heavy)) {
+    KScope(dst_ctx* ctx, const char* name, double bytes, bool heavy = false, double mads = 0.0, hipStream_t stream = nullptr)
+        : c(ctx), on(ctx->profile == 1 || (ctx->profile == 2 && heavy)), s(stream ? stream : ctx->stream) {
         if (!on) return;
         ev.name = name; ev.bytes = bytes; ev.mads = mads;
         if (c->event_pool.size() >= 2) { ev.e0 = c->event_pool.back(); c->event_pool.pop_back(); ev.e1 = c->event_pool.back(); c->event_pool.pop_back(); }
         else if (hipEventCreate(&ev.e0) != hipSuccess || hipEventCreate(&ev.e1) != hipSuccess) { on = false; return; }
-        (void)hipEventRecord(ev.e0, c->stream);
+        (void)hipEventRecord(ev.e0, s);
     }
-    ~KScope() { if (on) { (void)hipEventRecord(ev.e1, c->stream); c->kpending.push_back(ev); } }
+    ~KScope() { if (on) { (void)hipEventRecord(ev.e1, s); c->kpending.push_back(ev); } }
 };
 
 #define HIP_TRY(ctx, expr)                                                                          \
@@ -283,7 +290,11 @@
 void k_constraint_tree(dst_ctx* c);
 void k_fri_leaves_layer0(dst_ctx* c);
 void k_fri_leaves(dst_ctx* c, int layer);
-int k_eval_constraints(dst_ctx* c, const fe* coeffs_dev, const fe* tc_dev, int64_t* bad_step, bool defer_check = false);
+int k_eval_constraints(dst_ctx* c, const fe* coeffs_dev, const fe* tc_dev, int64_t* bad_step, bool defer_check = false, bool check_here = true);
+int k_air_check(dst_ctx* c, hipStream_t stream);
+int k_air_check_side(dst_ctx* c);
+size_t k_air_check_partials(const dst_ctx* c);
+int k_air_check_drain(dst_ctx* c);
 int k_constraint_check(dst_ctx* c, int64_t* bad_step);
 void k_syn_div(dst_ctx* c, fe* a, size_t len, fe b);
 void k_syn_div_batch(dst_ctx* c, fe* const* a, const fe* b, int count, size_t len);
diff --git a/distaff_amd/csrc/host/steps.h b/distaff_amd/csrc/host/steps.h
--- a/distaff_amd/csrc/host/steps.h
+++ b/distaff_amd/csrc/host/steps.h
@@ -27,7 +27,7 @@
 static_assert(ScratchTail::DRAWS + ScratchTail::MAX_TC <= ScratchTail::ELEMS && ScratchTail::COMPOSE <= ScratchTail::TZ1 && ScratchTail::CZ + 1 <= ScratchTail::ELEMS,
               "the scratch tail holds every phase's vectors for W <= 128 registers");
 
-int eval_constraints(dst_ctx* c, const dst_public* pub, const uint8_t* coeffs, int64_t* bad_step, bool defer_check);
+int eval_constraints(dst_ctx* c, const dst_public* pub, const uint8_t* coeffs, int64_t* bad_step, bool defer_check, bool check_here = true);
 int boundary_polys(dst_ctx* c, const fe* draws344, fe* ip, fe* fp, fe* o0 = nullptr, fe* o1 = nullptr, fe* o2 = nullptr, fe* o3 = nullptr);
 int boundary_quotients(dst_ctx* c, const fe* draws344, fe* q4, size_t stride);
 int combine(dst_ctx* c, int parts);
diff --git a/distaff_amd/csrc/host/steps_impl.h b/distaff_amd/csrc/host/steps_impl.h
--- a/distaff_amd/csrc/host/steps_impl.h
+++ b/distaff_amd/csrc/host/steps_impl.h
@@ -21,7 +21,7 @@
             if (deg[k] == d) { tc[k] = cc[2 * i]; tc[nc + k] = cc[2 * i + 1]; i++; }
 }
 
-int step::eval_constraints(dst_ctx* c, const dst_public* pub, const uint8_t* coeffs, int64_t* bad_step, bool defer_check) {
+int step::eval_constraints(dst_ctx* c, const dst_public* pub, const uint8_t* coeffs, int64_t* bad_step, bool defer_check, bool check_here) {
     c->pub = *pub;
     c->air_draws.resize(344);
     memcpy(c->air_draws.data(), coeffs, 344 * sizeof(fe));
@@ -35,7 +35,7 @@
     memcpy(h + 344, tc.data(), tc.size() * sizeof(fe));
     HIP_TRY(c, hipMemcpyAsync(tail.coef(), h, 344 * sizeof(fe), hipMemcpyHostToDevice, c->stream));
     HIP_TRY(c, hipMemcpyAsync(tail.tc(), h + 344, tc.size() * sizeof(fe), hipMemcpyHostToDevice, c->stream));
-    const int r = k_eval_constraints(c, tail.coef(), tail.tc(), bad_step, defer_check);
+    const int r = k_eval_constraints(c, tail.coef(), tail.tc(), bad_step, defer_check, check_here);
     if (r == DST_ERR_AIR) c->err = "transition constraints were not satisfied";
     return r;
 }
diff --git a/distaff_amd/csrc/kernels_air.hip b/distaff_amd/csrc/kernels_air.hip
--- a/distaff_amd/csrc/kernels_air.hip
+++ b/distaff_amd/csrc/kernels_air.hip
@@ -28,7 +28,7 @@
     if (bad_step) *bad_step = -1;
     return DST_OK;
 }
-int k_eval_constraints(dst_ctx* c, const fe* coeffs_dev, const fe* tc_dev, int64_t* bad_step, bool defer_check) {
+static int air_shape_args(dst_ctx* c, AirArgs& a) {
     if (!c->air_consts) {
         AirConsts h;
         memcpy(h.sponge_mds, SPONGE_MDS, sizeof(h.sponge_mds)); memcpy(h.sponge_inv_mds, SPONGE_INV_MDS, sizeof(h.sponge_inv_mds));
@@ -36,14 +36,7 @@
         HIP_TRY(c, hipMalloc(&c->air_consts, sizeof(AirConsts)));
         HIP_TRY(c, hipMemcpy(c->air_consts, &h, sizeof(AirConsts), hipMemcpyHostToDevice));
     }
-    AirArgs a{};
-    a.lde = c->lde; a.out = c->ceval; a.coef = coeffs_dev; a.tc = tc_dev; a.periodic = c->periodic; a.consts = (const AirConsts*)c->air_consts; a.partial = c->cwork;
-    {
-        const size_t per = (size_t)(c->Bc / (c->B / 8)) * c->n;
-        if (8 * per > c->Bc * c->tmp_regs * c->n) { c->err = "constraint evaluation: staging buffer too small for the stack partial values"; return DST_ERR_STATE; }
-        for (int i = 0; i < 8; i++) a.ev[i] = c->tmp + (size_t)i * per;
-        a.ev[8] = c->cpoly; a.ev[9] = c->comp_poly;
-    }
+    a.lde = c->lde; a.periodic = c->periodic; a.consts = (const AirConsts*)c->air_consts;
     a.tw_lo = c->tw_lo; a.tw_hi = c->tw_hi; a.lo_bits = c->tw_lo_bits;
     a.bad_step = (unsigned long long*)c->d_u64;
     a.n = c->n; a.col_stride = c->Bc * c->n;
@@ -51,15 +44,27 @@
     a.ctx_depth = c->prm.ctx_depth; a.loop_depth = c->prm.loop_depth; a.stack_depth = (uint32_t)c->stack_depth;
     a.coset_step = (uint32_t)(c->B / 8);
     a.q0 = (uint32_t)(c->j0 / (c->B / 8));
+    const uint32_t cd = c->prm.ctx_depth, lp = c->prm.loop_depth, sd = (uint32_t)c->stack_depth;
+    a.cl = cd > 1 ? cd : 1; a.ll = lp > 1 ? lp : 1; a.sl = sd > 8 ? sd : 8;
+    return DST_OK;
+}
+
+int k_eval_constraints(dst_ctx* c, const fe* coeffs_dev, const fe* tc_dev, int64_t* bad_step, bool defer_check, bool check_here) {
+    AirArgs a{};
+    { const int r = air_shape_args(c, a); if (r) return r; }
+    a.out = c->ceval; a.coef = coeffs_dev; a.tc = tc_dev; a.partial = c->cwork;
+    {
+        const size_t per = (size_t)(c->Bc / (c->B / 8)) * c->n;
+        if (8 * per > c->Bc * c->tmp_regs * c->n) { c->err = "constraint evaluation: staging buffer too small for the stack partial values"; return DST_ERR_STATE; }
+        for (int i = 0; i < 8; i++) a.ev[i] = c->tmp + (size_t)i * per;
+        a.ev[8] = c->cpoly; a.ev[9] = c->comp_poly;
+    }
     uint32_t Q = (uint32_t)(c->Bc / (c->B / 8));
     a.num_inputs = c->pub.num_inputs; a.num_outputs = c->pub.num_outputs;
     memcpy(a.inputs, c->pub.inputs, sizeof(a.inputs)); memcpy(a.outputs, c->pub.outputs, sizeof(a.outputs));
     memcpy(a.program_hash, c->program_hash, sizeof(a.program_hash));
     a.op_count = c->op_counter;
-    HIP_TRY(c, hipMemsetAsync(c->d_u64, 0xFF, 8, c->stream));
-    const uint32_t cd = c->prm.ctx_depth, lp = c->prm.loop_depth, sd = (uint32_t)c->stack_depth;
-    a.cl = cd > 1 ? cd : 1; a.ll = lp > 1 ? lp : 1; a.sl = sd > 8 ? sd : 8;
-    switch (air_instance_set(a.cl, a.ll, sd, c->sw("DISTAFF_AIR"))) {
+    switch (air_instance_set(a.cl, a.ll, a.stack_depth, c->sw("DISTAFF_AIR"))) {
         case AIR_SET_SD4: air_launch_sd4(c, a, Q); break;
         case AIR_SET_SMALL: air_launch_small(c, a, Q); break;
         case AIR_SET_GENERIC:
@@ -68,10 +73,59 @@
 #endif
         case AIR_SET_DEEP: air_launch_deep(c, a, Q); break;
     }
-    unsigned long long* flag = c->h_stage ? reinterpret_cast<unsigned long long*>(c->h_stage + HS_AIR_FLAG) : &c->air_flag_host;
-    HIP_TRY(c, hipMemcpyAsync(flag, c->d_u64, 8, hipMemcpyDeviceToHost, c->stream));
+    if (!check_here) return DST_OK;
+    { const int r = k_air_check(c, c->stream); if (r) return r; }
     if (defer_check && c->h_stage) return DST_OK;
     HIP_TRY(c, hipStreamSynchronize(c->stream));
-    c->air_flag_host = *flag;
+    c->air_flag_host = *reinterpret_cast<unsigned long long*>(c->h_stage + HS_AIR_FLAG);
     return k_constraint_check(c, bad_step);
 }
+
+size_t k_air_check_partials(const dst_ctx* c) {
+    const uint32_t cd = c->prm.ctx_depth, lp = c->prm.loop_depth;
+    const bool sd4 = air_instance_set(cd > 1 ? cd : 1, lp > 1 ? lp : 1, (uint32_t)c->stack_depth, c->sw("DISTAFF_AIR")) == AIR_SET_SD4;
+    return (size_t)(sd4 ? air_stack(4, 8).partials : air_stack(0, 12).partials);
+}
+
+int k_air_check(dst_ctx* c, hipStream_t stream) {
+    AirArgs a{};
+    { const int r = air_shape_args(c, a); if (r) return r; }
+    HIP_TRY(c, hipMemsetAsync(c->d_u64, 0xFF, 8, stream));
+    if (a.q0 == 0) {
+        const size_t slots = k_air_check_partials(c) - 2;
+        for (size_t i = 0; i < slots; i++) a.ev[i] = c->check_partials + i * c->n;
+        a.ev[ST_AUX0] = c->check_partials + slots * c->n; a.ev[ST_AUX1] = c->check_partials + (slots + 1) * c->n;
+        switch (air_instance_set(a.cl, a.ll, a.stack_depth, c->sw("DISTAFF_AIR"))) {
+            case AIR_SET_SD4: air_check_sd4(c, a, stream); break;
+            case AIR_SET_SMALL: air_check_small(c, a, stream); break;
+            case AIR_SET_GENERIC:
+            case AIR_SET_DEEP: air_check_deep(c, a, stream); break;
+        }
+    }
+    HIP_TRY(c, hipMemcpyAsync(c->h_stage + HS_AIR_FLAG, c->d_u64, 8, hipMemcpyDeviceToHost, stream));
+    return DST_OK;
+}
+
+int k_air_check_side(dst_ctx* c) {
+    if (!c->check_stream) {
+#ifdef DISTAFF_EMULATED
+        HIP_TRY(c, hipStreamCreateWithFlags(&c->check_stream, hipStreamNonBlocking));
+#else
+        int least = 0, greatest = 0;
+        HIP_TRY(c, hipDeviceGetStreamPriorityRange(&least, &greatest));
+        HIP_TRY(c, hipStreamCreateWithPriority(&c->check_stream, hipStreamNonBlocking, least));
+#endif
+        HIP_TRY(c, hipEventCreateWithFlags(&c->check_ev, hipEventDisableTiming));
+    }
+    HIP_TRY(c, hipEventRecord(c->check_ev, c->stream));
+    HIP_TRY(c, hipStreamWaitEvent(c->check_stream, c->check_ev, 0));
+    c->check_pending = true;
+    return k_air_check(c, c->check_stream);
+}
+int k_air_check_drain(dst_ctx* c) {
+    if (!c->check_pending) return DST_OK;
+    c->check_pending = false;
+    HIP_TRY(c, hipStreamSynchronize(c->check_stream));
+    c->air_flag_host = *reinterpret_cast<unsigned long long*>(c->h_stage + HS_AIR_FLAG);
+    return DST_OK;
+}
diff --git a/distaff_amd/csrc/kernels_air_deep.hip b/distaff_amd/csrc/kernels_air_deep.hip
--- a/distaff_amd/csrc/kernels_air_deep.hip
+++ b/distaff_amd/csrc/kernels_air_deep.hip
@@ -1,14 +1,17 @@
 #include "air_kernel.h"
-void air_launch_deep(dst_ctx* c, const AirArgs& a, uint32_t Q) {
-    launch_air_boundary<16, 8, 0, 12>(c, a, Q);
-    launch_air<16, 8, 0, 12, AS_OP_BITS, 0, AF_FIRST>(c, a, Q);
-    launch_air<16, 8, 0, 12, AS_SPONGE, 0, 0>(c, a, Q);
-    launch_air<16, 8, 0, 12, AS_FLOW, 0, 0>(c, a, Q);
-    launch_air<16, 8, 0, 12, 0, AG_DEEP, 0>(c, a, Q);
-    launch_air<16, 8, 0, 12, 0, AG_RESCR, AF_EV_OUT>(c, a, Q);
-    launch_air<16, 8, 0, 12, 0, AG_PUSH | AG_CMP | AG_KEEP, AF_EV_IN | AF_EV_OUT>(c, a, Q);
-    launch_air<16, 8, 0, 12, 0, AG_LOW(0, 0) | AG_LOW(0, 2), AF_EV_IN | AF_EV_OUT>(c, a, Q);
-    launch_air<16, 8, 0, 12, 0, AG_LOW(0, 1) | AG_LOW(0, 3), AF_EV_IN | AF_EV_OUT>(c, a, Q);
-    launch_air<16, 8, 0, 12, 0, AG_LOW(1, 2) | AG_LOW(1, 3), AF_EV_IN | AF_EV_OUT>(c, a, Q);
-    launch_air<16, 8, 0, 12, 0, AG_LOW(1, 0) | AG_LOW(1, 1), AF_EV_IN | AF_LAST>(c, a, Q);
+template <class CHAIN>
+static void air_chain_deep(const CHAIN& ch) {
+    ch.template boundary<16, 8, 0, 12>();
+    ch.template run<16, 8, 0, 12, AS_OP_BITS, 0, AF_FIRST>();
+    ch.template run<16, 8, 0, 12, AS_SPONGE, 0, 0>();
+    ch.template run<16, 8, 0, 12, AS_FLOW, 0, 0>();
+    ch.template run<16, 8, 0, 12, 0, AG_DEEP, 0>();
+    ch.template run<16, 8, 0, 12, 0, AG_RESCR, AF_EV_OUT>();
+    ch.template run<16, 8, 0, 12, 0, AG_PUSH | AG_CMP | AG_KEEP, AF_EV_IN | AF_EV_OUT>();
+    ch.template run<16, 8, 0, 12, 0, AG_LOW(0, 0) | AG_LOW(0, 2), AF_EV_IN | AF_EV_OUT>();
+    ch.template run<16, 8, 0, 12, 0, AG_LOW(0, 1) | AG_LOW(0, 3), AF_EV_IN | AF_EV_OUT>();
+    ch.template run<16, 8, 0, 12, 0, AG_LOW(1, 2) | AG_LOW(1, 3), AF_EV_IN | AF_EV_OUT>();
+    ch.template run<16, 8, 0, 12, 0, AG_LOW(1, 0) | AG_LOW(1, 1), AF_EV_IN | AF_LAST>();
 }
+void air_launch_deep(dst_ctx* c, const AirArgs& a, uint32_t Q) { air_chain_deep(AirEvalChain{c, a, Q}); }
+void air_check_deep(dst_ctx* c, const AirArgs& a, hipStream_t stream) { air_chain_deep(AirCheckChain{c, a, stream}); }
diff --git a/distaff_amd/csrc/kernels_air_sd4.hip b/distaff_amd/csrc/kernels_air_sd4.hip
--- a/distaff_amd/csrc/kernels_air_sd4.hip
+++ b/distaff_amd/csrc/kernels_air_sd4.hip
@@ -1,9 +1,12 @@
 #include "air_kernel.h"
-void air_launch_sd4(dst_ctx* c, const AirArgs& a, uint32_t Q) {
-    launch_air_boundary<2, 1, 4, 8>(c, a, Q);
-    launch_air<2, 1, 4, 8, AS_OP_BITS | AS_FLOW, 0, AF_FIRST>(c, a, Q);
-    launch_air<2, 1, 4, 8, AS_SPONGE, 0, 0>(c, a, Q);
-    launch_air<2, 1, 4, 8, 0, AG_HIGH, AF_EV_OUT>(c, a, Q);
-    launch_air<2, 1, 4, 8, 0, AG_LOW0, AF_EV_IN | AF_EV_OUT>(c, a, Q);
-    launch_air<2, 1, 4, 8, 0, AG_LOW1, AF_EV_IN | AF_LAST>(c, a, Q);
+template <class CHAIN>
+static void air_chain_sd4(const CHAIN& ch) {
+    ch.template boundary<2, 1, 4, 8>();
+    ch.template run<2, 1, 4, 8, AS_OP_BITS | AS_FLOW, 0, AF_FIRST>();
+    ch.template run<2, 1, 4, 8, AS_SPONGE, 0, 0>();
+    ch.template run<2, 1, 4, 8, 0, AG_HIGH, AF_EV_OUT>();
+    ch.template run<2, 1, 4, 8, 0, AG_LOW0, AF_EV_IN | AF_EV_OUT>();
+    ch.template run<2, 1, 4, 8, 0, AG_LOW1, AF_EV_IN | AF_LAST>();
 }
+void air_launch_sd4(dst_ctx* c, const AirArgs& a, uint32_t Q) { air_chain_sd4(AirEvalChain{c, a, Q}); }
+void air_check_sd4(dst_ctx* c, const AirArgs& a, hipStream_t stream) { air_chain_sd4(AirCheckChain{c, a, stream}); }
diff --git a/distaff_amd/csrc/kernels_air_small.hip b/distaff_amd/csrc/kernels_air_small.hip
--- a/distaff_amd/csrc/kernels_air_small.hip
+++ b/distaff_amd/csrc/kernels_air_small.hip
@@ -1,12 +1,15 @@
 #include "air_kernel.h"
-void air_launch_small(dst_ctx* c, const AirArgs& a, uint32_t Q) {
-    launch_air_boundary<2, 1, 0, 8>(c, a, Q);
-    launch_air<2, 1, 0, 8, AS_OP_BITS | AS_FLOW, 0, AF_FIRST>(c, a, Q);
-    launch_air<2, 1, 0, 8, AS_SPONGE, 0, 0>(c, a, Q);
-    launch_air<2, 1, 0, 8, 0, AG_RESCR, AF_EV_OUT>(c, a, Q);
-    launch_air<2, 1, 0, 8, 0, AG_PUSH | AG_CMP | AG_KEEP, AF_EV_IN | AF_EV_OUT>(c, a, Q);
-    launch_air<2, 1, 0, 8, 0, AG_LOW(0, 0) | AG_LOW(0, 2), AF_EV_IN | AF_EV_OUT>(c, a, Q);
-    launch_air<2, 1, 0, 8, 0, AG_LOW(0, 1) | AG_LOW(0, 3), AF_EV_IN | AF_EV_OUT>(c, a, Q);
-    launch_air<2, 1, 0, 8, 0, AG_LOW(1, 2) | AG_LOW(1, 3), AF_EV_IN | AF_EV_OUT>(c, a, Q);
-    launch_air<2, 1, 0, 8, 0, AG_LOW(1, 0) | AG_LOW(1, 1), AF_EV_IN | AF_LAST>(c, a, Q);
+template <class CHAIN>
+static void air_chain_small(const CHAIN& ch) {
+    ch.template boundary<2, 1, 0, 8>();
+    ch.template run<2, 1, 0, 8, AS_OP_BITS | AS_FLOW, 0, AF_FIRST>();
+    ch.template run<2, 1, 0, 8, AS_SPONGE, 0, 0>();
+    ch.template run<2, 1, 0, 8, 0, AG_RESCR, AF_EV_OUT>();
+    ch.template run<2, 1, 0, 8, 0, AG_PUSH | AG_CMP | AG_KEEP, AF_EV_IN | AF_EV_OUT>();
+    ch.template run<2, 1, 0, 8, 0, AG_LOW(0, 0) | AG_LOW(0, 2), AF_EV_IN | AF_EV_OUT>();
+    ch.template run<2, 1, 0, 8, 0, AG_LOW(0, 1) | AG_LOW(0, 3), AF_EV_IN | AF_EV_OUT>();
+    ch.template run<2, 1, 0, 8, 0, AG_LOW(1, 2) | AG_LOW(1, 3), AF_EV_IN | AF_EV_OUT>();
+    ch.template run<2, 1, 0, 8, 0, AG_LOW(1, 0) | AG_LOW(1, 1), AF_EV_IN | AF_LAST>();
 }
+void air_launch_small(dst_ctx* c, const AirArgs& a, uint32_t Q) { air_chain_small(AirEvalChain{c, a, Q}); }
+void air_check_small(dst_ctx* c, const AirArgs& a, hipStream_t stream) { air_chain_small(AirCheckChain{c, a, stream}); }
diff --git a/distaff_amd/lib.py b/distaff_amd/lib.py
--- a/distaff_amd/lib.py
+++ b/distaff_amd/lib.py
@@ -37,7 +37,7 @@
 
 EXPORTS = ["dst_ctx_create", "dst_ctx_destroy", "dst_last_error", "dst_phase_ms", "dst_trace_upload", "dst_trace_upload_contiguous", "dst_trace_upload_owned",
            "dst_commit_trace", "dst_eval_constraints", "dst_compose", "dst_fri_commit_layer", "dst_fri_fold", "dst_pow_grind",
-           "dst_build_proof", "dst_prove", "dst_prng_vector", "dst_query_positions", "dst_blake3", "dst_fibonacci_trace",
+           "dst_build_proof", "dst_prove", "dst_last_bad_step", "dst_prng_vector", "dst_query_positions", "dst_blake3", "dst_fibonacci_trace",
            "dst_read_buffer", "dst_bench_mulmod", "dst_bench_mad", "dst_bench_code", "dst_trace_upload_async", "dst_pinned_alloc", "dst_pinned_free", "dst_set_profiling", "dst_kernel_stats", "dst_field_op",
            "dst_shard_commit_trace", "dst_shard_eval_constraints", "dst_shard_combine", "dst_shard_fri_layer", "dst_shard_fri_fold",
            "dst_shard_export_size", "dst_shard_export", "dst_shard_import", "dst_shard_read", "dst_shard_fri_begin", "dst_shard_fri_end", "dst_shard_fri_roots", "dst_shard_open", "dst_shard_assemble", "dst_shard_info",
@@ -104,6 +104,9 @@
     lib = ctypes.CDLL(path)
     lib.dst_last_error.restype = ctypes.c_char_p
     lib.dst_last_error.argtypes = [ctypes.c_void_p]
+    if hasattr(lib, "dst_last_bad_step"):
+        lib.dst_last_bad_step.restype = ctypes.c_int64
+        lib.dst_last_bad_step.argtypes = [ctypes.c_void_p]
     return lib
 
 
@@ -741,7 +744,10 @@
         pub = make_public(inputs, outputs)
         buf = ctypes.create_string_buffer(cap)
         ln = ctypes.c_size_t(0)
-        self._check(self.lib.dst_prove(self._h, ctypes.byref(pub), buf, ctypes.c_size_t(cap), ctypes.byref(ln)))
+        r = self.lib.dst_prove(self._h, ctypes.byref(pub), buf, ctypes.c_size_t(cap), ctypes.byref(ln))
+        if hasattr(self.lib, "dst_last_bad_step"):
+            self.bad_step = self.lib.dst_last_bad_step(self._h)
+        self._check(r)
         return buf.raw[:ln.value]
 
     def phase_ms(self):
diff --git a/include/distaff_hip.h b/include/distaff_hip.h
--- a/include/distaff_hip.h
+++ b/include/distaff_hip.h
@@ -67,6 +67,7 @@
                     uint8_t* out, size_t cap, size_t* out_len);
 
 DST_API int dst_prove(dst_ctx* ctx, const dst_public* pub, uint8_t* proof_out, size_t cap, size_t* proof_len);
+DST_API int64_t dst_last_bad_step(const dst_ctx* ctx);
 
 DST_API int dst_verify(const uint8_t program_hash[32], const dst_public* pub, const uint8_t* proof, size_t len,
                        int* accepted, char* err, size_t err_cap);
```

After: 628.5 million, median of 6. 1.01x the previous value.
